# LimpBunion22/VIT-FPGA

Hardware: AMD Instinct MI355X
Metric: images/sec ViT-B/16 224x224, batch 512 per GPU (higher is better)
Workload: dtype bf16; 1 GPU; vit_base 224x224x3 inference, 512 images per GPU resident in HBM, random-init weights (seed 0); global_batch=512, per_gpu_batch=512

## Files before the change

### include/vithip.h

```cpp
#ifndef VITHIP_H
#define VITHIP_H

#include <stddef.h>
#include <stdint.h>

#ifdef __cplusplus
extern "C" {
#endif

#define VH_ABI_VERSION 1

#define VH_OK 0
#define VH_ERR_INVALID 1
#define VH_ERR_HIP 2
#define VH_ERR_STATE 3
#define VH_ERR_UNSUPPORTED 4
#define VH_ERR_NO_DEVICE 5
#define VH_ERR_RING_FULL 6
#define VH_ERR_RING_EMPTY 7

#define VH_DTYPE_BF16 0
#define VH_DTYPE_FP16 1
#define VH_DTYPE_FP8 2

// ... 104 lines not shown
int vh_ring_input_u8(vh_ctx* ctx, uint8_t** pinned_in_nhwc);
int vh_ring_submit_u8(vh_ctx* ctx, const uint8_t* in_nhwc_host, int batch);
int vh_ring_create_frames(vh_ctx* ctx, int slots, int batch_per_slot, size_t slot_bytes);
int vh_ring_input_frames(vh_ctx* ctx, uint8_t** pinned, size_t* capacity);
int vh_ring_submit_frames(vh_ctx* ctx, const uint8_t* frames_host, size_t nbytes, const vh_frame* desc, int batch);
int vh_ring_submit_frames_nv12(vh_ctx* ctx, const uint8_t* frames_host, size_t nbytes, const vh_frame_nv12* desc, int batch);

int vh_set_graph(vh_ctx* ctx, int enable);
int vh_get_graph(const vh_ctx* ctx, int* enabled, int* cached_graphs);

int vh_set_streams(vh_ctx* ctx, int n);
int vh_get_streams(const vh_ctx* ctx, int* n);

int vh_last_forward_us(const vh_ctx* ctx, int64_t* us);
int vh_last_kernel_ms(vh_ctx* ctx, double* ms);
int vh_profile_forward(vh_ctx* ctx, const float* in_nhwc_dev, int batch, float* logits_dev,
                       double* stage_ms, int n_stage_slots, int* n_stages_written);
const char* vh_stage_name(int stage_index);
int vh_set_stage_timing(vh_ctx* ctx, int stage_index);
int vh_get_stage_timing(vh_ctx* ctx, double* avg_ms, double* min_ms, int* launches);
int vh_set_step_timing(vh_ctx* ctx, int enable);
int vh_get_step_timing(vh_ctx* ctx, double* step_ms, int max_steps, int* steps);

int vh_debug_read(vh_ctx* ctx, int what, float* host_out, size_t n_floats);
int vh_debug_set_layers(vh_ctx* ctx, int n_layers);

#define VH_EPI_BIAS 0
#define VH_EPI_BIAS_GELU 1
#define VH_EPI_BIAS_RESID 2
#define VH_EPI_BIAS_F32 3
#define VH_EPI_PATCH 4
#define VH_EPI_LNFOLD 5
#define VH_EPI_LNFOLD_GELU 6
#define VH_EPI_RESID_LN 7
#define VH_EPI_RESID_SPLIT 8
#define VH_EPI_PATCH_SPLIT 9
#define VH_EPI_BIAS_QGELU 10
#define VH_EPI_LNFOLD_QGELU 11
int vh_op_gemm(const void* a16_dev, const void* w16_dev, const float* bias_dev, void* out_dev,
               int64_t M, int N, int K, int epilogue, const float* aux_dev, int aux_i,
               int dtype, int variant, void* stream);

int vh_op_gemm_fp8(const void* a8, const void* w8, const float* w_scale, const float* bias, void* out, int64_t M,
                   int N, int K, int epilogue, int variant , void* stream);
int vh_op_gemm_fp8_ex(const void* a8, const void* w8, const float* w_scale, const float* bias, void* out, int64_t M,
                      int N, int K, int epilogue, const float* c_dev, const float* stats_dev, void* out16,
                      float* partials, int variant, void* stream);
int vh_op_quantize_rows(const float* w, int rows, int cols, float post_scale, void* w8, float* scale, void* stream);

int vh_op_gemm_ex(const void* a16_dev, const void* w16_dev, const float* bias_dev, void* out_dev,
                  int64_t M, int N, int K, int epilogue, const float* aux_dev, int aux_i,
                  const float* stats_dev, void* out16_dev, float* partials_dev,
                  int dtype, int variant, void* stream);
int vh_op_rowstats_cast(const float* x_dev, int64_t rows, int dim, float eps, void* x16_dev, float* stats_dev,
                        int dtype, void* stream);
int vh_op_finalize_stats(const float* partials_dev, int nblk, int64_t rows, int dim, float eps, float* stats_dev,
                         void* stream);
int vh_op_rowstats_split(const float* x_dev, int64_t rows, int dim, float eps, void* hi_dev, void* lo_dev, float* stats_dev,
                         int dtype, void* stream);
int vh_op_fold_ln(const float* w_dev, const float* b_dev, const float* gamma_dev, const float* beta_dev, int rows,
                  int dim, float scale, void* w16_dev, float* c_dev, float* d_dev, int dtype, void* stream);
int vh_op_layernorm(const float* x_dev, int64_t rows, int dim, int64_t row_stride,
                    const float* gamma_dev, const float* beta_dev, float eps, void* out16_dev,
                    int dtype, void* stream);
int vh_op_pre_layernorm(const float* x_dev, int64_t rows, int dim, const float* gamma_dev, const float* beta_dev, float eps,
                        float* y32_dev, void* hi_dev, void* lo_dev, float* stats_dev, int dtype, void* stream);
#define VH_ATTN_Q_SCALE 0.18033688011112042f
int vh_op_attention(const void* qkv16_dev, int batch, int tokens, int heads, void* out16_dev,
                    int dtype, void* stream);
int vh_op_attention_stream(const void* qkv16_dev, int batch, int tokens, int heads, void* out16_dev,
                           int dtype, void* stream);
int vh_op_attention_hd(const void* qkv16_dev, int batch, int tokens, int heads, int head_dim, void* out16_dev,
                       int dtype, void* stream);
int vh_op_attention_cls(const void* qkv16_dev, int batch, int tokens, int heads, void* out16_dev,
                        int dtype, void* stream);
int vh_op_attention_layout(const void* qkv16_dev, int batch, int tokens, int heads, void* out16_dev,
                           int dtype, int out_tiled, int64_t in_hm_rows, void* stream);
int vh_op_im2col(const float* in_nhwc_dev, int batch, int image, int patch, int channels,
                 void* out16_dev, int dtype, void* stream);
int vh_op_im2col_padded(const float* in_nhwc_dev, int batch, int image, int patch, int channels, int kpad,
                        void* out16_dev, int dtype, void* stream);
int vh_op_im2col_u8(const uint8_t* in_nhwc_dev, int batch, int image, int patch, int channels, int kpad,
                    const float* scale_host, const float* shift_host, void* out16_dev, int dtype, void* stream);
int vh_op_resize_u8(const uint8_t* frames_dev, size_t nbytes, const vh_frame* desc_host, int batch, int channels,
                    int out_size, uint8_t* out_u8_dev, void* stream);
int vh_op_resize_nv12(const uint8_t* frames_dev, size_t nbytes, const vh_frame_nv12* desc_host, int batch, int out_size,
                      const float* m12_host, int chroma_site, uint8_t* out_u8_dev, void* stream);
int vh_op_cast(const float* in_dev, void* out16_dev, int64_t n, int dtype, void* stream);
int vh_op_fill(float* out_dev, int64_t n, uint64_t seed, uint32_t tensor_id, int kind,
               float sigma, void* stream);

int vh_bench_gemm(int device, int64_t M, int N, int K, int epilogue, int dtype, int variant, int iters,
                  double* avg_ms);

typedef struct vh_group vh_group;
int vh_group_create(const vh_config* cfg, const int* devices, int n, vh_group** out);
int vh_group_destroy(vh_group* g);
int vh_group_size(const vh_group* g, int* n);
int vh_group_member(vh_group* g, int i, vh_ctx** ctx, int* device);
const char* vh_group_last_error(const vh_group* g);
void vh_group_shard_bounds(int batch, int n, int r, int* lo, int* hi);
int vh_group_load_weights(vh_group* g, const void* host_blob, size_t nbytes);
int vh_group_init_weights_seeded(vh_group* g, uint64_t seed);
int vh_group_broadcast_weights(vh_group* g);
int vh_group_forward(vh_group* g, const float* in_nhwc_host, int batch, float* logits_host);
int vh_group_fill_inputs_seeded(vh_group* g, uint64_t seed, int batch_per_device);
// ... 31 lines not shown
```

### vit-fpga_amd/csrc/gemm_epilogue.h

```cpp
#pragma once

#include "vh_common.h"

namespace vh {

#ifndef VH_EPI_ABL
#define VH_EPI_ABL 0
#endif
#ifndef VH_EPI_NT
#define VH_EPI_NT 1
#endif
template <typename V>
__device__ __forceinline__ void epi_store(V v, V* p) {
    if constexpr (VH_EPI_NT) __builtin_nontemporal_store(v, p);
    else *p = v;
}

struct EpiArgs {
    const float* bias;
    void* out;
    int M, N;
    const float* aux;
    int aux_i;
    const float* stats;
    void* out16;
    float* partials;
    int64_t prow;
};

constexpr bool epi_has_qgelu(int epi) { return epi == VH_EPI_BIAS_QGELU || epi == VH_EPI_LNFOLD_QGELU; }
constexpr bool epi_has_act(int epi) { return epi == VH_EPI_BIAS_GELU || epi == VH_EPI_LNFOLD_GELU || epi_has_qgelu(epi); }
constexpr bool epi_is_lnfold(int epi) { return epi == VH_EPI_LNFOLD || epi == VH_EPI_LNFOLD_GELU || epi == VH_EPI_LNFOLD_QGELU; }
constexpr bool epi_is_16bit(int epi) { return epi == VH_EPI_BIAS || epi == VH_EPI_LNFOLD || epi_has_act(epi); }

__device__ __forceinline__ float gelu_fast(float v) {
    const float u = fabsf(v);
    const float t = __builtin_amdgcn_rcpf(fmaf(0.2316418882f, u, 1.0f));
    float p = fmaf(0.5307027145f, t, -0.7265760135f);
    p = fmaf(p, t, 0.7107068705f);
    p = fmaf(p, t, -0.142248368f);
    p = fmaf(p, t, 0.127414796f);
    p *= t;
    const float h = p * __builtin_amdgcn_exp2f(v * v * -0.72134752044f);
    return fmaf(-u, h, fmaxf(v, 0.f));
}

typedef __attribute__((ext_vector_type(2))) float f32x2;
template <int DEG> struct GeluW;
template <> struct GeluW<9> { static constexpr float a[10] = {1.111100093e-01f, 5.562581867e-02f, 3.875113651e-02f, 7.441916317e-02f, -2.459328771e-01f,
                                                                1.095633626e+00f, -2.419960260e+00f, 3.303298712e+00f, -2.415727854e+00f, 8.016663194e-01f}; };
template <> struct GeluW<8> { static constexpr float a[9] = {1.111119911e-01f, 5.524744466e-02f, 5.048053339e-02f, -6.402773410e-02f, 5.648611188e-01f,
                                                               -1.549515009e+00f, 2.612281084e+00f, -2.240322828e+00f, 8.585962057e-01f}; };
template <> struct GeluW<6> { static constexpr float a[7] = {1.111383960e-01f, 5.238987878e-02f, 9.770081192e-02f, -3.239865899e-01f, 1.061976552e+00f,
                                                               -1.360716462e+00f, 7.577903271e-01f}; };
__device__ __forceinline__ f32x2 pk_fma_clamp01(f32x2 a, f32x2 b, f32x2 c) {
    f32x2 d;
    asm("v_pk_fma_f32 %0, %1, %2, %3 clamp" : "=v"(d) : "v"(a), "v"(b), "v"(c));
    return d;
}
template <int DEG>
// ... 88 lines not shown
        if constexpr (EPI == VH_EPI_PATCH) {
            const int img = m / e.aux_i, p = m - img * e.aux_i;
            orow = (int64_t)img * (e.aux_i + 1) + 1 + p;
            posrow = e.aux + (int64_t)(1 + p) * N;
        }
        float rstd = 0.f, mr = 0.f;
        if constexpr (epi_is_lnfold(EPI)) {
            const float2 st = *(const float2*)(e.stats + 2 * (int64_t)m);
            rstd = st.y;
            mr = st.x * st.y;
        }
        f32x4 addv[NI];
        if constexpr (EPI == VH_EPI_BIAS_RESID || EPI == VH_EPI_PATCH) {
#pragma unroll
            for (int ni = 0; ni < NI; ++ni) {
                const int n = n0 + ni * 16;
                const bool ok = !GUARD || n < N;
                if constexpr (EPI == VH_EPI_BIAS_RESID) addv[ni] = ok ? *(const f32x4*)((const float*)e.out + orow * N + n) : f32x4{0.f, 0.f, 0.f, 0.f};
                else addv[ni] = ok ? *(const f32x4*)(posrow + n) : f32x4{0.f, 0.f, 0.f, 0.f};
            }
        }
#pragma unroll
        for (int ni = 0; ni < NI; ++ni) {
            const int n = n0 + ni * 16;
            if (GUARD && n >= N) continue;
            if constexpr (epi_is_16bit(EPI)) {
                const f32x4 v = epi_value16<EPI, T>(acc[mi][ni], bv[ni], cv[ni], mr, rstd);
                *(typename T::vec4*)((elem*)e.out + orow * N + n) = pack4<T>(v[0], v[1], v[2], v[3]);
            } else {
                const f32x4 v = acc[mi][ni] + bv[ni];
                f32x4* p = (f32x4*)((float*)e.out + orow * N + n);
                if constexpr (EPI == VH_EPI_BIAS_F32) *p = v;
                else *p = v + addv[ni];
            }
        }
    }
}

#ifndef VH_EPI_PRIO
#define VH_EPI_PRIO 1
#endif
__device__ __forceinline__ void epi_consts_from_lds(const char* sw, int frow, int fq, f32x4 (&bv)[4], f32x4 (&cv)[4], float2 (&lnst)[8]) {
    const uint32_t la = (uint32_t)(uintptr_t)sw + (uint32_t)((fq * 4) * 4), lr = (uint32_t)(uintptr_t)sw + (uint32_t)(frow * 8);
    asm volatile("ds_read_b128 %0, %8 offset:1024\n\tds_read_b128 %1, %8 offset:1088\n\tds_read_b128 %2, %8 offset:1152\n\tds_read_b128 %3, %8 offset:1216\n\t"
                 "ds_read_b128 %4, %8 offset:1280\n\tds_read_b128 %5, %8 offset:1344\n\tds_read_b128 %6, %8 offset:1408\n\tds_read_b128 %7, %8 offset:1472"
                 : "=&v"(bv[0]), "=&v"(bv[1]), "=&v"(bv[2]), "=&v"(bv[3]), "=&v"(cv[0]), "=&v"(cv[1]), "=&v"(cv[2]), "=&v"(cv[3]) : "v"(la));
    asm volatile("ds_read_b64 %0, %8\n\tds_read_b64 %1, %8 offset:128\n\tds_read_b64 %2, %8 offset:256\n\tds_read_b64 %3, %8 offset:384\n\t"
                 "ds_read_b64 %4, %8 offset:512\n\tds_read_b64 %5, %8 offset:640\n\tds_read_b64 %6, %8 offset:768\n\tds_read_b64 %7, %8 offset:896\n\t"
                 "s_waitcnt lgkmcnt(0)"
                 : "=&v"(lnst[0]), "=&v"(lnst[1]), "=&v"(lnst[2]), "=&v"(lnst[3]), "=&v"(lnst[4]), "=&v"(lnst[5]), "=&v"(lnst[6]), "=&v"(lnst[7]) : "v"(lr));
    asm volatile("" : "+v"(bv[0]), "+v"(bv[1]), "+v"(bv[2]), "+v"(bv[3]), "+v"(cv[0]), "+v"(cv[1]), "+v"(cv[2]), "+v"(cv[3]));
}

template <typename T, int EPI, int MI, int NI, int SMI = MI, bool MFULL = false, bool OTILED = false>
__device__ __forceinline__ void gemm_epilogue_staged(const f32x4 (&acc)[MI][NI], const EpiArgs& e, int m_w, int n_w,
                                                     int lane, char* sw, int prio_grp = -1, bool cpre = false) {
    static_assert(NI == 4, "staged epilogue assumes a 64-column wave tile");
    static_assert(MI % SMI == 0 && SMI % 2 == 0, "slice must divide the wave tile");
    using elem = typename T::elem;
    const int M = e.M, N = e.N;
    const int frow = lane & 15, fq = lane >> 4;
    f32x4 bv[NI], cv[NI];
    float2 lnst[epi_is_lnfold(EPI) ? MI : 1];
    auto consts_from_global = [&]() {
#pragma unroll
        for (int ni = 0; ni < NI; ++ni) {
            bv[ni] = *(const f32x4*)(e.bias + n_w + ni * 16 + fq * 4);
            if constexpr (epi_is_lnfold(EPI)) cv[ni] = *(const f32x4*)(e.aux + n_w + ni * 16 + fq * 4);
            else cv[ni] = f32x4{0.f, 0.f, 0.f, 0.f};
        }
        if constexpr (epi_is_lnfold(EPI)) {
#pragma unroll
            for (int mi = 0; mi < MI; ++mi) {
                int m = m_w + mi * 16 + frow;
                if constexpr (!MFULL) m = m < M ? m : M - 1;
                lnst[mi] = *(const float2*)(e.stats + 2 * (int64_t)m);
            }
        }
    };
    if constexpr (epi_is_lnfold(EPI) && MI == 8) {
        if (cpre) epi_consts_from_lds(sw, frow, fq, bv, cv, lnst);
        else consts_from_global();
    } else {
        consts_from_global();
    }

    if constexpr (epi_is_16bit(EPI) && (VH_EPI_ABL & 64)) {
#pragma unroll
        for (int mi = 0; mi < MI; ++mi)
#pragma unroll
            for (int ni = 0; ni < NI; ++ni) asm volatile("" :: "v"(acc[mi][ni]));
    } else if constexpr (epi_is_16bit(EPI) && epi_has_act(EPI) && MFULL && OTILED) {
        char* const obase = (char*)e.out + ((int64_t)(m_w >> 4) * (N >> 3) + (n_w >> 3) + (fq & 1) * 2 + (fq >> 1)) * 256 + frow * 16;
#pragma unroll
        for (int mi = 0; mi < MI; ++mi) {
            if constexpr (VH_EPI_PRIO == 1) {
                if (prio_grp >= 0 && (mi & 1) == 0) {
                    if (((mi >> 1) + prio_grp) & 1) __builtin_amdgcn_s_setprio(1);
                    else __builtin_amdgcn_s_setprio(0);
                }
            }
            float rstd = 0.f, mr = 0.f;
            if constexpr (epi_is_lnfold(EPI)) { rstd = lnst[mi].y; mr = lnst[mi].x * lnst[mi].y; }
#pragma unroll
            for (int j = 0; j < NI / 2; ++j) {
                const f32x4 v0 = epi_value16<EPI, T>(acc[mi][2 * j], bv[2 * j], cv[2 * j], mr, rstd);
                const f32x4 v1 = epi_value16<EPI, T>(acc[mi][2 * j + 1], bv[2 * j + 1], cv[2 * j + 1], mr, rstd);
// ... 78 lines not shown
            }
        };
        load_pass(0, xa[0]);
#pragma unroll
        for (int h = 0; h < NP; ++h) {
            if (h + 1 < NP) load_pass(h + 1, xa[(h + 1) & 1]);
#pragma unroll
            for (int mi = 0; mi < FMI; ++mi) {
                const int r = mi * 16 + frow;
#pragma unroll
                for (int ni = 0; ni < NI; ++ni)
                    *(f32x4*)(sw + r * 256 + (((ni * 4 + fq) ^ (r & 15)) << 4)) = acc[h * FMI + mi][ni] + bv[ni];
            }
#pragma unroll
            for (int i = 0; i < NL; ++i) {
                const int r = i * 8 + rr;
                const f32x4 v0 = *(const f32x4*)(sw + r * 256 + (((2 * pc) ^ (r & 15)) << 4));
                const f32x4 v1 = *(const f32x4*)(sw + r * 256 + (((2 * pc + 1) ^ (r & 15)) << 4));
                int m;
                const int64_t off = where(h, i, m);
                const bool ok = MFULL || m < M;
                const Add8& a = xa[h & 1][i];
                const f32x4 h0 = dec4(a.h[0]), h1 = dec4(a.h[1]);
                float v[8];
                float s1 = 0.f, s2 = 0.f;
#pragma unroll
                for (int j = 0; j < 8; ++j) {
                    v[j] = (j < 4 ? v0[j] : v1[j - 4]) + ((j < 4 ? h0[j] : h1[j - 4]) + (float)a.l[j]);
                    s1 += v[j];
                    s2 = fmaf(v[j], v[j], s2);
                }
                const u32x2 hn{pack4_e4m3(v[0], v[1], v[2], v[3]), pack4_e4m3(v[4], v[5], v[6], v[7])};
                const f32x4 d0 = dec4(hn[0]), d1 = dec4(hn[1]);
                lvec8 ln;
#pragma unroll
                for (int j = 0; j < 8; ++j) ln[j] = (typename BF16::elem)(v[j] - (j < 4 ? d0[j] : d1[j - 4]));
                if (ok && !(VH_EPI_ABL & 4)) { *(u32x2*)(hi + off) = hn; *(lvec8*)(lo + off) = ln; }
                s1 += dpp_mov<0xB1>(s1); s2 += dpp_mov<0xB1>(s2);
                s1 += dpp_mov<0x4E>(s1); s2 += dpp_mov<0x4E>(s2);
                s1 += dpp_mov<0x141>(s1); s2 += dpp_mov<0x141>(s2);
                if (ok && pc == 0 && !(VH_EPI_ABL & 1)) *(float2*)(e.partials + 2 * ((int64_t)(n_w >> 6) * M + m)) = make_float2(s1, s2);
            }
        }
    } else if constexpr (EPI == VH_EPI_RESID_SPLIT || EPI == VH_EPI_PATCH_SPLIT) {
        using vec8 = typename T::vec8;
        constexpr bool PATCHS = EPI == VH_EPI_PATCH_SPLIT;
        constexpr int FMI = SMI / 2, NP = MI / FMI, NL = FMI * 2;
        const int rr = lane >> 3, pc = lane & 7;
        elem* const hi = (elem*)e.out;
        uint8_t* const lo = (uint8_t*)e.out16;
        const int64_t prow = PATCHS ? e.prow : (int64_t)M;
        struct Add { vec8 h; u32x2 l; f32x4 p0, p1; };
        Add xa[2][NL];
        const int q0 = PATCHS ? m_w / e.aux_i : 0, r0 = PATCHS ? m_w - q0 * e.aux_i : 0;
        auto where = [&](int h, int i, int& m, int64_t& orow, int& p) {
            const int dr = h * FMI * 16 + i * 8 + rr;
            m = m_w + dr;
            p = 0;
            if constexpr (PATCHS) {
                int img = q0;
                p = r0 + dr;
                while (p >= e.aux_i) { p -= e.aux_i; ++img; }
                orow = (int64_t)m + img + 1;
            } else {
                orow = m;
            }
            return orow * N + n_w + 8 * pc;
        };
        auto load_pass = [&](int h, Add (&a)[NL]) {
#pragma unroll
            for (int i = 0; i < NL; ++i) {
                int m, p;
                int64_t orow;
                const int64_t off = where(h, i, m, orow, p);
                if constexpr (PATCHS) {
                    const float* pr = e.aux + (int64_t)(1 + p) * N + n_w + 8 * pc;
                    a[i].p0 = *(const f32x4*)pr;
                    a[i].p1 = *(const f32x4*)(pr + 4);
                } else {
                    if ((MFULL || m < M) && !(VH_EPI_ABL & 8)) { a[i].h = *(const vec8*)(hi + off); a[i].l = *(const u32x2*)(lo + off); }
                    else { a[i].h = vec8{}; a[i].l = u32x2{0u, 0u}; }
                }
            }
        };
        load_pass(0, xa[0]);
#pragma unroll
        for (int h = 0; h < NP; ++h) {
            if (h + 1 < NP) load_pass(h + 1, xa[(h + 1) & 1]);
#pragma unroll
            for (int mi = 0; mi < FMI; ++mi) {
                const int r = mi * 16 + frow;
#pragma unroll
                for (int ni = 0; ni < NI; ++ni)
                    *(f32x4*)(sw + r * 256 + (((ni * 4 + fq) ^ (r & 15)) << 4)) = acc[h * FMI + mi][ni] + bv[ni];
            }
#pragma unroll
            for (int i = 0; i < NL; ++i) {
                const int r = i * 8 + rr;
                const f32x4 v0 = *(const f32x4*)(sw + r * 256 + (((2 * pc) ^ (r & 15)) << 4));
                const f32x4 v1 = *(const f32x4*)(sw + r * 256 + (((2 * pc + 1) ^ (r & 15)) << 4));
                int m, p;
                int64_t orow;
                const int64_t off = where(h, i, m, orow, p);
                const bool ok = MFULL || m < M;
                const Add& a = xa[h & 1][i];
                float v[8], ln[8];
                vec8 hn;
                float s1 = 0.f, s2 = 0.f;
                f32x4 l0 = f32x4{0.f, 0.f, 0.f, 0.f}, l1 = l0;
                if constexpr (!PATCHS) { l0 = lo8_unpack4<T>(a.l[0]); l1 = lo8_unpack4<T>(a.l[1]); }
#pragma unroll
                for (int j = 0; j < 8; ++j) {
                    const float add = PATCHS ? (j < 4 ? a.p0[j] : a.p1[j - 4]) : ((float)a.h[j] + (j < 4 ? l0[j] : l1[j - 4]));
                    v[j] = (j < 4 ? v0[j] : v1[j - 4]) + add;
                    hn[j] = (elem)v[j];
                    ln[j] = v[j] - (float)hn[j];
                    s1 += v[j];
                    s2 = fmaf(v[j], v[j], s2);
                }
                if (ok && !(VH_EPI_ABL & 4)) {
                    *(vec8*)(hi + off) = hn;
                    *(u32x2*)(lo + off) = u32x2{lo8_pack4<T>(ln[0], ln[1], ln[2], ln[3]), lo8_pack4<T>(ln[4], ln[5], ln[6], ln[7])};
                }
                s1 += dpp_mov<0xB1>(s1); s2 += dpp_mov<0xB1>(s2);
                s1 += dpp_mov<0x4E>(s1); s2 += dpp_mov<0x4E>(s2);
                s1 += dpp_mov<0x141>(s1); s2 += dpp_mov<0x141>(s2);
                if (ok && pc == 0 && !(VH_EPI_ABL & 1)) *(float2*)(e.partials + 2 * ((int64_t)(n_w >> 6) * prow + orow)) = make_float2(s1, s2);
            }
        }
    } else {
        constexpr int FMI = SMI / 2, NP = MI / FMI, NL = FMI * 4;
        constexpr bool RESID = EPI == VH_EPI_BIAS_RESID || EPI == VH_EPI_RESID_LN;
        const int rr = lane >> 4, pc = lane & 15;
        f32x4 xv[2][RESID ? NL : 1];
        auto line = [&](int h, int i, int& m, int& n) {
            const int r = i * 4 + rr;
            n = n_w + ((pc ^ (r & 15)) << 2);
            m = m_w + h * FMI * 16 + r;
            return (f32x4*)((float*)e.out + (int64_t)m * N + n);
        };
        auto load_pass = [&](int h, f32x4 (&x)[RESID ? NL : 1]) {
            if constexpr (RESID) {
#pragma unroll
                for (int i = 0; i < NL; ++i) {
                    int m, n;
                    const f32x4* p = line(h, i, m, n);
                    x[i] = (m < M && !(VH_EPI_ABL & 8)) ? *p : f32x4{0.f, 0.f, 0.f, 0.f};
                }
            }
        };
        load_pass(0, xv[0]);
#pragma unroll
        for (int h = 0; h < NP; ++h) {
            if (h + 1 < NP) load_pass(h + 1, xv[(h + 1) & 1]);
#pragma unroll
            for (int mi = 0; mi < FMI; ++mi) {
                const int r = mi * 16 + frow;
#pragma unroll
                for (int ni = 0; ni < NI; ++ni)
                    *(f32x4*)(sw + r * 256 + (((ni * 4 + fq) ^ (r & 15)) << 4)) = acc[h * FMI + mi][ni] + bv[ni];
            }
#pragma unroll
            for (int i = 0; i < NL; ++i) {
                const int r = i * 4 + rr;
                f32x4 v = *(const f32x4*)(sw + r * 256 + (pc << 4));
                int m, n;
                f32x4* p = line(h, i, m, n);
                const bool ok = m < M;
                if constexpr (RESID) v = v + xv[h & 1][i];
                if (ok && !(VH_EPI_ABL & 4)) *p = v;
                if constexpr (EPI == VH_EPI_RESID_LN) {
                    if (ok && !(VH_EPI_ABL & 2)) *(typename T::vec4*)((elem*)e.out16 + (int64_t)m * N + n) = pack4<T>(v[0], v[1], v[2], v[3]);
                    const float s1 = row16_sum((v[0] + v[1]) + (v[2] + v[3]));
                    const float s2 = row16_sum(fmaf(v[0], v[0], v[1] * v[1]) + fmaf(v[2], v[2], v[3] * v[3]));
                    if (ok && pc == 0 && !(VH_EPI_ABL & 1)) *(float2*)(e.partials + 2 * ((int64_t)(n_w >> 6) * M + m)) = make_float2(s1, s2);
                }
            }
        }
    }
}

template <typename T, int EPI, int MI, int NI, int SMI = MI, bool BARRIER = true>
__device__ __forceinline__ void gemm_epilogue(const f32x4 (&acc)[MI][NI], const EpiArgs& e, int m_w, int n_w, int lane,
                                              bool n_full, bool m_full, char* smem, int wave) {
    if constexpr (EPI != VH_EPI_PATCH) {
        if (EPI == VH_EPI_RESID_LN || EPI == VH_EPI_RESID_SPLIT || EPI == VH_EPI_PATCH_SPLIT || n_full) {
            if constexpr (BARRIER) __syncthreads();
            if (m_full && epi_is_16bit(EPI)) gemm_epilogue_staged<T, EPI, MI, NI, SMI, true>(acc, e, m_w, n_w, lane, smem + wave * (SMI * 16 * 128));
            else gemm_epilogue_staged<T, EPI, MI, NI, SMI, false>(acc, e, m_w, n_w, lane, smem + wave * (SMI * 16 * 128));
            return;
        }
    }
    if constexpr (EPI != VH_EPI_RESID_LN && EPI != VH_EPI_RESID_SPLIT && EPI != VH_EPI_PATCH_SPLIT) {
        const int m0 = m_w + (lane & 15), n0 = n_w + (lane >> 4) * 4;
        if (n_full && m_full) gemm_epilogue_impl<T, EPI, MI, NI, false>(acc, e, m0, n0);
        else gemm_epilogue_impl<T, EPI, MI, NI, true>(acc, e, m0, n0);
    }
}

template <int EPI, int MI, int NI, int SMI, bool MFULL = false, bool OTILED = false>
__device__ __forceinline__ void gemm_epilogue8(const f32x4 (&acc)[MI][NI], const EpiArgs& e, int m_w, int n_w, int lane,
                                               bool n_full, char* smem, int wave, bool cpre = false) {
    static_assert(NI == 4 && MI % SMI == 0, "64-column wave tile");
    static_assert(EPI == VH_EPI_BIAS || (epi_has_act(EPI)), "8-bit output: bias, bias + activation or LN-fold + activation");
    const int M = e.M, N = e.N;
    const int frow = lane & 15, fq = lane >> 4;
    uint8_t* const out = (uint8_t*)e.out;
    auto value = [&](const f32x4& a, const f32x4& b, const f32x4& cq = f32x4{0.f, 0.f, 0.f, 0.f}, float mean_rstd = 0.f, float rstd = 0.f) {
        f32x4 v = epi_value16<EPI, E4M3>(a, b, cq, mean_rstd, rstd);
        return pack4_e4m3(v[0], v[1], v[2], v[3]);
    };
    if (n_full || epi_is_lnfold(EPI)) {
        f32x4 bv[NI], cv[NI];
        float2 lnst[epi_is_lnfold(EPI) ? MI : 1];
        bool have = false;
        if constexpr (epi_is_lnfold(EPI) && MI == 8) { if (cpre) { epi_consts_from_lds(smem + wave * (SMI * 16 * 128), frow, fq, bv, cv, lnst); have = true; } }
        if (!have) {
#pragma unroll
            for (int ni = 0; ni < NI; ++ni) {
                bv[ni] = *(const f32x4*)(e.bias + n_w + ni * 16 + fq * 4);
                if constexpr (epi_is_lnfold(EPI)) cv[ni] = *(const f32x4*)(e.aux + n_w + ni * 16 + fq * 4);
                else cv[ni] = f32x4{0.f, 0.f, 0.f, 0.f};
            }
            if constexpr (epi_is_lnfold(EPI)) {
#pragma unroll
                for (int mi = 0; mi < MI; ++mi) {
                    int m = m_w + mi * 16 + frow;
                    m = m < M ? m : M - 1;
                    lnst[mi] = *(const float2*)(e.stats + 2 * (int64_t)m);
                }
            }
        }
        if constexpr (OTILED && MFULL) {
            uint8_t* const obase = out + ((int64_t)(m_w >> 4) * (N >> 4) + (n_w >> 4) + fq) * 256 + frow * 16;
#pragma unroll
            for (int mi = 0; mi < MI; ++mi) {
                uint32_t x[NI];
#pragma unroll
                for (int ni = 0; ni < NI; ++ni) {
                    if constexpr (epi_is_lnfold(EPI)) x[ni] = value(acc[mi][ni], bv[ni], cv[ni], lnst[mi].x * lnst[mi].y, lnst[mi].y);
                    else x[ni] = value(acc[mi][ni], bv[ni]);
                }
// ... 53 lines not shown
```

### vit-fpga_amd/csrc/kernels_gemm.hip

```cpp
#include <cstdlib>

#include "gemm_epilogue.h"
#include "vh_kernels.h"

namespace vh {

template <typename T, int BM, int BN, int WM, int WN, int EPI>
__global__ void __launch_bounds__(WM* WN * 64)
gemm_nt_kernel(const typename T::elem* __restrict__ A, const typename T::elem* __restrict__ W,
               const float* __restrict__ bias, void* __restrict__ outp, int M, int N, int K,
               const float* __restrict__ aux, int aux_i, int tiles_m, int tiles_n, const float* __restrict__ stats,
               void* __restrict__ out16, float* __restrict__ partials, int64_t prow) {
    using elem = typename T::elem;
    using vec8 = typename T::vec8;
    constexpr int NW = WM * WN;
    constexpr int BK = 64;
    constexpr int ROWS = BM + BN;
    constexpr int STAGE_BYTES = ROWS * 128;
    constexpr int GROUPS_A = BM / 8;
    constexpr int GROUPS = ROWS / 8;
    constexpr int LOADS = GROUPS / NW;
    constexpr int LOADS_A = GROUPS_A / NW;
    constexpr int TM = BM / WM, TN = BN / WN;
    constexpr int MI = TM / 16, NI = TN / 16;
// ... 112 lines not shown
    case VH_EPI_PATCH: return launch_tile<T, VH_EPI_PATCH>(g, variant, s);
    case VH_EPI_LNFOLD: return launch_tile<T, VH_EPI_LNFOLD>(g, variant, s);
    case VH_EPI_LNFOLD_GELU: return launch_tile<T, VH_EPI_LNFOLD_GELU>(g, variant, s);
    case VH_EPI_RESID_LN: return launch_tile<T, VH_EPI_RESID_LN>(g, variant, s);
    case VH_EPI_RESID_SPLIT: return launch_tile<T, VH_EPI_RESID_SPLIT>(g, variant, s);
    case VH_EPI_PATCH_SPLIT: return launch_tile<T, VH_EPI_PATCH_SPLIT>(g, variant, s);
    case VH_EPI_BIAS_QGELU: return launch_tile<T, VH_EPI_BIAS_QGELU>(g, variant, s);
    case VH_EPI_LNFOLD_QGELU: return launch_tile<T, VH_EPI_LNFOLD_QGELU>(g, variant, s);
    default: return hipErrorInvalidValue;
    }
}

int gemm_pp_variant(int epilogue) {
    (void)epilogue;
    static const int v = [] { const int e = env_int("VH_GEMM_PP", 0); return e < 5 || e > 7 ? 0 : e; }();
    return v ? v : 6;
}
int gemm_pick_variant(int64_t M, int N, int epilogue) {
    static const int min_tiles = [] { const int e = env_int("VH_PP_MIN_TILES", 128); return e < 1 ? 1 : e; }();
    const int64_t t256 = ((M + 255) / 256) * ((N + 255) / 256);
    return t256 >= min_tiles ? gemm_pp_variant(epilogue) : 1;
}

bool gemm_tiled_applies(int64_t M, int N, int K) {
    return M > 0 && M % 256 == 0 && N % 256 == 0 && K % 64 == 0 && K / 64 >= 4 && gemm_pick_variant(M, N, VH_EPI_BIAS) == 6;
}

bool gemm_tiled_applies_f8(int64_t M, int N, int K) {
    return M > 0 && M % 256 == 0 && N % 256 == 0 && K % 128 == 0 && K / 128 >= 4 && gemm_pp_variant(VH_EPI_BIAS) == 6;
}

const char* gemm_check(const GemmArgs& g) {
    if (g.M <= 0 || g.N <= 0 || g.K <= 0) return "gemm: empty shape";
    if (g.K % 64) return "gemm: K must be a multiple of 64";
    if (g.N % 4) return "gemm: N must be a multiple of 4";
    if (g.M > 0x7fffffff) return "gemm: M too large";
    if (g.epilogue < 0 || g.epilogue > VH_EPI_LNFOLD_QGELU) return "gemm: unknown epilogue";
    if ((g.epilogue == VH_EPI_LNFOLD || g.epilogue == VH_EPI_LNFOLD_GELU || g.epilogue == VH_EPI_LNFOLD_QGELU) && (!g.stats || !g.aux)) return "gemm: LNFOLD needs stats and c (aux)";
    if ((g.epilogue == VH_EPI_RESID_LN || g.epilogue == VH_EPI_RESID_SPLIT) && (!g.out16 || !g.partials || g.N % 256))
        return "gemm: RESID_LN / RESID_SPLIT need out16, partials and N % 256 == 0";
    if (g.epilogue == VH_EPI_PATCH && (!g.aux || g.aux_i <= 0)) return "gemm: EPI_PATCH needs pos-emb and patches/image";
    if (g.epilogue == VH_EPI_PATCH_SPLIT && (!g.aux || g.aux_i <= 0 || !g.out16 || !g.partials || g.N % 256 || g.prow < 0))
        return "gemm: EPI_PATCH_SPLIT needs pos-emb, patches/image, the lo plane, partials and N % 256 == 0";
    if (g.dtype != VH_DTYPE_BF16 && g.dtype != VH_DTYPE_FP16) return "gemm: dtype";
    if (g.variant < 0 || g.variant > 7) return "gemm: variant";
    if (g.variant == 3 || g.variant == 4) return "gemm: variants 3/4 (BK=32 pipeline) were removed";
    if (!g.a || !g.w || !g.bias || !g.out) return "gemm: null pointer";
    return nullptr;
}

hipError_t launch_gemm(const GemmArgs& g, hipStream_t s) {
    if (gemm_check(g)) return hipErrorInvalidValue;
    const int variant = g.variant ? g.variant : gemm_pick_variant(g.M, g.N, g.epilogue);
    if ((g.out_tiled || g.ab_tiled) && variant != 6) return hipErrorInvalidValue;
    if ((g.tile_count || g.tile_begin) && variant != 5 && variant != 7) return hipErrorInvalidValue;
    return g.dtype == VH_DTYPE_BF16 ? launch_epi<BF16>(g, variant, s) : launch_epi<FP16>(g, variant, s);
}

}
```

### vit-fpga_amd/csrc/kernels_gemm5.hip

```cpp
#include <cstdlib>
#include <type_traits>

#include "gemm_epilogue.h"
#include "vh_kernels.h"

#ifndef VH_PP_SMI
#define VH_PP_SMI 2
#endif

namespace vh {

#ifndef VH_MAIN_ABL
#define VH_MAIN_ABL 0
#endif
#ifndef VH_PP_CPRE
#define VH_PP_CPRE 1
#endif
constexpr int kAblHalf = (VH_MAIN_ABL & 64) ? 1 : 0;
constexpr int kWPieces = kAblHalf ? 2 : 4;
#ifdef VH_DIAG_STAMPS
#ifndef VH_DIAG_KT
#define VH_DIAG_KT -1
#endif
#ifndef VH_DIAG_REC_IT
#define VH_DIAG_REC_IT 1
#endif
#define VH_STAMP_PARAM , unsigned long long* __restrict__ stamps
__device__ __forceinline__ unsigned long long diag_rt() {
    unsigned long long t;
    asm volatile("s_memrealtime %0\n\ts_waitcnt lgkmcnt(0)" : "=s"(t)::"memory");
    return t;
}
__device__ __forceinline__ unsigned long long diag_ct() {
    unsigned long long t;
    asm volatile("s_memtime %0\n\ts_waitcnt lgkmcnt(0)" : "=s"(t)::"memory");
    return t;
}
__device__ __forceinline__ unsigned long long diag_hwid() {
    unsigned int hw, xcc;
    asm volatile("s_getreg_b32 %0, hwreg(HW_REG_HW_ID)" : "=s"(hw));
    asm volatile("s_getreg_b32 %0, hwreg(HW_REG_XCC_ID)" : "=s"(xcc));
    return ((unsigned long long)xcc << 32) | hw;
}
#define VH_STAMP(i, expr) do { __builtin_amdgcn_sched_barrier(0); st_[i] = (expr); __builtin_amdgcn_sched_barrier(0); } while (0)
#define VH_PSTAMP(i) do { if (pst_) { __builtin_amdgcn_sched_barrier(0); const unsigned long long t_ = diag_ct(); \
    if (lane == 0) pst_[i] = t_; __builtin_amdgcn_sched_barrier(0); } } while (0)
#else
#define VH_PSTAMP(i) do { } while (0)
#define VH_STAMP_PARAM
#define VH_STAMP(i, expr) do { } while (0)
#endif

template <int EPI, bool F8>
__host__ __device__ constexpr bool pp_uses_cpre() {
    return VH_PP_CPRE && epi_is_lnfold(EPI) && !(F8 && epi_has_act(EPI));
}

template <int N>
__device__ __forceinline__ void pp_wait_vmcnt() {
    asm volatile("s_waitcnt vmcnt(%0)" ::"n"(N) : "memory");
}
__device__ __forceinline__ void pp_barrier() {
    __builtin_amdgcn_sched_barrier(0);
#if VH_MAIN_ABL & 16
    return;
#endif
    __builtin_amdgcn_s_barrier();
    __builtin_amdgcn_sched_barrier(0);
}
__device__ __forceinline__ int xcd_remap(int bid, int n) {
    const int xcd = bid & 7, qd = n >> 3, rm = n & 7;
    return (xcd < rm ? xcd * (qd + 1) : rm * (qd + 1) + (xcd - rm) * qd) + (bid >> 3);
}

template <typename T, int EPI, bool PERSIST, bool F8 = false, int AST = 2, bool OT = false, bool AT = false>
__global__ void __launch_bounds__(512, 2)
gemm_nt_pp_kernel(const void* __restrict__ Av, const void* __restrict__ Wv,
                  const float* __restrict__ bias, void* __restrict__ outp, int M, int N, int K,
                  const float* __restrict__ aux, int aux_i, int tiles_m, int tiles_n, const float* __restrict__ stats,
                  void* __restrict__ out16, float* __restrict__ partials, int tile0, int sn,
                  const float* __restrict__ wscale, int64_t prow VH_STAMP_PARAM) {
    using vec8 = typename T::vec8;
#ifdef VH_DIAG_STAMPS
    unsigned long long st_[8] = {0, 0, 0, 0, 0, 0, 0, 0};
    int it_ = 0;
    constexpr int rec_it_ = PERSIST ? VH_DIAG_REC_IT : 0;
#define first_tile_ (it_ == rec_it_)
#endif
    constexpr int BM = 256, BN = 256;
    constexpr int KT_BYTES = 128;
    static_assert(!(OT || AT) || PERSIST, "tiled layouts: persistent form only");
    constexpr int KT_STEP = AT ? 2048 : KT_BYTES;
    constexpr int STAGE_BYTES = 65536, W_OFF = 32768;
    static_assert(AST == 2 || (AST == 3 && !PERSIST), "three A stages: one tile per workgroup only");
    const char* const A = (const char*)Av;
    const char* const W = (const char*)Wv;
    const int64_t row_bytes = (int64_t)K * (F8 ? 1 : 2);
    constexpr int MI = 8, NI = 4;

    extern __shared__ __attribute__((aligned(16))) char smem[];

    const int ntiles = tiles_m * tiles_n;
    const int stride = (int)gridDim.x;
    int t = tile0 + xcd_remap(blockIdx.x, stride);

    const int lane = threadIdx.x & 63;
    const int wave = __builtin_amdgcn_readfirstlane(threadIdx.x >> 6);
    const int grp = wave >> 2, wn = wave & 3;

    const int lr = lane >> 3, lc = (lane & 7) ^ lr;
    const int rb = (int)row_bytes;
    struct TileSrc { const char *a, *w; uint32_t oa[4], ow[4]; };
    int tile_m = 0, tile_n = 0;
    auto tile_coords = [&](int tt, int& tm, int& tn) {
        if (sn > 0) {
            const int blk = tiles_m * sn, sc = tt / blk, r = tt - sc * blk;
            const int width = tiles_n - sc * sn < sn ? tiles_n - sc * sn : sn;
            tm = r / width;
            tn = sc * sn + (r - tm * width);
        } else {
            tm = tt / tiles_n;
            tn = tt - tm * tiles_n;
        }
    };
    auto base_a = [&](int tm) { return A + (int64_t)tm * BM * row_bytes; };
    auto base_w = [&](int tn) { return W + (int64_t)tn * BN * row_bytes; };
    TileSrc cur;
    auto setup_tile = [&](int tt) {
// ... 222 lines not shown
            for (int mi = 0; mi < MI_A; ++mi)
#pragma unroll
                for (int ni = 0; ni < NI; ++ni) {
                    if constexpr (VH_MAIN_ABL & 1) asm volatile("" : "+v"(acc[mi][ni]) : "v"(wf1[ni]), "v"(xf[mi]));
                    else acc[mi][ni] = T::mfma16(wf1[ni], xf[mi], acc[mi][ni]);
                }
            __builtin_amdgcn_s_setprio(0);
            c1_wait(kt);
            VH_PSTAMP(7);
            pp_barrier();
        }
        }
        if (grp == 0) pp_barrier();
#ifdef VH_DIAG_STAMPS
        if (first_tile_) { VH_STAMP(6, diag_ct()); VH_STAMP(2, diag_rt()); }
#endif

        const int m_w = tile_m * BM + grp * 128, n_w = tile_n * BN + wn * 64;
        const bool m_full = (tile_m + 1) * BM <= M, n_full = (tile_n + 1) * BN <= N;
        char* const stage_epi = smem + (PERSIST ? 2 * STAGE_BYTES : STAGE_BYTES);
        const EpiArgs e{bias, outp, M, N, aux, aux_i, stats, out16, partials, prow};
        int lane_e = lane;
        if constexpr (PERSIST) asm volatile("" : "+v"(lane_e));
        if constexpr (F8) {
#pragma clang fp contract(off)
            const int fq_e = lane_e >> 4;
            f32x4 wsv[NI];
            if (cpre) {
                const uint32_t la = (uint32_t)(uintptr_t)(smem + 2 * STAGE_BYTES + wave * 4096) + (uint32_t)(fq_e * 16);
                static_assert(NI == 4, "64-column wave tile");
                asm volatile("ds_read_b128 %0, %4 offset:1536\n\tds_read_b128 %1, %4 offset:1600\n\tds_read_b128 %2, %4 offset:1664\n\tds_read_b128 %3, %4 offset:1728\n\t"
                             "s_waitcnt lgkmcnt(0)" : "=&v"(wsv[0]), "=&v"(wsv[1]), "=&v"(wsv[2]), "=&v"(wsv[3]) : "v"(la));
            } else {
#pragma unroll
                for (int ni = 0; ni < NI; ++ni) {
                    const int n = n_w + ni * 16 + fq_e * 4;
                    wsv[ni] = n < N ? *(const f32x4*)(wscale + n) : f32x4{0.f, 0.f, 0.f, 0.f};
                }
            }
#pragma unroll
            for (int ni = 0; ni < NI; ++ni) {
#pragma unroll
                for (int mi = 0; mi < MI; ++mi) acc[mi][ni] = acc[mi][ni] * wsv[ni];
            }
        }
        if constexpr (PERSIST) {
            constexpr int SLICE = VH_PP_SMI * 16 * 128;
            static_assert(VH_PP_SMI == 2, "staging region of the persistent form: 8 waves x 4 KiB");
            if constexpr (F8 && epi_has_act(EPI))
                gemm_epilogue8<EPI, MI, NI, VH_PP_SMI, true, OT>(acc, e, m_w, n_w, lane_e, true, stage_epi, wave, cpre);
            else if constexpr (F8 && (EPI == VH_EPI_RESID_LN || EPI == VH_EPI_RESID_SPLIT))
                gemm_epilogue_staged<E4M3, EPI, MI, NI, VH_PP_SMI, true>(acc, e, m_w, n_w, lane_e, stage_epi + wave * SLICE);
            else
                gemm_epilogue_staged<T, EPI, MI, NI, VH_PP_SMI, true, OT>(acc, e, m_w, n_w, lane_e, stage_epi + wave * SLICE, epi_is_16bit(EPI) ? grp : -1, cpre);
        } else {
            if constexpr (F8 && epi_has_act(EPI))
                gemm_epilogue8<EPI, MI, NI, VH_PP_SMI>(acc, e, m_w, n_w, lane_e, n_full, stage_epi, wave);
            else if constexpr (F8 && (EPI == VH_EPI_RESID_LN || EPI == VH_EPI_RESID_SPLIT))
                gemm_epilogue<E4M3, EPI, MI, NI, 4, false>(acc, e, m_w, n_w, lane_e, n_full, m_full, stage_epi, wave);
            else
                gemm_epilogue<T, EPI, MI, NI, (epi_is_16bit(EPI) ? VH_PP_SMI : 4), false>(acc, e, m_w, n_w, lane_e, n_full, m_full, stage_epi, wave);
        }
#ifdef VH_DIAG_STAMPS
        if (first_tile_) VH_STAMP(3, diag_rt());
        if (!has_next && first_tile_) asm volatile("s_waitcnt vmcnt(0)" ::: "memory");
        if (first_tile_) {
            VH_STAMP(4, diag_rt());
            st_[7] = diag_hwid();
            if (stamps && lane == 0) {
#pragma unroll
                for (int i = 0; i < 8; ++i) stamps[((size_t)blockIdx.x * 8 + wave) * 16 + i] = st_[i];
            }
        }
        ++it_;
#endif
        if (!has_next) break;
        par = (par + nk) & 1;
        first = false;
        t = t_next;
        tile_m = tm_n;
        tile_n = tn_n;
    }
}

static int gemm_super_columns(int tiles_n) {
    static const int env = [] { const int e = env_int("VH_PP_SN", -1); return e < -1 ? -1 : e; }();
    if (env >= 0) return env > 0 && env < tiles_n ? env : 0;
    if (tiles_n < 6) return 0;
    if (tiles_n % 4 == 0) return 4;
    if (tiles_n % 3 == 0) return 3;
    return 4;
}

#ifdef VH_DIAG_STAMPS
struct DiagRec { int64_t M; int N, K, epi, f8, grid, variant; };
static unsigned long long* g_diag_buf = nullptr;
static int g_diag_slots = 0, g_diag_max_wgs = 0;
static long long g_diag_count = 0;
static DiagRec g_diag_rec[1024];
static unsigned long long* diag_next(const GemmArgs& g, int epi, bool f8, int grid, int variant) {
    if (!g_diag_buf || grid > g_diag_max_wgs) return nullptr;
    const int slot = (int)(g_diag_count % g_diag_slots);
    g_diag_rec[slot] = DiagRec{g.M, g.N, g.K, epi, f8 ? 1 : 0, grid, variant};
    ++g_diag_count;
    return g_diag_buf + (size_t)slot * g_diag_max_wgs * 128;
}
#define VH_STAMP_ARG(g, epi, f8, grid, variant) , diag_next(g, epi, f8, grid, variant)
#else
#define VH_STAMP_ARG(g, epi, f8, grid, variant)
#endif

template <typename T, int EPI, bool F8, bool PERSIST, int AST, bool OT = false, bool AT = false>
static hipError_t launch_pp_one(const GemmArgs& g, int grid, int tiles_m, int tiles_n, hipStream_t s) {
    constexpr size_t lds = (AST == 3 || PERSIST) ? 163840 : 131072;
    auto k = gemm_nt_pp_kernel<T, EPI, PERSIST, F8, AST, OT, AT>;
    static LdsDone lds_done;
    if (hipError_t e = ensure_dynamic_lds((const void*)k, lds, lds_done); e != hipSuccess) return e;
    hipLaunchKernelGGL(k, dim3(grid), dim3(512), lds, s, g.a, g.w, g.bias, g.out, (int)g.M, g.N, g.K, g.aux, g.aux_i, tiles_m,
                       tiles_n, g.stats, g.out16, g.partials, PERSIST ? 0 : g.tile_begin, (g.tile_count || g.tile_begin) ? 0 : gemm_super_columns(tiles_n),
                       F8 ? (g.wscale ? g.wscale : g.aux) : (const float*)nullptr, gemm_prow(g)
                       VH_STAMP_ARG(g, EPI, F8, grid, PERSIST ? 6 : (AST == 3 ? 7 : 5)));
    return hipGetLastError();
}

template <typename T, int EPI, bool F8>
static hipError_t launch_pp(const GemmArgs& g, int mode, hipStream_t s) {
    if constexpr (EPI == VH_EPI_PATCH) { if (mode == 1) mode = 0; }
    const int tiles_m = (int)((g.M + 255) / 256), tiles_n = (g.N + 255) / 256;
    int ntiles = tiles_m * tiles_n;
    if (g.tile_count > 0) {
        if (mode == 1 || g.tile_begin < 0 || g.tile_begin + g.tile_count > ntiles) return hipErrorInvalidValue;
        ntiles = g.tile_count;
    } else if (g.tile_begin != 0) {
        return hipErrorInvalidValue;
    }
    if (mode == 2) return launch_pp_one<T, EPI, F8, false, 3>(g, ntiles, tiles_m, tiles_n, s);
    if constexpr (EPI != VH_EPI_PATCH) {
        const int full_m = (int)(g.M / 256);
        const int nk = g.K / (F8 ? 128 : 64);
        if (mode == 1 && (g.N % 256 != 0 || full_m == 0 || nk < (pp_uses_cpre<EPI, F8>() ? 4 : 2))) mode = 0;
        if (mode == 1 && full_m != tiles_m && g.variant != 6) mode = 0;
        if ((g.out_tiled || g.ab_tiled) && (mode != 1 || full_m != tiles_m)) return hipErrorInvalidValue;
        if (mode == 1) {
            const int num_cu = device_num_cu();
            if (!num_cu) return hipErrorUnknown;
            const int nfull = full_m * tiles_n;
            if constexpr (epi_has_act(EPI) || EPI == VH_EPI_LNFOLD || (!F8 && EPI == VH_EPI_BIAS)) {
                if (g.out_tiled) return g.ab_tiled ? hipErrorInvalidValue : launch_pp_one<T, EPI, F8, true, 2, true, false>(g, nfull < num_cu ? nfull : num_cu, full_m, tiles_n, s);
            }
            if constexpr (F8 ? EPI == VH_EPI_RESID_SPLIT : (EPI == VH_EPI_RESID_SPLIT || EPI == VH_EPI_BIAS)) {
                if (g.ab_tiled) return g.out_tiled ? hipErrorInvalidValue : launch_pp_one<T, EPI, F8, true, 2, false, true>(g, nfull < num_cu ? nfull : num_cu, full_m, tiles_n, s);
            }
            if (g.out_tiled || g.ab_tiled) return hipErrorInvalidValue;
            if (hipError_t e = launch_pp_one<T, EPI, F8, true, 2>(g, nfull < num_cu ? nfull : num_cu, full_m, tiles_n, s); e != hipSuccess) return e;
            if (full_m == tiles_m) return hipSuccess;
            GemmArgs tail = g;
            tail.tile_begin = nfull;
            tail.tile_count = tiles_n;
            return launch_pp_one<T, EPI, F8, false, 2>(tail, tiles_n, tiles_m, tiles_n, s);
        }
    }
    if (g.out_tiled || g.ab_tiled) return hipErrorInvalidValue;
    return launch_pp_one<T, EPI, F8, false, 2>(g, ntiles, tiles_m, tiles_n, s);
}

template <typename T, int EPI>
hipError_t launch_gemm_pingpong(const GemmArgs& g, int mode, hipStream_t s) {
    return launch_pp<T, EPI, false>(g, mode, s);
}

#define VH_INST(T)                                                                                     \
    template hipError_t launch_gemm_pingpong<T, VH_EPI_BIAS>(const GemmArgs&, int, hipStream_t);       \
    template hipError_t launch_gemm_pingpong<T, VH_EPI_BIAS_GELU>(const GemmArgs&, int, hipStream_t);  \
    template hipError_t launch_gemm_pingpong<T, VH_EPI_BIAS_RESID>(const GemmArgs&, int, hipStream_t); \
    template hipError_t launch_gemm_pingpong<T, VH_EPI_BIAS_F32>(const GemmArgs&, int, hipStream_t);   \
    template hipError_t launch_gemm_pingpong<T, VH_EPI_PATCH>(const GemmArgs&, int, hipStream_t);       \
    template hipError_t launch_gemm_pingpong<T, VH_EPI_LNFOLD>(const GemmArgs&, int, hipStream_t);      \
    template hipError_t launch_gemm_pingpong<T, VH_EPI_LNFOLD_GELU>(const GemmArgs&, int, hipStream_t); \
    template hipError_t launch_gemm_pingpong<T, VH_EPI_RESID_LN>(const GemmArgs&, int, hipStream_t);   \
    template hipError_t launch_gemm_pingpong<T, VH_EPI_RESID_SPLIT>(const GemmArgs&, int, hipStream_t); \
    template hipError_t launch_gemm_pingpong<T, VH_EPI_PATCH_SPLIT>(const GemmArgs&, int, hipStream_t); \
    template hipError_t launch_gemm_pingpong<T, VH_EPI_BIAS_QGELU>(const GemmArgs&, int, hipStream_t);  \
    template hipError_t launch_gemm_pingpong<T, VH_EPI_LNFOLD_QGELU>(const GemmArgs&, int, hipStream_t);
VH_INST(BF16)
VH_INST(FP16)

hipError_t launch_gemm_fp8(const GemmArgs& g, hipStream_t s) {
    const int v = g.variant ? g.variant : gemm_pp_variant(g.epilogue);
    const int mode = v == 7 ? 2 : (v == 6 && !g.tile_count && !g.tile_begin ? 1 : 0);
    switch (g.epilogue) {
        case VH_EPI_BIAS: return launch_pp<BF16, VH_EPI_BIAS, true>(g, mode, s);
        case VH_EPI_BIAS_GELU: return launch_pp<BF16, VH_EPI_BIAS_GELU, true>(g, mode, s);
        case VH_EPI_BIAS_QGELU: return launch_pp<BF16, VH_EPI_BIAS_QGELU, true>(g, mode, s);
        case VH_EPI_BIAS_RESID: return launch_pp<BF16, VH_EPI_BIAS_RESID, true>(g, mode, s);
        case VH_EPI_BIAS_F32: return launch_pp<BF16, VH_EPI_BIAS_F32, true>(g, mode, s);
        case VH_EPI_LNFOLD: return g.wscale && g.stats && g.aux ? launch_pp<BF16, VH_EPI_LNFOLD, true>(g, mode, s) : hipErrorInvalidValue;
        case VH_EPI_LNFOLD_GELU: return g.wscale && g.stats && g.aux && g.N % 256 == 0 ? launch_pp<BF16, VH_EPI_LNFOLD_GELU, true>(g, mode, s) : hipErrorInvalidValue;
        case VH_EPI_LNFOLD_QGELU: return g.wscale && g.stats && g.aux && g.N % 256 == 0 ? launch_pp<BF16, VH_EPI_LNFOLD_QGELU, true>(g, mode, s) : hipErrorInvalidValue;
        case VH_EPI_RESID_LN: return g.out16 && g.partials && g.N % 256 == 0 ? launch_pp<BF16, VH_EPI_RESID_LN, true>(g, mode, s) : hipErrorInvalidValue;
        case VH_EPI_RESID_SPLIT: return g.out16 && g.partials && g.N % 256 == 0 ? launch_pp<BF16, VH_EPI_RESID_SPLIT, true>(g, mode, s) : hipErrorInvalidValue;
        default: return hipErrorInvalidValue;
    }
}

}

#ifdef VH_DIAG_STAMPS
extern "C" int vh_diag_stamps_arm(int slots, int max_wgs) {
    using namespace vh;
    if (slots < 1 || slots > 1024 || max_wgs < 1) return 1;
    if (g_diag_buf) { hipFree(g_diag_buf); g_diag_buf = nullptr; }
    if (hipMalloc((void**)&g_diag_buf, (size_t)slots * max_wgs * 1024) != hipSuccess) return 2;
    if (hipMemset(g_diag_buf, 0, (size_t)slots * max_wgs * 1024) != hipSuccess) return 2;
    g_diag_slots = slots; g_diag_max_wgs = max_wgs; g_diag_count = 0;
    return 0;
// ... 15 lines not shown
```

### vit-fpga_amd/csrc/kernels_misc.hip

```cpp
#include <type_traits>

#include "vh_kernels.h"

namespace vh {

template <typename T, int CH>
__global__ void __launch_bounds__(256)
layernorm_kernel(const float* __restrict__ x, int64_t rows, int dim, int64_t row_stride,
                 const float* __restrict__ gamma, const float* __restrict__ beta, float eps,
                 typename T::elem* __restrict__ out) {
    const int lane = threadIdx.x & 63;
    const int64_t row = (int64_t)blockIdx.x * 4 + (threadIdx.x >> 6);
    if (row >= rows) return;
    const int nchunk = dim >> 2;
    const f32x4* xr = (const f32x4*)(x + row * row_stride);
    f32x4 v[CH];
    float sum = 0.f;
#pragma unroll
    for (int i = 0; i < CH; ++i) {
        const int c = lane + 64 * i;
        v[i] = c < nchunk ? xr[c] : f32x4{0.f, 0.f, 0.f, 0.f};
        sum += (v[i][0] + v[i][1]) + (v[i][2] + v[i][3]);
    }
#pragma unroll
// ... 158 lines not shown
#pragma unroll
            for (int i = 0; i < 8; ++i) {
                v[i] = k0 + i < kp ? __builtin_fmaf((float)src[((int64_t)ky * image) * ch + r], s_scale[c], s_shift[c]) : 0.f;
                if (++r == pc) { r = 0; ++ky; }
                if (++c == ch) c = 0;
            }
        }
        const typename T::vec4 lo = pack4<T>(v[0], v[1], v[2], v[3]), hi = pack4<T>(v[4], v[5], v[6], v[7]);
        *(typename T::vec8*)(out + f * 8) = __builtin_shufflevector(lo, hi, 0, 1, 2, 3, 4, 5, 6, 7);
    }
}

hipError_t launch_im2col_u8(const uint8_t* in, int batch, int image, int patch, int channels, int kpad, const float* scale,
                            const float* shift, void* out16, int dtype, hipStream_t s) {
    if (patch <= 0 || image % patch || channels < 1 || channels > kMaxChannels || batch < 1) return hipErrorInvalidValue;
    const int kp = patch * patch * channels;
    if (kpad < kp || kpad % 8 || (dtype != VH_DTYPE_BF16 && dtype != VH_DTYPE_FP16)) return hipErrorInvalidValue;
    U8Norm norm;
    for (int c = 0; c < kMaxChannels; ++c) {
        norm.scale[c] = c < channels ? scale[c] : 0.f;
        norm.shift[c] = c < channels ? shift[c] : 0.f;
    }
    const int g = image / patch;
    const int64_t n8 = (int64_t)batch * g * g * (kpad / 8);
    const unsigned grid = (unsigned)((n8 + 255) / 256 < 16384 ? (n8 + 255) / 256 : 16384);
    const bool vec8 = (patch * channels) % 8 == 0 && (image * channels) % 8 == 0 && ((uintptr_t)in & 7) == 0;
    auto go = [&](auto kern, auto* o) { hipLaunchKernelGGL(kern, dim3(grid), dim3(256), 0, s, in, o, n8, image, patch, channels, kpad, norm); };
    if (dtype == VH_DTYPE_BF16) {
        if (vec8) go(im2col_u8_kernel<BF16, true>, (BF16::elem*)out16);
        else go(im2col_u8_kernel<BF16, false>, (BF16::elem*)out16);
    } else {
        if (vec8) go(im2col_u8_kernel<FP16, true>, (FP16::elem*)out16);
        else go(im2col_u8_kernel<FP16, false>, (FP16::elem*)out16);
    }
    return hipGetLastError();
}

__global__ void cls_rows_kernel(float* __restrict__ x, const float* __restrict__ cls, const float* __restrict__ pos,
                                int batch, int tokens, int dim) {
    const int64_t i = (int64_t)blockIdx.x * blockDim.x + threadIdx.x;
    if (i >= (int64_t)batch * dim) return;
    const int b = (int)(i / dim), d = (int)(i - (int64_t)b * dim);
    x[(int64_t)b * tokens * dim + d] = cls[d] + pos[d];
}
hipError_t launch_cls_rows(float* x, const float* cls, const float* pos, int batch, int tokens, int dim, hipStream_t s) {
    const int64_t n = (int64_t)batch * dim;
    hipLaunchKernelGGL(cls_rows_kernel, dim3((unsigned)((n + 255) / 256)), dim3(256), 0, s, x, cls, pos, batch, tokens, dim);
    return hipGetLastError();
}

template <typename T>
__global__ void __launch_bounds__(256)
cls_rows_split_kernel(typename T::elem* __restrict__ hi, uint8_t* __restrict__ lo, float* __restrict__ partials, int64_t prow,
                      const float* __restrict__ cls, const float* __restrict__ pos, int batch, int tokens, int dim) {
    const int lane = threadIdx.x & 63;
    const int b = blockIdx.x * 4 + (threadIdx.x >> 6);
    if (b >= batch) return;
    const int64_t row = (int64_t)b * tokens;
    for (int blk = 0; blk * 64 < dim; ++blk) {
        const int d = blk * 64 + lane;
        float v = 0.f;
        if (d < dim) {
            v = cls[d] + pos[d];
            const typename T::elem h = (typename T::elem)v;
            hi[row * dim + d] = h;
            lo[row * dim + d] = lo8_pack1<T>(v - (float)h);
        }
        float s1 = v, s2 = v * v;
#pragma unroll
        for (int o = 32; o > 0; o >>= 1) { s1 += __shfl_xor(s1, o); s2 += __shfl_xor(s2, o); }
        if (lane == 0) *(float2*)(partials + 2 * ((int64_t)blk * prow + row)) = make_float2(s1, s2);
    }
}
hipError_t launch_cls_rows_split(void* hi, void* lo, float* partials, int64_t prow, const float* cls, const float* pos, int batch,
                                 int tokens, int dim, int dtype, hipStream_t s) {
    if (batch <= 0 || dim % 64) return hipErrorInvalidValue;
    const dim3 grid((unsigned)((batch + 3) / 4));
    if (dtype == VH_DTYPE_BF16)
        hipLaunchKernelGGL(cls_rows_split_kernel<BF16>, grid, dim3(256), 0, s, (BF16::elem*)hi, (uint8_t*)lo, partials, prow, cls, pos, batch, tokens, dim);
    else
        hipLaunchKernelGGL(cls_rows_split_kernel<FP16>, grid, dim3(256), 0, s, (FP16::elem*)hi, (uint8_t*)lo, partials, prow, cls, pos, batch, tokens, dim);
    return hipGetLastError();
}

template <typename T>
__global__ void __launch_bounds__(256) cast_kernel(const float* __restrict__ in, typename T::elem* __restrict__ out, int64_t n4) {
    for (int64_t f = (int64_t)blockIdx.x * blockDim.x + threadIdx.x; f < n4; f += (int64_t)gridDim.x * blockDim.x) {
        const f32x4 v = ((const f32x4*)in)[f];
        ((typename T::vec4*)out)[f] = pack4<T>(v[0], v[1], v[2], v[3]);
    }
}
hipError_t launch_cast(const float* in, void* out16, int64_t n, int dtype, hipStream_t s) {
    if (n <= 0 || (n & 3)) return hipErrorInvalidValue;
    const int64_t n4 = n / 4;
    const unsigned grid = (unsigned)((n4 + 255) / 256 < 8192 ? (n4 + 255) / 256 : 8192);
    if (dtype == VH_DTYPE_FP8) hipLaunchKernelGGL(cast_kernel<E4M3>, dim3(grid), dim3(256), 0, s, in, (E4M3::elem*)out16, n4);
    else if (dtype == VH_DTYPE_BF16) hipLaunchKernelGGL(cast_kernel<BF16>, dim3(grid), dim3(256), 0, s, in, (BF16::elem*)out16, n4);
    else hipLaunchKernelGGL(cast_kernel<FP16>, dim3(grid), dim3(256), 0, s, in, (FP16::elem*)out16, n4);
    return hipGetLastError();
}

template <typename T>
__global__ void __launch_bounds__(256) cast_tiled_w_kernel(const float* __restrict__ w, typename T::elem* __restrict__ out, int rows, int cols) {
    const int64_t nchunk = (int64_t)rows * (cols >> 3);
    for (int64_t i = (int64_t)blockIdx.x * blockDim.x + threadIdx.x; i < nchunk; i += (int64_t)gridDim.x * blockDim.x) {
        const int r16 = (int)(i & 15);
        const int64_t bc = i >> 4;
        const int chunk = (int)(bc % (cols >> 3)), block = (int)(bc / (cols >> 3));
        const float* src = w + (int64_t)(block * 16 + r16) * cols + chunk * 8;
        const f32x4 a = *(const f32x4*)src, b = *(const f32x4*)(src + 4);
        const typename T::vec4 lo = pack4<T>(a[0], a[1], a[2], a[3]), hi = pack4<T>(b[0], b[1], b[2], b[3]);
        *(typename T::vec8*)(out + i * 8) = __builtin_shufflevector(lo, hi, 0, 1, 2, 3, 4, 5, 6, 7);
    }
}
hipError_t launch_cast_tiled_w(const float* w, int rows, int cols, void* w16, int dtype, hipStream_t s) {
    if (rows <= 0 || cols <= 0 || (rows & 15) || (cols & 7)) return hipErrorInvalidValue;
    const int64_t nchunk = (int64_t)rows * (cols >> 3);
    const unsigned grid = (unsigned)((nchunk + 255) / 256 < 8192 ? (nchunk + 255) / 256 : 8192);
    if (dtype == VH_DTYPE_BF16) hipLaunchKernelGGL(cast_tiled_w_kernel<BF16>, dim3(grid), dim3(256), 0, s, w, (BF16::elem*)w16, rows, cols);
    else if (dtype == VH_DTYPE_FP16) hipLaunchKernelGGL(cast_tiled_w_kernel<FP16>, dim3(grid), dim3(256), 0, s, w, (FP16::elem*)w16, rows, cols);
    else return hipErrorInvalidValue;
    return hipGetLastError();
}

__global__ void __launch_bounds__(256) tile_bytes_kernel(const u32x4* __restrict__ w, u32x4* __restrict__ out, int rows, int cols) {
    const int cpr = cols >> 4;
    const int64_t nchunk = (int64_t)rows * cpr;
    for (int64_t i = (int64_t)blockIdx.x * blockDim.x + threadIdx.x; i < nchunk; i += (int64_t)gridDim.x * blockDim.x) {
        const int r16 = (int)(i & 15);
        const int64_t bc = i >> 4;
        const int chunk = (int)(bc % cpr), block = (int)(bc / cpr);
        out[i] = w[(int64_t)(block * 16 + r16) * cpr + chunk];
    }
}
// ... 405 lines not shown
                if constexpr (!std::is_same<T, E4M3>::value) {
                    uint8_t* const xlo = (uint8_t*)lo_;
                    if (xlo) *(uint32_t*)(xlo + row * dim + 4 * c) = lo8_pack4<T>(v[i][0] - (float)hq[0], v[i][1] - (float)hq[1],
                                                                                v[i][2] - (float)hq[2], v[i][3] - (float)hq[3]);
                } else {
                    typename BF16::elem* const xlo = (typename BF16::elem*)lo_;
                    if (xlo) {
                        const uint32_t w = (uint32_t)hq;
                        *(typename BF16::vec4*)(xlo + row * dim + 4 * c) =
                            pack4<BF16>(v[i][0] - __builtin_amdgcn_cvt_f32_fp8((int)w, 0), v[i][1] - __builtin_amdgcn_cvt_f32_fp8((int)w, 1),
                                        v[i][2] - __builtin_amdgcn_cvt_f32_fp8((int)w, 2), v[i][3] - __builtin_amdgcn_cvt_f32_fp8((int)w, 3));
                    }
                }
            }
        }
    }
#pragma unroll
    for (int o = 32; o > 0; o >>= 1) yvar += __shfl_xor(yvar, o);
    const float yrstd = 1.0f / sqrtf(yvar / (float)dim + eps);
    if (stats && lane == 0) *(float2*)(stats + 2 * row) = make_float2(ymean, yrstd);
    if (guard) ln_guard_update(row < guard_rows ? fabsf(ymean) * yrstd : 0.f, guard);
}

template <typename T>
static hipError_t pre_ln_t(const float* x, int64_t rows, int dim, const float* g, const float* b, float eps, float* y32, void* hi, void* lo,
                           float* stats, hipStream_t s, int64_t guard_rows, unsigned int* guard, unsigned int* amax_guard) {
    const dim3 grid((unsigned)((rows + 3) / 4)), block(256);
    auto h = (typename T::elem*)hi;
#define VH_PRE_LN(CH) hipLaunchKernelGGL((pre_layernorm_kernel<T, CH>), grid, block, 0, s, x, rows, dim, g, b, eps, y32, h, lo, stats, guard_rows, guard, amax_guard)
    if (dim <= 256) VH_PRE_LN(1);
    else if (dim <= 512) VH_PRE_LN(2);
    else if (dim <= 768) VH_PRE_LN(3);
    else if (dim <= 1024) VH_PRE_LN(4);
    else if (dim <= 1280) VH_PRE_LN(5);
    else if (dim <= 2048) VH_PRE_LN(8);
    else return hipErrorInvalidValue;
#undef VH_PRE_LN
    return hipGetLastError();
}
hipError_t launch_pre_layernorm(const float* x, int64_t rows, int dim, const float* gamma, const float* beta, float eps, float* y32,
                                void* hi, void* lo, float* stats, int dtype, hipStream_t s, int64_t guard_rows, unsigned int* guard,
                                unsigned int* amax_guard) {
    if (rows <= 0 || dim <= 0 || (dim & 3) || dim > 2048 || !x || !gamma || !beta || (!y32 && !hi) || (lo && !hi)) return hipErrorInvalidValue;
    if (dtype == VH_DTYPE_FP8) return pre_ln_t<E4M3>(x, rows, dim, gamma, beta, eps, y32, hi, lo, stats, s, guard_rows, guard, amax_guard);
    if (dtype == VH_DTYPE_BF16) return pre_ln_t<BF16>(x, rows, dim, gamma, beta, eps, y32, hi, lo, stats, s, guard_rows, guard, amax_guard);
    if (dtype == VH_DTYPE_FP16) return pre_ln_t<FP16>(x, rows, dim, gamma, beta, eps, y32, hi, lo, stats, s, guard_rows, guard, amax_guard);
    return hipErrorInvalidValue;
}

template <typename T>
__global__ void __launch_bounds__(256)
layernorm_split_kernel(const typename T::elem* __restrict__ hi, const void* __restrict__ lo_, int64_t rows, int dim,
                       int64_t row_stride, const float* __restrict__ gamma, const float* __restrict__ beta, float eps,
                       float* __restrict__ out) {
    const int lane = threadIdx.x & 63;
    const int64_t row = (int64_t)blockIdx.x * 4 + (threadIdx.x >> 6);
    if (row >= rows) return;
    const typename T::elem* hr = hi + row * row_stride;
    auto xk = [&](int k) {
        if constexpr (std::is_same<T, E4M3>::value)
            return __builtin_amdgcn_cvt_f32_fp8((int)hr[k], 0) + (float)((const typename BF16::elem*)lo_ + row * row_stride)[k];
        else
            return (float)hr[k] + lo8_unpack1<T>(((const uint8_t*)lo_ + row * row_stride)[k]);
    };
    float sum = 0.f;
    for (int k = lane; k < dim; k += 64) sum += xk(k);
#pragma unroll
    for (int o = 32; o > 0; o >>= 1) sum += __shfl_xor(sum, o);
    const float mean = sum / (float)dim;
    float var = 0.f;
    for (int k = lane; k < dim; k += 64) { const float d = (xk(k)) - mean; var += d * d; }
#pragma unroll
    for (int o = 32; o > 0; o >>= 1) var += __shfl_xor(var, o);
    const float rstd = 1.0f / sqrtf(var / (float)dim + eps);
    for (int k = lane; k < dim; k += 64) out[row * dim + k] = ((xk(k)) - mean) * rstd * gamma[k] + beta[k];
}
hipError_t launch_layernorm_split(const void* hi, const void* lo, int64_t rows, int dim, int64_t row_stride, const float* gamma,
                                  const float* beta, float eps, float* out32, int dtype, hipStream_t s) {
    if (rows <= 0 || dim <= 0) return hipErrorInvalidValue;
    const dim3 grid((unsigned)((rows + 3) / 4)), block(256);
    if (dtype == VH_DTYPE_FP8)
        hipLaunchKernelGGL(layernorm_split_kernel<E4M3>, grid, block, 0, s, (const E4M3::elem*)hi, lo, rows, dim, row_stride, gamma, beta, eps, out32);
    else if (dtype == VH_DTYPE_BF16)
        hipLaunchKernelGGL(layernorm_split_kernel<BF16>, grid, block, 0, s, (const BF16::elem*)hi, (const void*)lo, rows, dim, row_stride, gamma, beta, eps, out32);
    else
        hipLaunchKernelGGL(layernorm_split_kernel<FP16>, grid, block, 0, s, (const FP16::elem*)hi, (const void*)lo, rows, dim, row_stride, gamma, beta, eps, out32);
    return hipGetLastError();
}

__device__ __forceinline__ void ln_guard_update(float ratio, unsigned int* guard) {
    unsigned int b = __float_as_uint(ratio) & 0x7FFFFFFFu;
#pragma unroll
    for (int o = 32; o > 0; o >>= 1) { const unsigned int t = (unsigned int)__shfl_xor((int)b, o); b = t > b ? t : b; }
    if ((threadIdx.x & 63) == 0 && b > __hip_atomic_load(guard, __ATOMIC_RELAXED, __HIP_MEMORY_SCOPE_AGENT)) atomicMax(guard, b);
}
__global__ void __launch_bounds__(256)
finalize_stats_kernel(const float* __restrict__ partials, int nblk, int64_t rows, int dim, float eps, float* __restrict__ stats,
                      int64_t guard_rows, unsigned int* __restrict__ guard, unsigned int* __restrict__ amax_guard) {
    const int64_t r = (int64_t)blockIdx.x * blockDim.x + threadIdx.x;
    float ratio = 0.f, bound = 0.f;
    if (r < rows) {
        float s1 = 0.f, s2 = 0.f, b2 = 0.f;
        constexpr int U = 16;
        for (int b0 = 0; b0 < nblk; b0 += U) {
            float2 p[U];
#pragma unroll
            for (int u = 0; u < U; ++u)
                p[u] = b0 + u < nblk ? *(const float2*)(partials + 2 * ((int64_t)(b0 + u) * rows + r)) : make_float2(0.f, 0.f);
#pragma unroll
            for (int u = 0; u < U; ++u) {
                s1 += p[u].x;
                s2 += p[u].y;
                b2 = fmaxf(b2, p[u].y);
            }
        }
        const float mean = s1 / (float)dim;
        const float var = fmaxf(s2 / (float)dim - mean * mean, 0.f);
        const float rstd = 1.0f / sqrtf(var + eps);
        *(float2*)(stats + 2 * r) = make_float2(mean, rstd);
        if (r < guard_rows) { ratio = fabsf(mean) * rstd; bound = sqrtf(b2); }
    }
    if (guard) ln_guard_update(ratio, guard);
    if (amax_guard) ln_guard_update(bound, amax_guard);
}
hipError_t launch_finalize_stats(const float* partials, int nblk, int64_t rows, int dim, float eps, float* stats, hipStream_t s,
                                 int64_t guard_rows, unsigned int* guard, unsigned int* amax_guard) {
    if (rows <= 0 || nblk <= 0) return hipErrorInvalidValue;
    hipLaunchKernelGGL(finalize_stats_kernel, dim3((unsigned)((rows + 255) / 256)), dim3(256), 0, s, partials, nblk, rows, dim, eps, stats,
                       guard_rows, guard, amax_guard);
    return hipGetLastError();
}
__global__ void __launch_bounds__(256)
ln_guard_kernel(const float* __restrict__ stats, int64_t rows, unsigned int* __restrict__ guard) {
    const int64_t r = (int64_t)blockIdx.x * blockDim.x + threadIdx.x;
    float ratio = 0.f;
    if (r < rows) {
        const float2 st = *(const float2*)(stats + 2 * r);
        ratio = fabsf(st.x) * st.y;
    }
// ... 191 lines not shown
```

### vit-fpga_amd/csrc/vh_common.h

```cpp
#pragma once

#include <hip/hip_runtime.h>
#include <stdint.h>

#include "../../include/vithip.h"

namespace vh {

typedef __attribute__((ext_vector_type(8))) __bf16 bf16x8;
typedef __attribute__((ext_vector_type(4))) __bf16 bf16x4;
typedef __attribute__((ext_vector_type(8))) _Float16 f16x8;
typedef __attribute__((ext_vector_type(4))) _Float16 f16x4;
typedef __attribute__((ext_vector_type(4))) float f32x4;
typedef __attribute__((ext_vector_type(16))) float f32x16;
typedef __attribute__((ext_vector_type(4))) uint32_t u32x4;
typedef __attribute__((ext_vector_type(2))) uint32_t u32x2;

struct BF16 {
    using elem = __bf16;
    using vec8 = bf16x8;
    using vec4 = bf16x4;
    static constexpr int id = VH_DTYPE_BF16;
    static __device__ __forceinline__ f32x4 mfma16(vec8 a, vec8 b, f32x4 c) {
        return __builtin_amdgcn_mfma_f32_16x16x32_bf16(a, b, c, 0, 0, 0);
// ... 32 lines not shown

template <typename T>
__device__ __forceinline__ typename T::vec4 pack4(float a, float b, float c, float d) {
    typedef float f32x2_ __attribute__((ext_vector_type(2)));
    typedef typename T::elem e2_ __attribute__((ext_vector_type(2)));
    const e2_ lo = __builtin_convertvector(f32x2_{a, b}, e2_), hi = __builtin_convertvector(f32x2_{c, d}, e2_);
    return __builtin_shufflevector(lo, hi, 0, 1, 2, 3);
}

typedef __attribute__((ext_vector_type(8))) int i32x8;
struct E4M3 {
    using elem = uint8_t;
    using vec4 = uint32_t;
    static constexpr int id = VH_DTYPE_FP8;
};
__device__ __forceinline__ uint32_t pack4_e4m3(float a, float b, float c, float d) {
    a = __builtin_amdgcn_fmed3f(a, -448.f, 448.f);
    b = __builtin_amdgcn_fmed3f(b, -448.f, 448.f);
    c = __builtin_amdgcn_fmed3f(c, -448.f, 448.f);
    d = __builtin_amdgcn_fmed3f(d, -448.f, 448.f);
    int p = __builtin_amdgcn_cvt_pk_fp8_f32(a, b, 0, false);
    p = __builtin_amdgcn_cvt_pk_fp8_f32(c, d, p, true);
    return (uint32_t)p;
}
template <>
__device__ __forceinline__ uint32_t pack4<E4M3>(float a, float b, float c, float d) {
    return pack4_e4m3(a, b, c, d);
}
template <>
__device__ __forceinline__ f32x4 pack4<F32OUT>(float a, float b, float c, float d) {
    return f32x4{a, b, c, d};
}

template <typename T> struct Lo8;
template <> struct Lo8<BF16> { static constexpr float scale = 32.f, inv = 1.f / 32.f; };
template <> struct Lo8<FP16> { static constexpr float scale = 256.f, inv = 1.f / 256.f; };
template <typename T>
__device__ __forceinline__ uint32_t lo8_pack4(float a, float b, float c, float d) {
    return pack4_e4m3(a * Lo8<T>::scale, b * Lo8<T>::scale, c * Lo8<T>::scale, d * Lo8<T>::scale);
}
template <typename T>
__device__ __forceinline__ f32x4 lo8_unpack4(uint32_t w) {
    typedef float f32x2_ __attribute__((ext_vector_type(2)));
    const f32x2_ a = __builtin_amdgcn_cvt_pk_f32_fp8((int)w, false), b = __builtin_amdgcn_cvt_pk_f32_fp8((int)w, true);
    return f32x4{a[0] * Lo8<T>::inv, a[1] * Lo8<T>::inv, b[0] * Lo8<T>::inv, b[1] * Lo8<T>::inv};
}
template <typename T>
__device__ __forceinline__ uint8_t lo8_pack1(float a) {
    a = __builtin_amdgcn_fmed3f(a * Lo8<T>::scale, -448.f, 448.f);
    return (uint8_t)(__builtin_amdgcn_cvt_pk_fp8_f32(a, a, 0, false) & 0xFF);
}
template <typename T>
__device__ __forceinline__ float lo8_unpack1(uint8_t b) { return __builtin_amdgcn_cvt_f32_fp8((int)b, 0) * Lo8<T>::inv; }

__device__ __forceinline__ void asm_lds_dma16(const void* base, uint32_t lane_off, uint32_t lds_addr) {
    asm volatile("s_mov_b32 m0, %0\n\ts_nop 4\n\tglobal_load_lds_dwordx4 %1, %2"
                 :: "s"(lds_addr), "v"(lane_off), "s"(base) : "memory", "m0");
}
__device__ __forceinline__ void asm_lds_dma4(const void* base, uint32_t lane_off, uint32_t lds_addr) {
    asm volatile("s_mov_b32 m0, %0\n\ts_nop 4\n\tglobal_load_lds_dword %1, %2"
                 :: "s"(lds_addr), "v"(lane_off), "s"(base) : "memory", "m0");
}
__device__ __forceinline__ void asm_atomic_add_ret_issue(unsigned int* base, uint32_t add, uint32_t& ret) {
    const uint32_t zero = 0;
    asm volatile("s_nop 4\n\tglobal_atomic_add %0, %1, %2, %3 sc0" : "=&v"(ret) : "v"(zero), "v"(add), "s"(base) : "memory");
}

__device__ __forceinline__ float gelu_erf(float v) {
    return 0.5f * v * (1.0f + erff(v * 0.70710678118654752440f));
}

__host__ __device__ __forceinline__ uint64_t mix64(uint64_t x) {
    x += 0x9E3779B97F4A7C15ull;
    x ^= x >> 30;
    x *= 0xBF58476D1CE4E5B9ull;
    x ^= x >> 27;
    x *= 0x94D049BB133111EBull;
    x ^= x >> 31;
    return x;
}
__host__ __device__ __forceinline__ uint64_t rng_stream(uint64_t seed, uint32_t tensor_id) {
    return mix64(mix64(seed) ^ (uint64_t)tensor_id);
}
__host__ __device__ __forceinline__ float rng_uniform(uint64_t stream, uint64_t i) {
    const uint64_t w = mix64(stream ^ i);
    const int32_t u = (int32_t)(w >> 40) - (1 << 23);
    return (float)u * (1.0f / 8388608.0f);
}
__host__ __device__ __forceinline__ float rng_ih4(uint64_t stream, uint64_t i, double scale,
                                                  float offset) {
    const uint64_t w = mix64(stream ^ i);
    const int32_t s = (int32_t)(w & 0xFFFF) + (int32_t)((w >> 16) & 0xFFFF) +
                      (int32_t)((w >> 32) & 0xFFFF) + (int32_t)((w >> 48) & 0xFFFF) - 131070;
    const float v = (float)((double)s * scale);
    return offset + v;
}
constexpr double kIH4Std = 37837.22725;

enum : uint32_t { TID_PATCH_W = 1, TID_PATCH_B = 2, TID_CLS = 3, TID_POS = 4, TID_PRE_LN_W = 5, TID_PRE_LN_B = 6, TID_LAYER0 = 16,
                  TID_FINAL = 0x7000, TID_IMAGES = 0x100 };

}
```

### vit-fpga_amd/csrc/vh_kernels.h

```cpp
#pragma once

#include <atomic>
#include <cstdlib>
#include <vector>

#include "vh_common.h"

namespace vh {

struct GemmArgs {
    const void* a;
    const void* w;
    const float* bias;
    void* out;
    int64_t M;
    int N, K;
    int epilogue;
    const float* aux;
    int aux_i;
    int dtype;
    int variant;
    const float* stats = nullptr;
    void* out16 = nullptr;
    float* partials = nullptr;
    const float* wscale = nullptr;
    int tile_begin = 0, tile_count = 0;
    int64_t prow = 0;
    int out_tiled = 0, ab_tiled = 0;
};
bool gemm_tiled_applies(int64_t M, int N, int K);
hipError_t launch_cast_tiled_w(const float* w, int rows, int cols, void* w16, int dtype, hipStream_t stream);
bool gemm_tiled_applies_f8(int64_t M, int N, int K);
hipError_t launch_tile_bytes(const void* w8, int rows, int cols, void* out, hipStream_t stream);

inline int64_t gemm_prow(const GemmArgs& g) {
    if (g.epilogue != VH_EPI_PATCH_SPLIT) return g.M;
    return g.prow > 0 ? g.prow : (g.M / g.aux_i) * (int64_t)(g.aux_i + 1);
}

hipError_t launch_gemm(const GemmArgs& g, hipStream_t stream);
hipError_t launch_gemm_fp8(const GemmArgs& g, hipStream_t stream);
const char* gemm_check(const GemmArgs& g);
int gemm_pick_variant(int64_t M, int N, int epilogue);
int gemm_pp_variant(int epilogue);

hipError_t launch_layernorm(const float* x, int64_t rows, int dim, int64_t row_stride,
                            const float* gamma, const float* beta, float eps, void* out16,
                            int dtype, hipStream_t stream);
constexpr int VH_DTYPE_F32_INTERNAL = 100;
hipError_t launch_head_f32(const float* y, const float* w, const float* bias, float* out, int batch, int classes, int dim,
                           hipStream_t stream);
constexpr float kAttnQScale = 0.125f * 1.4426950408889634f;
hipError_t launch_attention(const void* qkv16, int batch, int tokens, int heads, void* out16,
                            int dtype, unsigned int* ticket, hipStream_t stream, bool ticket_zeroed = false, bool out_tiled = false,
                            int64_t in_hm_rows = 0);
bool attention_tiled_applies(int batch, int tokens, int heads);
hipError_t launch_attention_cls(const void* qkv16, int batch, int tokens, int heads, void* out16, int dtype, hipStream_t stream);
size_t attention_lds_bytes(int tokens);
constexpr int kAttnStreamMaxTokens = 4097;
hipError_t launch_attention_stream(const void* qkv16, int batch, int tokens, int heads, void* out16, int dtype, hipStream_t stream);
constexpr int kAttnHdMaxWidth = 2048;
bool attention_hd_supported(int head_dim);
hipError_t launch_attention_hd(const void* qkv16, int batch, int tokens, int heads, int head_dim, void* out16, int dtype,
                               hipStream_t stream);
inline float attention_q_scale(int head_dim) {
    return head_dim == 64 ? kAttnQScale : (float)(1.4426950408889634 / __builtin_sqrt((double)head_dim));
}
hipError_t launch_im2col(const float* in_nhwc, int batch, int image, int patch, int channels, int kpad,
                         void* out16, int dtype, hipStream_t stream);
constexpr int kMaxChannels = 64;
hipError_t launch_im2col_u8(const uint8_t* in_nhwc, int batch, int image, int patch, int channels, int kpad,
                            const float* scale, const float* shift, void* out16, int dtype, hipStream_t stream);
constexpr int kResizeMaxTaps = 65, kResizeMaxScale = 32, kResizeMaxSide = 8192;
constexpr int kResizeLdsFloats = 16384;
constexpr int kResizeFrameWords = 16;
int resize_axis_table(int n_in, double lo, double hi, int n_out, int32_t* first, int32_t* count, float* weights, int max_taps);
const char* resize_plan_build(const vh_frame* desc, int batch, int channels, int S, size_t nbytes, bool base_aligned4,
                              std::vector<uint32_t>* words, int* max_tiles);
hipError_t launch_resize_u8(const uint8_t* frames, const uint32_t* plan_dev, int batch, int channels, int S, int max_tiles,
                            uint8_t* out_u8, hipStream_t stream);
constexpr int kResizeNv12FrameWords = 24;
int resize_axis_table_over(int n_in, double lo, double hi, double over, int n_out, int32_t* first, int32_t* count, float* weights,
                           int max_taps);
const char* resize_plan_build_nv12(const vh_frame_nv12* desc, int batch, int S, size_t nbytes, bool base_aligned2, int chroma_site,
                                   std::vector<uint32_t>* words, int* max_tiles);
hipError_t launch_resize_nv12(const uint8_t* frames, const uint32_t* plan_dev, int batch, int S, int max_tiles, const float* m12_host,
                              uint8_t* out_u8, hipStream_t stream);
int yuv_matrix(int standard, int full_range, float m[12]);
bool patch_fused_supported(int image, int patch, int channels, int dim);
hipError_t launch_patch_fused(const float* images, int batch, int image, int patch, int channels, const void* wp16, const float* bias,
                              const float* pos, void* hi, void* lo, float* partials, int64_t prow, int dim, int dtype, hipStream_t stream);
hipError_t launch_cls_rows(float* x, const float* cls, const float* pos, int batch, int tokens,
                           int dim, hipStream_t stream);
hipError_t launch_cls_rows_split(void* hi, void* lo, float* partials, int64_t prow, const float* cls, const float* pos, int batch,
                                 int tokens, int dim, int dtype, hipStream_t stream);
hipError_t launch_cast(const float* in, void* out16, int64_t n, int dtype, hipStream_t stream);
hipError_t launch_fill(float* out, int64_t n, uint64_t seed, uint32_t tensor_id, int kind,
                       float sigma, float offset, hipStream_t stream);
hipError_t launch_fake_quant_rows(const float* w, int rows, int cols, float* out, hipStream_t stream);
hipError_t launch_quantize_rows(const float* w, int rows, int cols, float post, void* w8, float* scale, hipStream_t stream);
hipError_t launch_pack_qkv(const float* qw, const float* qb, const float* kw, const float* kb,
                           const float* vw, const float* vb, int dim, float q_scale, void* w16,
                           float* b32, int dtype, hipStream_t stream);
hipError_t launch_permute_patch(const float* w_nchw, int dim, int channels, int patch, int kpad, void* w16,
                                int dtype, hipStream_t stream);
hipError_t launch_rowstats_cast(const float* x, int64_t rows, int dim, float eps, void* x16, float* stats, int dtype,
                                hipStream_t stream, int64_t guard_rows = 0, unsigned int* amax_guard = nullptr);
hipError_t launch_finalize_stats(const float* partials, int nblk, int64_t rows, int dim, float eps, float* stats,
                                 hipStream_t stream, int64_t guard_rows = 0, unsigned int* guard = nullptr,
                                 unsigned int* amax_guard = nullptr);
hipError_t launch_ln_guard(const float* stats, int64_t rows, unsigned int* guard, hipStream_t stream);
hipError_t launch_rowstats_split(const float* x, int64_t rows, int dim, float eps, void* hi, void* lo, float* stats, int dtype,
                                 hipStream_t stream, int64_t guard_rows = 0, unsigned int* amax_guard = nullptr);
hipError_t launch_pre_layernorm(const float* x, int64_t rows, int dim, const float* gamma, const float* beta, float eps, float* y32,
                                void* hi, void* lo, float* stats, int dtype, hipStream_t stream, int64_t guard_rows = 0,
                                unsigned int* guard = nullptr, unsigned int* amax_guard = nullptr);
hipError_t launch_layernorm_split(const void* hi, const void* lo, int64_t rows, int dim, int64_t row_stride, const float* gamma,
                                  const float* beta, float eps, float* out32, int dtype, hipStream_t stream);
hipError_t launch_fold_ln_f8(const float* w, const float* b, const float* gamma, const float* beta, int rows, int dim,
                             float scale, void* w8, float* wscale, float* c, float* d, hipStream_t stream);
hipError_t launch_fold_ln(const float* w, const float* b, const float* gamma, const float* beta, int rows, int dim,
                          float scale, void* w16, float* c, float* d, int dtype, hipStream_t stream);
hipError_t launch_dense_layer(const float* w, const float* b, const float* x, float* y, int n_in,
                              int n_out, int n_vec, int activation, hipStream_t stream, float* z = nullptr);
hipError_t launch_mlp_out_delta(const float* a, const float* z, const float* t, float* d, int64_t n, int act, float* err,
                                hipStream_t stream);
hipError_t launch_mlp_back_delta(const float* w, const float* d, const float* z_prev, float* d_prev, int n_in, int n_out,
                                 int n_sets, int act, hipStream_t stream);
hipError_t launch_mlp_update(float* w, float* b, const float* d, const float* x, int n_in, int n_out, int n_sets, float scale,
                             hipStream_t stream);

hipError_t launch_filter3x3(const uint8_t* in, uint8_t* out, int h, int w, int kind, hipStream_t stream);

constexpr int kMaxDevices = 64;
inline int env_int(const char* name, int dflt) {
    const char* e = getenv(name);
    return e ? atoi(e) : dflt;
}
inline int device_num_cu() {
    static std::atomic<int> table[kMaxDevices];
    int dev = 0;
    if (hipGetDevice(&dev) != hipSuccess || dev < 0 || dev >= kMaxDevices) return 0;
    int n = table[dev].load(std::memory_order_relaxed);
    if (n) return n;
    if (hipDeviceGetAttribute(&n, hipDeviceAttributeMultiprocessorCount, dev) != hipSuccess || n <= 0) return 0;
    table[dev].store(n, std::memory_order_relaxed);
    return n;
}
using LdsDone = std::atomic<int>[kMaxDevices];
inline hipError_t ensure_dynamic_lds(const void* kernel, size_t bytes, LdsDone& done) {
    int dev = 0;
    hipError_t e = hipGetDevice(&dev);
    if (e != hipSuccess) return e;
    if (dev < 0 || dev >= kMaxDevices) return hipErrorInvalidDevice;
    if ((size_t)done[dev].load(std::memory_order_acquire) >= bytes) return hipSuccess;
    e = hipFuncSetAttribute(kernel, hipFuncAttributeMaxDynamicSharedMemorySize, (int)bytes);
    if (e == hipSuccess) done[dev].store((int)bytes, std::memory_order_release);
    return e;
}

}
```

### vit-fpga_amd/csrc/vithip_api.hip

```cpp
#include <dlfcn.h>

#include <chrono>
#include <cmath>
#include <condition_variable>
#include <cstdarg>
#include <cstdio>
#include <cstdlib>
#include <cstring>
#include <functional>
#include <memory>
#include <mutex>
#include <string>
#include <thread>
#include <vector>

#include "vh_kernels.h"

using namespace vh;

namespace {

thread_local std::string g_err;

int fail(std::string* ctx_err, int code, const char* fmt, ...) {
// ... 152 lines not shown
    float* partials = nullptr;
    bool split = false;
    bool cls_tail = false;
    int head_dim = 64;
    float q_scale = kAttnQScale;
    bool patch_fused = false;
    void* xlo16 = nullptr;
    bool ln_fold_cfg = false, split_cfg = false;
    unsigned int* guard_dev = nullptr;
    float* guard_host = nullptr;
    float guard_thresh = 0.5f;
    bool guard_auto = false, guard_tripped = false;
    char* arena = nullptr;
    unsigned int* tickets = nullptr;
    float* x = nullptr;
    void* xn16 = nullptr;
    void* qkv16 = nullptr;
    void* att16 = nullptr;
    void* h16 = nullptr;
    void* col16 = nullptr;
    float* clsn32 = nullptr;
    float* in_dev = nullptr;
    float in_scale[kMaxChannels], in_shift[kMaxChannels];
    float* logits_dev = nullptr;
    uint8_t* rz_u8 = nullptr;
    uint32_t *rz_plan_dev = nullptr, *rz_plan_host = nullptr;
    size_t rz_plan_dev_cap = 0, rz_plan_host_cap = 0;
    uint8_t* rz_frames = nullptr;
    size_t rz_frames_cap = 0;
    std::vector<uint32_t> rz_words;
    float nv12_m[12];
    int nv12_site = VH_CHROMA_LEFT;
    int64_t last_us = 0;
    bool timed = false;
    int last_batch = 0;
    struct RingSlot {
        float *h_in = nullptr, *h_out = nullptr, *d_in = nullptr, *d_out = nullptr;
        hipEvent_t in_done = nullptr, fwd_done = nullptr, out_done = nullptr;
        int batch = 0;
        uint32_t* h_plan = nullptr;
        size_t plan_cap = 0;
    };
    std::vector<RingSlot> ring;
    enum RingKind { RING_F32, RING_U8, RING_FRAMES };
    RingKind ring_kind = RING_F32;
    size_t ring_slot_bytes = 0;
    hipStream_t copy_in = nullptr, copy_out = nullptr;
    int ring_batch = 0, ring_wr = 0, ring_rd = 0, ring_used = 0;
    hipStream_t tstream = nullptr;
    hipEvent_t ev_tail_a = nullptr, ev_tail_l = nullptr;
    bool tail_overlap = false;
    bool last_h_tiled = false;
    bool last_qkv_hm = false;
    int tail_splits = 0;
    int num_cu = 256;
    bool use_graph = false;
    struct GraphEntry { ImgIn in; float* out; int batch; hipGraph_t graph; hipGraphExec_t exec; };
    std::vector<GraphEntry> graphs;
    std::vector<int> graph_warm;
    int timing_stage = -1;
    std::vector<hipEvent_t> tev;
    size_t tev_used = 0;
    bool step_timing = false;
    std::vector<hipEvent_t> sev;
    size_t sev_used = 0;
    std::string err;
};

struct vh_filter {
    int device, height, width, kind;
    struct Slot {
        uint8_t *h_in = nullptr, *h_out = nullptr, *d_in = nullptr, *d_out = nullptr;
        hipEvent_t in_done = nullptr, k_done = nullptr, out_done = nullptr;
    };
    std::vector<Slot> slot;
    hipStream_t copy_in = nullptr, compute = nullptr, copy_out = nullptr;
    int wr = 0, rd = 0, used = 0;
    std::string err;
};

struct vh_mlp {
    int device, n_ins, n_layers, activation;
    std::vector<int> npl;
    size_t n_params = 0, n_neurons = 0;
    int widest = 0, max_vec = 0;
    hipStream_t stream = nullptr;
    float *params = nullptr, *bias = nullptr, *buf0 = nullptr, *buf1 = nullptr;
    bool loaded = false;
    int64_t last_us = 0;
    int n_sets = 0;
    float *set_ins = nullptr, *set_outs = nullptr, *tz = nullptr, *ta = nullptr, *td = nullptr, *terr = nullptr;
    int64_t last_gradient_us = 0;
    std::string err;
};

namespace {

size_t align_up(size_t v, size_t a) { return (v + a - 1) / a * a; }

int set_device(std::string* err, int device) {
    int n = 0;
    hipError_t e = hipGetDeviceCount(&n);
    if (e != hipSuccess || n <= 0) return fail(err, VH_ERR_NO_DEVICE, "no HIP device visible (%s)", hipGetErrorString(e));
    if (device < 0 || device >= n) return fail(err, VH_ERR_INVALID, "device %d out of range (0..%d)", device, n - 1);
    HIPCHK(err, hipSetDevice(device));
    return VH_OK;
// ... 87 lines not shown
    c->split = c->split_cfg;
    drop_graphs(c);
    return VH_OK;
}

int check_blob_header(vh_ctx* c, const BlobHeader& h) {
    const vh_config& f = c->cfg;
    if (memcmp(h.magic, "VHBLOB1", 8) != 0) return fail(&c->err, VH_ERR_INVALID, "weight blob: bad magic");
    if (h.image_size != f.image_size || h.patch_size != f.patch_size || h.channels != f.channels || h.dim != f.dim ||
        h.heads != f.heads || h.mlp_dim != f.mlp_dim || h.layers != f.layers || h.classes != f.classes)
        return fail(&c->err, VH_ERR_INVALID, "weight blob: shape differs from the context's vh_config");
    const uint32_t want = blob_model_bits(f);
    if ((h.flags ^ want) & kBlobPreLn)
        return fail(&c->err, VH_ERR_INVALID, "weight blob: header bit 1 (pre-LayerNorm) is %d, the context's VH_FLAG_PRE_LN is %d",
                    (h.flags & kBlobPreLn) != 0, (want & kBlobPreLn) != 0);
    if ((h.flags ^ want) & kBlobQuickGelu)
        return fail(&c->err, VH_ERR_INVALID, "weight blob: header bit 2 (QuickGELU) is %d, the context's VH_FLAG_QUICK_GELU is %d",
                    (h.flags & kBlobQuickGelu) != 0, (want & kBlobQuickGelu) != 0);
    return VH_OK;
}

int enqueue_forward(vh_ctx* c, ImgIn in, int batch, float* logits, std::vector<std::pair<int, hipEvent_t>>* ev,
                    hipStream_t s, int img0, bool allow_tail = false, bool may_pad = true) {
    const vh_config& f = c->cfg;
    const Layout& L = c->L;
    const int D = f.dim, M = f.mlp_dim, T = L.T;
    const int64_t rows = (int64_t)batch * T;
    const int64_t row_tiles = (rows + 255) / 256;
    const int64_t rows_g = (may_pad && c->ln_fold && row_tiles * ((D + 255) / 256) >= 2 * (int64_t)c->num_cu) ? row_tiles * 256 : rows;
    const float* P = c->params;
    const size_t r0 = (size_t)img0 * T, esz = 2, esz_op = c->fp8 ? 1 : 2;
    const int dt16 = c->dt16;
    float* const x = c->x + r0 * D;
    float* const stats_p = c->stats + r0 * 2;
    float* const partials_p = c->partials + (size_t)(D / 64) * r0 * 2;
    char* const xn16 = (char*)c->xn16 + r0 * D * esz_op;
    char* const xlo16 = (char*)c->xlo16 + r0 * D * (c->fp8 ? 2 : 1);
    char* const qkv16 = (char*)c->qkv16 + r0 * 3 * D * esz;
    char* const att16 = (char*)c->att16 + r0 * D * esz_op;
    char* const h16 = (char*)c->h16 + r0 * M * esz_op;
    char* const col16 = (char*)c->col16 + (size_t)img0 * L.NP * L.KPA * esz;
    float* const clsn32 = c->clsn32 + (size_t)img0 * D;
    unsigned int* const tickets_part = c->tickets + (size_t)img0 * (f.layers > 0 ? f.layers : 1);
    if (f.layers > 0) HIPCHK(&c->err, hipMemsetAsync(tickets_part, 0, sizeof(unsigned int) * f.layers, s));
    unsigned int* const amax_guard = c->fp8 ? c->guard_dev + 1 : nullptr;
    auto mark = [&](int stage) -> int {
        if (!ev) return VH_OK;
        hipEvent_t e;
        HIPCHK(&c->err, hipEventCreate(&e));
        HIPCHK(&c->err, hipEventRecord(e, s));
        ev->push_back({stage, e});
        return VH_OK;
    };
    auto gemm = [&](const void* a, const void* w, const float* bias, void* out, int64_t Mr, int N, int K, int epi,
                    const float* aux, int aux_i, const float* wscale = nullptr) {
        GemmArgs g{a, w, bias, out, Mr, N, K, epi, aux, aux_i, dt16, 0};
        g.stats = stats_p;
        g.out16 = epi == VH_EPI_RESID_SPLIT ? xlo16 : xn16;
        g.partials = partials_p;
        if (wscale) {
            g.dtype = VH_DTYPE_FP8;
            if (epi == VH_EPI_LNFOLD || epi == VH_EPI_LNFOLD_GELU || epi == VH_EPI_LNFOLD_QGELU) g.wscale = wscale;
            else g.aux = wscale;
            return launch_gemm_fp8(g, s);
        }
        return launch_gemm(g, s);
    };
    auto tmark = [&](int stage) -> int {
        if (stage != c->timing_stage) return VH_OK;
        if (c->tev_used == c->tev.size()) {
            hipEvent_t e;
            HIPCHK(&c->err, hipEventCreate(&e));
            c->tev.push_back(e);
        }
        HIPCHK(&c->err, hipEventRecord(c->tev[c->tev_used++], s));
        return VH_OK;
    };
    int rc;
    if (img0 == 0) c->tail_splits = 0;
    if ((rc = mark(-1))) return rc;
    const int nl = (c->run_layers < 0 || c->run_layers > f.layers) ? f.layers : c->run_layers;
    const bool pre_ln = (f.flags & VH_FLAG_PRE_LN) != 0;
    const int epi_fc1 = (f.flags & VH_FLAG_QUICK_GELU) ? VH_EPI_LNFOLD_QGELU : VH_EPI_LNFOLD_GELU;
    const int epi_fc1_plain = (f.flags & VH_FLAG_QUICK_GELU) ? VH_EPI_BIAS_QGELU : VH_EPI_BIAS_GELU;
    const bool fused_patch = !in.u8 && !pre_ln && c->patch_fused && c->split && !c->fp8 && nl > 0 && patch_fused_supported(f.image_size, f.patch_size, f.channels, D);
    if (!fused_patch) {
        if ((rc = tmark(ST_IM2COL))) return rc;
        if (in.u8)
            HIPCHK(&c->err, launch_im2col_u8((const uint8_t*)in.p, batch, f.image_size, f.patch_size, f.channels, L.KPA, c->in_scale, c->in_shift,
                                             col16, dt16, s));
        else
            HIPCHK(&c->err, launch_im2col((const float*)in.p, batch, f.image_size, f.patch_size, f.channels, L.KPA, col16, dt16, s));
        if ((rc = tmark(ST_IM2COL))) return rc;
    }
    if ((rc = mark(ST_IM2COL))) return rc;
    if (fused_patch) {
        if ((rc = tmark(ST_PATCH))) return rc;
        HIPCHK(&c->err, launch_patch_fused((const float*)in.p, batch, f.image_size, f.patch_size, f.channels, c->wp16, P + L.patch_b, P + L.pos, xn16, xlo16,
                                           partials_p, rows_g, D, dt16, s));
        if ((rc = tmark(ST_PATCH))) return rc;
        if ((rc = mark(ST_PATCH))) return rc;
        HIPCHK(&c->err, launch_cls_rows_split(xn16, xlo16, partials_p, rows_g, P + L.cls, P + L.pos, batch, T, D, dt16, s));
        if ((rc = mark(ST_CLS))) return rc;
        HIPCHK(&c->err, launch_finalize_stats(partials_p, D / 64, rows_g, D, f.ln_eps, stats_p, s, rows, c->guard_dev, amax_guard));
        if ((rc = mark(ST_LNSTATS))) return rc;
    } else if (c->split && !c->fp8 && nl > 0 && !pre_ln) {
        GemmArgs g{col16, c->wp16, P + L.patch_b, xn16, (int64_t)batch * L.NP, D, L.KPA, VH_EPI_PATCH_SPLIT, P + L.pos, L.NP, dt16, 0};
        g.out16 = xlo16; g.partials = partials_p; g.prow = rows_g;
        if ((rc = tmark(ST_PATCH))) return rc;
        HIPCHK(&c->err, launch_gemm(g, s));
        if ((rc = tmark(ST_PATCH))) return rc;
        if ((rc = mark(ST_PATCH))) return rc;
        HIPCHK(&c->err, launch_cls_rows_split(xn16, xlo16, partials_p, rows_g, P + L.cls, P + L.pos, batch, T, D, dt16, s));
        if ((rc = mark(ST_CLS))) return rc;
        HIPCHK(&c->err, launch_finalize_stats(partials_p, D / 64, rows_g, D, f.ln_eps, stats_p, s, rows, c->guard_dev, amax_guard));
        if ((rc = mark(ST_LNSTATS))) return rc;
    } else {
        if ((rc = tmark(ST_PATCH))) return rc;
        HIPCHK(&c->err, gemm(col16, c->wp16, P + L.patch_b, x, (int64_t)batch * L.NP, D, L.KPA, VH_EPI_PATCH, P + L.pos, L.NP));
        if ((rc = tmark(ST_PATCH))) return rc;
        if ((rc = mark(ST_PATCH))) return rc;
        HIPCHK(&c->err, launch_cls_rows(x, P + L.cls, P + L.pos, batch, T, D, s));
        if ((rc = mark(ST_CLS))) return rc;
        if (pre_ln) {
            const bool fold0 = c->ln_fold && nl > 0;
            if ((rc = tmark(ST_PRELN))) return rc;
            HIPCHK(&c->err, launch_pre_layernorm(x, fold0 ? rows_g : rows, D, P + L.prew, P + L.preb, f.ln_eps, fold0 && c->split ? nullptr : x,
                                                 fold0 ? xn16 : nullptr, fold0 && c->split ? xlo16 : nullptr, fold0 ? stats_p : nullptr,
                                                 c->fp8 ? VH_DTYPE_FP8 : dt16, s, rows, fold0 ? c->guard_dev : nullptr, fold0 ? amax_guard : nullptr));
            if ((rc = tmark(ST_PRELN))) return rc;
            if ((rc = mark(ST_PRELN))) return rc;
        } else if (c->ln_fold && nl > 0) {
            if (c->split) HIPCHK(&c->err, launch_rowstats_split(x, rows_g, D, f.ln_eps, xn16, xlo16, stats_p, c->fp8 ? VH_DTYPE_FP8 : dt16, s, rows, amax_guard));
            else HIPCHK(&c->err, launch_rowstats_cast(x, rows_g, D, f.ln_eps, xn16, stats_p, c->fp8 ? VH_DTYPE_FP8 : dt16, s, rows, amax_guard));
            HIPCHK(&c->err, launch_ln_guard(stats_p, rows, c->guard_dev, s));
            if ((rc = mark(ST_LNSTATS))) return rc;
        }
    }
    const bool hd64 = c->head_dim == 64;
    const bool tail = c->cls_tail && hd64 && c->ln_fold && c->split && !c->fp8 && nl == f.layers && c->run_layers < 0 && T <= 1024 &&
                      (size_t)L.NP * L.KPA * esz >= 2 * ((size_t)D * esz + 256);
    const bool h_tiled = c->h_tiled && c->split && !c->fp8 && c->weights_ready_tiled && gemm_tiled_applies(rows_g, M, D) && gemm_tiled_applies(rows_g, D, M);
    const bool h_tiled8 = c->h_tiled && c->split && c->fp8 && c->weights_ready_tiled && gemm_tiled_applies_f8(rows_g, M, D) && gemm_tiled_applies_f8(rows_g, D, M);
    const bool att_tiled = hd64 && h_tiled && c->att_tiled && gemm_tiled_applies(rows_g, D, D) && attention_tiled_applies(batch, T, f.heads) && !tail;
    const bool att_tiled8 = hd64 && h_tiled8 && c->att_tiled && gemm_tiled_applies_f8(rows_g, D, D) && attention_tiled_applies(batch, T, f.heads);
    const bool qkv_hm = hd64 && c->qkv_hm && ((att_tiled && gemm_tiled_applies(rows_g, 3 * D, D)) || (att_tiled8 && gemm_tiled_applies_f8(rows_g, 3 * D, D)));
    c->last_h_tiled = (h_tiled || h_tiled8) && nl > 0 && c->ln_fold;
    c->last_qkv_hm = qkv_hm && nl > 0 && c->ln_fold;
    for (int l = 0; l < nl && c->ln_fold; ++l) {
        const LayerOff& o = L.layer[l];
        const float* cd = c->fold_cd + (size_t)l * (6 * D + 2 * M);
        const int nblk = D / 64;
        if ((rc = tmark(ST_QKV))) return rc;
        const float *sq = c->fp8 ? c->sqkv[l] : nullptr, *so = c->fp8 ? c->so[l] : nullptr;
        const float *s1 = c->fp8 ? c->s1[l] : nullptr, *s2 = c->fp8 ? c->s2[l] : nullptr;
        if (qkv_hm) {
            GemmArgs gq{xn16, c->wqkv16[l], cd + 3 * D, qkv16, rows_g, 3 * D, D, VH_EPI_LNFOLD, cd, 0, c->fp8 ? VH_DTYPE_FP8 : dt16, 0};
            gq.stats = stats_p; gq.out_tiled = 1; gq.wscale = sq;
            HIPCHK(&c->err, c->fp8 ? launch_gemm_fp8(gq, s) : launch_gemm(gq, s));
        } else
        HIPCHK(&c->err, gemm(xn16, c->wqkv16[l], cd + 3 * D, qkv16, rows_g, 3 * D, D, VH_EPI_LNFOLD, cd, 0, sq));
        if ((rc = tmark(ST_QKV))) return rc;
        if ((rc = mark(ST_QKV))) return rc;
        if (tail && l + 1 == nl) {
            char* const hc = col16;
            char* const lc = col16 + (((size_t)batch * D * esz + 255) & ~(size_t)255);
            HIPCHK(&c->err, launch_attention_cls(qkv16, batch, T, f.heads, att16, dt16, s));
            if ((rc = mark(ST_ATTN))) return rc;
            HIPCHK(&c->err, hipMemcpy2DAsync(hc, (size_t)D * esz, xn16, (size_t)T * D * esz, (size_t)D * esz, batch, hipMemcpyDeviceToDevice, s));
            HIPCHK(&c->err, hipMemcpy2DAsync(lc, (size_t)D, xlo16, (size_t)T * D, (size_t)D, batch, hipMemcpyDeviceToDevice, s));
            GemmArgs gp{att16, c->wo16[l], P + o.ob, hc, batch, D, D, VH_EPI_RESID_SPLIT, nullptr, 0, dt16, 0};
            gp.out16 = lc; gp.partials = partials_p;
            HIPCHK(&c->err, launch_gemm(gp, s));
            if ((rc = mark(ST_PROJ))) return rc;
            HIPCHK(&c->err, launch_finalize_stats(partials_p, nblk, batch, D, f.ln_eps, stats_p, s, batch, c->guard_dev));
            if ((rc = mark(ST_LNSTATS))) return rc;
            GemmArgs g1{hc, c->w1_16[l], cd + 6 * D + M, h16, batch, M, D, epi_fc1, cd + 6 * D, 0, dt16, 0};
            g1.stats = stats_p;
            HIPCHK(&c->err, launch_gemm(g1, s));
            if ((rc = mark(ST_FC1))) return rc;
            GemmArgs g2{h16, c->w2_16[l], P + o.f2b, hc, batch, D, M, VH_EPI_RESID_SPLIT, nullptr, 0, dt16, 0};
            g2.out16 = lc; g2.partials = partials_p;
            HIPCHK(&c->err, launch_gemm(g2, s));
            if ((rc = mark(ST_FC2))) return rc;
            HIPCHK(&c->err, launch_layernorm_split(hc, lc, batch, D, D, P + L.lnfw, P + L.lnfb, f.ln_eps, clsn32, dt16, s));
            if ((rc = mark(ST_LNF))) return rc;
            HIPCHK(&c->err, launch_head_f32(clsn32, P + L.headw, P + L.headb, logits, batch, f.classes, D, s));
            if ((rc = mark(ST_HEAD))) return rc;
            c->last_batch = batch;
            return VH_OK;
        }
        if ((rc = tmark(ST_ATTN))) return rc;
        if (hd64)
            HIPCHK(&c->err, launch_attention(qkv16, batch, T, f.heads, att16, c->fp8 ? VH_DTYPE_FP8 : dt16, tickets_part + l, s, true, att_tiled || att_tiled8,
                                             qkv_hm ? (int64_t)rows_g : 0));
        else
            HIPCHK(&c->err, launch_attention_hd(qkv16, batch, T, f.heads, c->head_dim, att16, c->fp8 ? VH_DTYPE_FP8 : dt16, s));
        if ((rc = tmark(ST_ATTN))) return rc;
        if ((rc = mark(ST_ATTN))) return rc;
        if ((rc = tmark(ST_PROJ))) return rc;
        if (att_tiled) {
            GemmArgs go{att16, c->wot_16[l], P + o.ob, xn16, rows_g, D, D, VH_EPI_RESID_SPLIT, nullptr, 0, dt16, 0};
            go.out16 = xlo16; go.partials = partials_p; go.ab_tiled = 1;
            HIPCHK(&c->err, launch_gemm(go, s));
        } else if (att_tiled8) {
            GemmArgs go{att16, c->wot_16[l], P + o.ob, xn16, rows_g, D, D, VH_EPI_RESID_SPLIT, so, 0, VH_DTYPE_FP8, 0};
            go.out16 = xlo16; go.partials = partials_p; go.ab_tiled = 1;
            HIPCHK(&c->err, launch_gemm_fp8(go, s));
        } else
        if (c->split) HIPCHK(&c->err, gemm(att16, c->wo16[l], P + o.ob, xn16, rows_g, D, D, VH_EPI_RESID_SPLIT, nullptr, 0, so));
        else HIPCHK(&c->err, gemm(att16, c->wo16[l], P + o.ob, x, rows_g, D, D, VH_EPI_RESID_LN, nullptr, 0, so));
        if ((rc = tmark(ST_PROJ))) return rc;
        if ((rc = mark(ST_PROJ))) return rc;
        HIPCHK(&c->err, launch_finalize_stats(partials_p, nblk, rows_g, D, f.ln_eps, stats_p, s, rows, c->guard_dev, amax_guard));
        if ((rc = mark(ST_LNSTATS))) return rc;
        if ((rc = tmark(ST_FC1))) return rc;
        if (h_tiled) {
            GemmArgs g1{xn16, c->w1_16[l], cd + 6 * D + M, h16, rows_g, M, D, epi_fc1, cd + 6 * D, 0, dt16, 0};
            g1.stats = stats_p; g1.out_tiled = 1;
            HIPCHK(&c->err, launch_gemm(g1, s));
        } else if (h_tiled8) {
            GemmArgs g1{xn16, c->w1_16[l], cd + 6 * D + M, h16, rows_g, M, D, epi_fc1, cd + 6 * D, 0, VH_DTYPE_FP8, 0};
            g1.stats = stats_p; g1.wscale = s1; g1.out_tiled = 1;
            HIPCHK(&c->err, launch_gemm_fp8(g1, s));
        } else
        HIPCHK(&c->err, gemm(xn16, c->w1_16[l], cd + 6 * D + M, h16, rows_g, M, D, epi_fc1, cd + 6 * D, 0, s1));
        if ((rc = tmark(ST_FC1))) return rc;
        if ((rc = mark(ST_FC1))) return rc;
        if ((rc = tmark(ST_FC2))) return rc;
        if (h_tiled) {
            GemmArgs g2{h16, c->w2t_16[l], P + o.f2b, xn16, rows_g, D, M, VH_EPI_RESID_SPLIT, nullptr, 0, dt16, 0};
            g2.out16 = xlo16; g2.partials = partials_p; g2.ab_tiled = 1;
            HIPCHK(&c->err, launch_gemm(g2, s));
        } else if (h_tiled8) {
            GemmArgs g2{h16, c->w2t_16[l], P + o.f2b, xn16, rows_g, D, M, VH_EPI_RESID_SPLIT, s2, 0, VH_DTYPE_FP8, 0};
            g2.out16 = xlo16; g2.partials = partials_p; g2.ab_tiled = 1;
            HIPCHK(&c->err, launch_gemm_fp8(g2, s));
        } else
        if (c->split) HIPCHK(&c->err, gemm(h16, c->w2_16[l], P + o.f2b, xn16, rows_g, D, M, VH_EPI_RESID_SPLIT, nullptr, 0, s2));
        else HIPCHK(&c->err, gemm(h16, c->w2_16[l], P + o.f2b, x, rows_g, D, M, l + 1 < nl ? VH_EPI_RESID_LN : VH_EPI_BIAS_RESID, nullptr, 0, s2));
        if ((rc = tmark(ST_FC2))) return rc;
        if ((rc = mark(ST_FC2))) return rc;
        if (l + 1 < nl) {
            HIPCHK(&c->err, launch_finalize_stats(partials_p, nblk, rows_g, D, f.ln_eps, stats_p, s, rows, c->guard_dev, amax_guard));
            if ((rc = mark(ST_LNSTATS))) return rc;
        }
    }
    const bool plain = !c->ln_fold;
    const int op_dt = c->fp8 ? VH_DTYPE_FP8 : dt16;
    auto gemm_any = [&](const void* a, const void* w, const float* bias, const float* scale, void* out, int N, int K, int epi,
                        int tile_begin, int tile_count) {
        GemmArgs g{a, w, bias, out, rows, N, K, epi, c->fp8 ? scale : nullptr, 0, op_dt, 0};
        g.tile_begin = tile_begin;
        g.tile_count = tile_count;
        if ((tile_begin || tile_count) && !c->fp8) g.variant = gemm_pick_variant(rows, N, epi) == 7 ? 7 : 5;
        return c->fp8 ? launch_gemm_fp8(g, s) : launch_gemm(g, s);
    };
    auto ln_rows = [&](int64_t r_begin, int64_t r_count, const float* w, const float* b, hipStream_t st) {
        return launch_layernorm(x + r_begin * D, r_count, D, D, w, b, f.ln_eps, xn16 + r_begin * D * esz_op, op_dt, st);
    };
    auto resid_gemm_ln = [&](const void* a, const void* w, const float* bias, const float* scale, int K, const float* lnw,
                             const float* lnb, int st_gemm) -> int {
        const int tiles_n = (D + 255) / 256, ntile = (int)((rows + 255) / 256) * tiles_n;
        int split = 0;
        const bool pp = c->fp8 || gemm_pick_variant(rows, D, VH_EPI_BIAS_RESID) >= 5;
        if (allow_tail && c->tail_overlap && lnw && !ev && pp && ntile > c->num_cu && ntile % c->num_cu != 0 &&
            c->timing_stage != ST_LN && c->timing_stage != ST_PROJ && c->timing_stage != ST_FC2) {
            split = ntile / c->num_cu * c->num_cu;
            split -= split % tiles_n;
        }
        int r;
        if ((r = tmark(st_gemm))) return r;
        if (!split) {
            HIPCHK(&c->err, gemm_any(a, w, bias, scale, x, D, K, VH_EPI_BIAS_RESID, 0, 0));
            if ((r = tmark(st_gemm))) return r;
            if ((r = mark(st_gemm))) return r;
            if (!lnw) return VH_OK;
            if ((r = tmark(ST_LN))) return r;
            HIPCHK(&c->err, ln_rows(0, rows, lnw, lnb, s));
            if ((r = tmark(ST_LN))) return r;
            return mark(ST_LN);
        }
        ++c->tail_splits;
        const int64_t rows_a = (int64_t)(split / tiles_n) * 256;
        HIPCHK(&c->err, gemm_any(a, w, bias, scale, x, D, K, VH_EPI_BIAS_RESID, 0, split));
        HIPCHK(&c->err, hipEventRecord(c->ev_tail_a, s));
        HIPCHK(&c->err, gemm_any(a, w, bias, scale, x, D, K, VH_EPI_BIAS_RESID, split, ntile - split));
        HIPCHK(&c->err, hipStreamWaitEvent(c->tstream, c->ev_tail_a, 0));
        HIPCHK(&c->err, ln_rows(0, rows_a, lnw, lnb, c->tstream));
        HIPCHK(&c->err, hipEventRecord(c->ev_tail_l, c->tstream));
        HIPCHK(&c->err, ln_rows(rows_a, rows - rows_a, lnw, lnb, s));
        HIPCHK(&c->err, hipStreamWaitEvent(s, c->ev_tail_l, 0));
        return tmark(st_gemm);
    };
    if (plain && nl > 0) {
        const LayerOff& o0 = L.layer[0];
        if ((rc = tmark(ST_LN))) return rc;
        HIPCHK(&c->err, ln_rows(0, rows, P + o0.ln1w, P + o0.ln1b, s));
        if ((rc = tmark(ST_LN))) return rc;
        if ((rc = mark(ST_LN))) return rc;
    }
    for (int l = 0; l < nl && plain; ++l) {
        const LayerOff& o = L.layer[l];
        const float *sq = c->fp8 ? c->sqkv[l] : nullptr, *so = c->fp8 ? c->so[l] : nullptr;
        const float *s1 = c->fp8 ? c->s1[l] : nullptr, *s2 = c->fp8 ? c->s2[l] : nullptr;
        if ((rc = tmark(ST_QKV))) return rc;
        HIPCHK(&c->err, gemm_any(xn16, c->wqkv16[l], c->bqkv + (size_t)l * 3 * D, sq, qkv16, 3 * D, D, VH_EPI_BIAS, 0, 0));
        if ((rc = tmark(ST_QKV))) return rc;
        if ((rc = mark(ST_QKV))) return rc;
        if ((rc = tmark(ST_ATTN))) return rc;
        if (c->head_dim == 64) HIPCHK(&c->err, launch_attention(qkv16, batch, T, f.heads, att16, op_dt, tickets_part + l, s, true));
        else HIPCHK(&c->err, launch_attention_hd(qkv16, batch, T, f.heads, c->head_dim, att16, op_dt, s));
        if ((rc = tmark(ST_ATTN))) return rc;
        if ((rc = mark(ST_ATTN))) return rc;
        if ((rc = resid_gemm_ln(att16, c->wo16[l], P + o.ob, so, D, P + o.ln2w, P + o.ln2b, ST_PROJ))) return rc;
        if ((rc = tmark(ST_FC1))) return rc;
        HIPCHK(&c->err, gemm_any(xn16, c->w1_16[l], P + o.f1b, s1, h16, M, D, epi_fc1_plain, 0, 0));
        if ((rc = tmark(ST_FC1))) return rc;
        if ((rc = mark(ST_FC1))) return rc;
        const bool more = l + 1 < nl;
        if ((rc = resid_gemm_ln(h16, c->w2_16[l], P + o.f2b, s2, M, more ? P + L.layer[l + 1].ln1w : nullptr,
                                more ? P + L.layer[l + 1].ln1b : nullptr, ST_FC2))) return rc;
    }
    if (c->split && nl > 0)
        HIPCHK(&c->err, launch_layernorm_split(xn16, xlo16, batch, D, (int64_t)T * D, P + L.lnfw, P + L.lnfb, f.ln_eps, clsn32, c->fp8 ? VH_DTYPE_FP8 : dt16, s));
    else
        HIPCHK(&c->err, launch_layernorm(x, batch, D, (int64_t)T * D, P + L.lnfw, P + L.lnfb, f.ln_eps, clsn32, VH_DTYPE_F32_INTERNAL, s));
    if ((rc = mark(ST_LNF))) return rc;
    HIPCHK(&c->err, launch_head_f32(clsn32, P + L.headw, P + L.headb, logits, batch, f.classes, D, s));
    if ((rc = mark(ST_HEAD))) return rc;
    c->last_batch = batch;
    return VH_OK;
}

int guard_publish(vh_ctx* c) {
    if (c->ln_fold) HIPCHK(&c->err, hipMemcpyAsync(c->guard_host, c->guard_dev, 2 * sizeof(float), hipMemcpyDeviceToHost, c->stream));
    return VH_OK;
}
constexpr float kE4M3Max = 448.f;
bool guard_exceeded(const vh_ctx* c) {
    if (!c->ln_fold || !c->guard_host) return false;
    const volatile float* g = c->guard_host;
    return !(g[0] <= c->guard_thresh) || (c->fp8 && !(g[1] <= kE4M3Max));
}
int prepare_weights(vh_ctx* c);
void drop_graphs(vh_ctx* c);
int guard_poll(vh_ctx* c) {
    if (!guard_exceeded(c)) return VH_OK;
    c->guard_tripped = true;
    if (!c->guard_auto) return VH_OK;
    c->ln_fold = false;
    c->split = false;
    drop_graphs(c);
    return prepare_weights(c);
}

int enqueue_step(vh_ctx* c, ImgIn in, int batch, float* logits) {
    const size_t img_elems = (size_t)c->cfg.image_size * c->cfg.image_size * c->cfg.channels;
    const int parts = batch < c->nstreams ? batch : c->nstreams;
    int rc;
    if (parts > 1) {
        HIPCHK(&c->err, hipEventRecord(c->ev_fork, c->stream));
        int b0 = 0;
        for (int p = 0; p < parts; ++p) {
            const int nb = batch / parts + (p < batch % parts ? 1 : 0);
            hipStream_t st = p == 0 ? c->stream : c->xstream[p - 1];
            if (p) HIPCHK(&c->err, hipStreamWaitEvent(st, c->ev_fork, 0));
            if ((rc = enqueue_forward(c, in.skip((size_t)b0 * img_elems), nb, logits + (size_t)b0 * c->cfg.classes, nullptr, st, b0, false,
                                       p == parts - 1))) return rc;
            if (p) {
                HIPCHK(&c->err, hipEventRecord(c->ev_join[p - 1], st));
                HIPCHK(&c->err, hipStreamWaitEvent(c->stream, c->ev_join[p - 1], 0));
            }
            b0 += nb;
        }
        c->last_batch = batch;
        return guard_publish(c);
    }
// ... 313 lines not shown
        c->tail_overlap = e && e[0] == '1';
    }
    {
        const char* e = getenv("VH_GRAPH");
        c->use_graph = e && e[0] == '1';
    }
    CK(hipEventCreate(&c->ev0));
    CK(hipEventCreate(&c->ev1));
    CK(hipMalloc((void**)&c->blob, sizeof(BlobHeader) + 4 * L.total));
    c->params = (float*)(c->blob + sizeof(BlobHeader));
    size_t w16_bytes = 0;
    auto carve16 = [&](size_t elems) { size_t o = w16_bytes; w16_bytes += align_up(elems * 2, 256); return o; };
    const size_t o_wp = carve16(D * L.KPA);
    std::vector<size_t> o_qkv(cfg->layers), o_o(cfg->layers), o_1(cfg->layers), o_2(cfg->layers), o_2t(cfg->layers);
    const bool want_tiled_any = D % 256 == 0 && M % 256 == 0 && !(getenv("VH_H_TILED") && getenv("VH_H_TILED")[0] == '0');
    const bool want_tiled = cfg->dtype != VH_DTYPE_FP8 && want_tiled_any;
    const bool want_tiled8 = cfg->dtype == VH_DTYPE_FP8 && want_tiled_any;
    for (int l = 0; l < cfg->layers; ++l) {
        o_qkv[l] = carve16(3 * D * D); o_o[l] = carve16(D * D); o_1[l] = carve16(M * D); o_2[l] = carve16(D * M);
        o_2t[l] = want_tiled ? carve16(D * M) : want_tiled8 ? carve16((D * M + 1) / 2) : 0;
    }
    std::vector<size_t> o_ot(cfg->layers);
    for (int l = 0; l < cfg->layers; ++l) o_ot[l] = want_tiled ? carve16(D * D) : want_tiled8 ? carve16((D * D + 1) / 2) : 0;
    const size_t o_bqkv = w16_bytes;
    w16_bytes += align_up((size_t)cfg->layers * 3 * D * 4, 256);
    {
        const bool eligible = (cfg->dim % 256 == 0) && (cfg->mlp_dim % 256 == 0);
        bool want = true;
        if (cfg->flags & VH_FLAG_LN_FOLD_OFF) want = false;
        else if (!(cfg->flags & VH_FLAG_LN_FOLD_ON)) { const char* e = getenv("VH_LN_FOLD"); if (e) want = e[0] == '1'; }
        c->ln_fold = eligible && want;
        c->guard_auto = c->ln_fold && !(cfg->flags & (VH_FLAG_LN_FOLD_ON | VH_FLAG_LN_FOLD_OFF)) && !getenv("VH_LN_FOLD");
        if (const char* e = getenv("VH_LN_GUARD")) { const float t = (float)atof(e); if (t > 0.f) c->guard_thresh = t; }
    }
    c->fp8 = cfg->dtype == VH_DTYPE_FP8;
    c->dt16 = c->fp8 ? VH_DTYPE_BF16 : cfg->dtype;
    for (int i = 0; i < kMaxChannels; ++i) {
        c->in_scale[i] = i < cfg->channels ? 1.0f / 255.0f : 0.f;
        c->in_shift[i] = 0.f;
    }
    yuv_matrix(VH_YUV_BT709, 0, c->nv12_m);
    c->nv12_site = VH_CHROMA_LEFT;
    {
        const char* e = getenv("VH_RESID_SPLIT");
        c->split = c->ln_fold && !(e && e[0] == '0');
        c->ln_fold_cfg = c->ln_fold;
        c->split_cfg = c->split;
        c->cls_tail = (cfg->flags & VH_FLAG_CLS_TAIL) != 0;
        c->head_dim = cfg->dim / cfg->heads;
        c->q_scale = attention_q_scale(c->head_dim);
        c->h_tiled = want_tiled || want_tiled8;
        { const char* e = getenv("VH_ATT_TILED"); c->att_tiled = !(e && e[0] == '0'); }
        { const char* e = getenv("VH_QKV_HM"); c->qkv_hm = !(e && e[0] == '0'); }
        const char* pf = getenv("VH_PATCH_FUSED");
        c->patch_fused = pf && pf[0] == '1';
    }
    CK(hipHostMalloc((void**)&c->guard_host, 64, hipHostMallocDefault));
    *c->guard_host = 0.f;
    const size_t o_cd = w16_bytes;
    w16_bytes += align_up((size_t)cfg->layers * (6 * D + 2 * M) * 4, 256);
    const size_t o_sc = w16_bytes, sc_per_layer = 5 * D + M;
    if (c->fp8) w16_bytes += align_up((size_t)cfg->layers * sc_per_layer * 4, 256);
    CK(hipMalloc((void**)&c->w16, w16_bytes));
    c->wp16 = c->w16 + o_wp; c->bqkv = (float*)(c->w16 + o_bqkv);
    c->fold_cd = (float*)(c->w16 + o_cd);
    for (int l = 0; l < cfg->layers; ++l) {
        c->wqkv16.push_back(c->w16 + o_qkv[l]); c->wo16.push_back(c->w16 + o_o[l]);
        c->w1_16.push_back(c->w16 + o_1[l]); c->w2_16.push_back(c->w16 + o_2[l]);
        c->w2t_16.push_back(want_tiled || want_tiled8 ? c->w16 + o_2t[l] : nullptr);
        c->wot_16.push_back(want_tiled || want_tiled8 ? c->w16 + o_ot[l] : nullptr);
        if (c->fp8) {
            float* sc = (float*)(c->w16 + o_sc) + (size_t)l * sc_per_layer;
            c->sqkv.push_back(sc); c->so.push_back(sc + 3 * D); c->s1.push_back(sc + 4 * D); c->s2.push_back(sc + 4 * D + M);
        }
    }
    size_t a = 0;
    auto carve = [&](size_t bytes) { size_t o = a; a += align_up(bytes, 256); return o; };
    const size_t rows_p = rows + 256;
    const size_t o_x = carve(rows_p * D * 4), o_xn = carve(rows_p * D * 2), o_qkvA = carve(rows_p * 3 * D * 2),
                 o_att = carve(rows_p * D * 2), o_h = carve(rows_p * M * 2), o_col = carve(B * L.NP * (size_t)L.KPA * 2),
                 o_cls = carve(B * D * 4),
                 o_in = carve(B * (size_t)cfg->image_size * cfg->image_size * cfg->channels * 4), o_lg = carve(B * C * 4),
                 o_st = carve(rows_p * 2 * 4), o_pt = carve((D / 64 + 1) * rows_p * 2 * 4), o_xlo = carve(rows_p * D * 2),
                 o_tk = carve(B * 4 * (size_t)(cfg->layers > 0 ? cfg->layers : 1)),
                 o_gd = carve(256);
    CK(hipMalloc((void**)&c->arena, a));
    c->guard_dev = (unsigned int*)(c->arena + o_gd);
    CK(hipMemsetAsync(c->guard_dev, 0, 256, c->stream));
    c->x = (float*)(c->arena + o_x); c->xn16 = c->arena + o_xn; c->qkv16 = c->arena + o_qkvA; c->att16 = c->arena + o_att;
    c->h16 = c->arena + o_h; c->col16 = c->arena + o_col; c->clsn32 = (float*)(c->arena + o_cls);
    c->in_dev = (float*)(c->arena + o_in); c->logits_dev = (float*)(c->arena + o_lg);
    c->stats = (float*)(c->arena + o_st); c->partials = (float*)(c->arena + o_pt); c->xlo16 = c->arena + o_xlo;
    c->tickets = (unsigned int*)(c->arena + o_tk);
#undef CK
    *out = c;
    return VH_OK;
}

int vh_destroy(vh_ctx* c) {
    if (!c) return VH_OK;
    hipSetDevice(c->device);
    vh_ring_destroy(c);
    if (c->stream) hipStreamSynchronize(c->stream);
    drop_graphs(c);
    if (c->guard_host) hipHostFree(c->guard_host);
    if (c->rz_plan_host) hipHostFree(c->rz_plan_host);
// ... 661 lines not shown
}

int vh_set_step_timing(vh_ctx* c, int enable) {
    if (!c) return fail(nullptr, VH_ERR_INVALID, "null context");
    c->step_timing = enable != 0;
    c->sev_used = 0;
    return VH_OK;
}

int vh_get_step_timing(vh_ctx* c, double* step_ms, int max_steps, int* steps) {
    if (!c || !steps || (max_steps > 0 && !step_ms)) return fail(c ? &c->err : nullptr, VH_ERR_INVALID, "null argument");
    HIPCHK(&c->err, hipSetDevice(c->device));
    HIPCHK(&c->err, hipStreamSynchronize(c->stream));
    int n = 0;
    for (size_t i = 0; i + 1 < c->sev_used; ++i) {
        float t = 0.f;
        HIPCHK(&c->err, hipEventElapsedTime(&t, c->sev[i], c->sev[i + 1]));
        if (n < max_steps) step_ms[n] = t;
        ++n;
    }
    *steps = n;
    return VH_OK;
}

int vh_debug_read(vh_ctx* c, int what, float* host_out, size_t n_floats) {
    if (!c || !host_out) return fail(c ? &c->err : nullptr, VH_ERR_INVALID, "null argument");
    if (c->last_batch <= 0) return fail(&c->err, VH_ERR_STATE, "no forward has run");
    HIPCHK(&c->err, hipSetDevice(c->device));
    HIPCHK(&c->err, hipStreamSynchronize(c->stream));
    const size_t D = c->cfg.dim;
    if (what == 0) {
        const size_t n = (size_t)c->last_batch * c->L.T * D;
        if (n_floats != n) return fail(&c->err, VH_ERR_INVALID, "expected %zu floats", n);
        const int nl = (c->run_layers < 0 || c->run_layers > c->cfg.layers) ? c->cfg.layers : c->run_layers;
        if (c->split && nl > 0) {
            auto f = [&](uint16_t b, int dt) {
                if (dt == VH_DTYPE_BF16) { uint32_t u = (uint32_t)b << 16; float v; memcpy(&v, &u, 4); return v; }
                _Float16 hv; memcpy(&hv, &b, 2); return (float)hv;
            };
            auto g = [&](uint8_t b) {
                const int e = (b >> 3) & 15, m = b & 7;
                float v = e ? ldexpf(1.f + m / 8.f, e - 7) : ldexpf(m / 8.f, -6);
                return (b & 0x80) ? -v : v;
            };
            if (c->fp8) {
                std::vector<uint8_t> hi(n);
                std::vector<uint16_t> lo(n);
                HIPCHK(&c->err, hipMemcpy(hi.data(), c->xn16, n, hipMemcpyDeviceToHost));
                HIPCHK(&c->err, hipMemcpy(lo.data(), c->xlo16, n * 2, hipMemcpyDeviceToHost));
                for (size_t i = 0; i < n; ++i) host_out[i] = g(hi[i]) + f(lo[i], VH_DTYPE_BF16);
                return VH_OK;
            }
            std::vector<uint16_t> hi(n);
            std::vector<uint8_t> lo(n);
            HIPCHK(&c->err, hipMemcpy(hi.data(), c->xn16, n * 2, hipMemcpyDeviceToHost));
            HIPCHK(&c->err, hipMemcpy(lo.data(), c->xlo16, n, hipMemcpyDeviceToHost));
            const float inv = c->dt16 == VH_DTYPE_BF16 ? 1.f / 32.f : 1.f / 256.f;
            for (size_t i = 0; i < n; ++i) host_out[i] = f(hi[i], c->dt16) + g(lo[i]) * inv;
            return VH_OK;
        }
        HIPCHK(&c->err, hipMemcpy(host_out, c->x, n * 4, hipMemcpyDeviceToHost));
        return VH_OK;
    }
    if (what == 1) {
        const size_t n = (size_t)c->last_batch * D;
        if (n_floats != n) return fail(&c->err, VH_ERR_INVALID, "expected %zu floats", n);
        HIPCHK(&c->err, hipMemcpy(host_out, c->clsn32, n * 4, hipMemcpyDeviceToHost));
        return VH_OK;
    }
    if (what == 2) {
        if (n_floats != 1) return fail(&c->err, VH_ERR_INVALID, "expected 1 float");
        host_out[0] = (float)c->tail_splits;
        return VH_OK;
    }
    if (what == 3) {
        if (n_floats != 1) return fail(&c->err, VH_ERR_INVALID, "expected 1 float");
        host_out[0] = c->last_h_tiled ? 1.f : 0.f;
        return VH_OK;
    }
    if (what == 4) {
        if (n_floats != 1) return fail(&c->err, VH_ERR_INVALID, "expected 1 float");
        host_out[0] = c->last_qkv_hm ? 1.f : 0.f;
        return VH_OK;
    }
    return fail(&c->err, VH_ERR_INVALID, "unknown tap %d", what);
}

int vh_debug_set_layers(vh_ctx* c, int n_layers) {
    if (!c) return fail(nullptr, VH_ERR_INVALID, "null context");
    c->run_layers = n_layers;
    if (c->stream) hipStreamSynchronize(c->stream);
    drop_graphs(c);
    return VH_OK;
}

#define OPCHK(expr) do { hipError_t e_ = (expr); if (e_ != hipSuccess) return fail(nullptr, VH_ERR_HIP, "%s failed: %s", #expr, hipGetErrorString(e_)); } while (0)

int vh_op_gemm(const void* a, const void* w, const float* bias, void* out, int64_t M, int N, int K, int epi,
               const float* aux, int aux_i, int dtype, int variant, void* stream) {
    GemmArgs g{a, w, bias, out, M, N, K, epi, aux, aux_i, dtype, variant};
    if (const char* why = gemm_check(g)) return fail(nullptr, VH_ERR_INVALID, "%s", why);
    OPCHK(launch_gemm(g, (hipStream_t)stream));
    OPCHK(hipStreamSynchronize((hipStream_t)stream));
    return VH_OK;
}
int vh_op_gemm_fp8(const void* a8, const void* w8, const float* w_scale, const float* bias, void* out, int64_t M, int N, int K,
                   int epi, int variant, void* stream) {
    if (variant != 0 && variant != 5 && variant != 6 && variant != 7) return fail(nullptr, VH_ERR_INVALID, "gemm_fp8: variant must be 0, 5, 6 or 7");
    if (!a8 || !w8 || !w_scale || !bias || !out) return fail(nullptr, VH_ERR_INVALID, "gemm_fp8: null pointer");
    if (M <= 0 || N <= 0 || K <= 0 || K % 128 || N % 4) return fail(nullptr, VH_ERR_INVALID, "gemm_fp8: need K %% 128 == 0 and N %% 4 == 0");
    if (M > 0x7FFFFFFF / 2) return fail(nullptr, VH_ERR_INVALID, "gemm_fp8: M too large");
    if (epi != VH_EPI_BIAS && epi != VH_EPI_BIAS_GELU && epi != VH_EPI_BIAS_QGELU && epi != VH_EPI_BIAS_RESID && epi != VH_EPI_BIAS_F32)
        return fail(nullptr, VH_ERR_UNSUPPORTED, "gemm_fp8: epilogue %d not available", epi);
    GemmArgs g{a8, w8, bias, out, M, N, K, epi, w_scale, 0, VH_DTYPE_FP8, variant};
    OPCHK(launch_gemm_fp8(g, (hipStream_t)stream));
    OPCHK(hipStreamSynchronize((hipStream_t)stream));
    return VH_OK;
}
int vh_op_gemm_fp8_ex(const void* a8, const void* w8, const float* w_scale, const float* bias, void* out, int64_t M, int N, int K,
                      int epi, const float* c_dev, const float* stats, void* out16, float* partials, int variant, void* stream) {
    if (variant != 0 && variant != 5 && variant != 6 && variant != 7) return fail(nullptr, VH_ERR_INVALID, "gemm_fp8_ex: variant must be 0, 5, 6 or 7");
    if (!a8 || !w8 || !w_scale || !bias || !out) return fail(nullptr, VH_ERR_INVALID, "gemm_fp8_ex: null pointer");
    if (M <= 0 || N <= 0 || K <= 0 || K % 128 || N % 4) return fail(nullptr, VH_ERR_INVALID, "gemm_fp8_ex: need K %% 128 == 0 and N %% 4 == 0");
    if (M > 0x7FFFFFFF / 2) return fail(nullptr, VH_ERR_INVALID, "gemm_fp8_ex: M too large");
    const bool fold_act = epi == VH_EPI_LNFOLD_GELU || epi == VH_EPI_LNFOLD_QGELU;
    const bool fold = epi == VH_EPI_LNFOLD || fold_act, resid = epi == VH_EPI_RESID_LN || epi == VH_EPI_RESID_SPLIT;
    if (!fold && !resid) return fail(nullptr, VH_ERR_UNSUPPORTED, "gemm_fp8_ex: epilogue %d not available", epi);
    if (fold && (!c_dev || !stats)) return fail(nullptr, VH_ERR_INVALID, "gemm_fp8_ex: LNFOLD needs c and stats");
    if (resid && (!out16 || !partials)) return fail(nullptr, VH_ERR_INVALID, "gemm_fp8_ex: RESID_* needs out16 and partials");
    if ((resid || fold_act) && N % 256) return fail(nullptr, VH_ERR_INVALID, "gemm_fp8_ex: N %% 256 != 0");
    GemmArgs g{a8, w8, bias, out, M, N, K, epi, fold ? c_dev : w_scale, 0, VH_DTYPE_FP8, variant};
    if (fold) g.wscale = w_scale;
    g.stats = stats; g.out16 = out16; g.partials = partials;
    OPCHK(launch_gemm_fp8(g, (hipStream_t)stream));
    OPCHK(hipStreamSynchronize((hipStream_t)stream));
    return VH_OK;
}
int vh_op_quantize_rows(const float* w, int rows, int cols, float post_scale, void* w8, float* scale, void* stream) {
    if (!w || !w8 || !scale || rows <= 0 || cols <= 0 || cols % 4) return fail(nullptr, VH_ERR_INVALID, "quantize_rows: bad argument");
    OPCHK(launch_quantize_rows(w, rows, cols, post_scale, w8, scale, (hipStream_t)stream));
    OPCHK(hipStreamSynchronize((hipStream_t)stream));
    return VH_OK;
}
int vh_op_gemm_ex(const void* a, const void* w, const float* bias, void* out, int64_t M, int N, int K, int epi,
                  const float* aux, int aux_i, const float* stats, void* out16, float* partials, int dtype, int variant,
                  void* stream) {
    GemmArgs g{a, w, bias, out, M, N, K, epi, aux, aux_i, dtype, variant};
    g.stats = stats; g.out16 = out16; g.partials = partials;
    if (const char* why = gemm_check(g)) return fail(nullptr, VH_ERR_INVALID, "%s", why);
    OPCHK(launch_gemm(g, (hipStream_t)stream));
    OPCHK(hipStreamSynchronize((hipStream_t)stream));
    return VH_OK;
}
int vh_op_rowstats_cast(const float* x, int64_t rows, int dim, float eps, void* x16, float* stats, int dtype, void* stream) {
    if (!x || !x16 || !stats || rows <= 0 || dim <= 0 || dim % 4 || dim > 2048) return fail(nullptr, VH_ERR_INVALID, "rowstats_cast: bad argument");
    OPCHK(launch_rowstats_cast(x, rows, dim, eps, x16, stats, dtype, (hipStream_t)stream));
    OPCHK(hipStreamSynchronize((hipStream_t)stream));
    return VH_OK;
}
int vh_op_rowstats_split(const float* x, int64_t rows, int dim, float eps, void* hi, void* lo, float* stats, int dtype, void* stream) {
    if (!x || !hi || !lo || !stats || rows <= 0 || dim <= 0 || dim % 4 || dim > 2048) return fail(nullptr, VH_ERR_INVALID, "rowstats_split: bad argument");
    OPCHK(launch_rowstats_split(x, rows, dim, eps, hi, lo, stats, dtype, (hipStream_t)stream));
    OPCHK(hipStreamSynchronize((hipStream_t)stream));
    return VH_OK;
}
int vh_op_pre_layernorm(const float* x, int64_t rows, int dim, const float* gamma, const float* beta, float eps, float* y32, void* hi,
                        void* lo, float* stats, int dtype, void* stream) {
    if (!x || !gamma || !beta) return fail(nullptr, VH_ERR_INVALID, "pre_layernorm: null pointer");
    if (!y32 && !hi) return fail(nullptr, VH_ERR_INVALID, "pre_layernorm: one of y32 / hi is needed");
    if (lo && !hi) return fail(nullptr, VH_ERR_INVALID, "pre_layernorm: the lo plane needs the hi plane");
    if (rows <= 0 || dim <= 0 || dim % 4 || dim > 2048) return fail(nullptr, VH_ERR_INVALID, "pre_layernorm: need rows > 0, dim %% 4 == 0, dim <= 2048");
    if (!(eps > 0.f)) return fail(nullptr, VH_ERR_INVALID, "pre_layernorm: eps must be positive");
    if (dtype != VH_DTYPE_BF16 && dtype != VH_DTYPE_FP16 && dtype != VH_DTYPE_FP8) return fail(nullptr, VH_ERR_INVALID, "pre_layernorm: dtype");
    OPCHK(launch_pre_layernorm(x, rows, dim, gamma, beta, eps, y32, hi, lo, stats, dtype, (hipStream_t)stream));
    OPCHK(hipStreamSynchronize((hipStream_t)stream));
    return VH_OK;
}
int vh_op_finalize_stats(const float* partials, int nblk, int64_t rows, int dim, float eps, float* stats, void* stream) {
    if (!partials || !stats || nblk <= 0 || rows <= 0 || dim <= 0) return fail(nullptr, VH_ERR_INVALID, "finalize_stats: bad argument");
    OPCHK(launch_finalize_stats(partials, nblk, rows, dim, eps, stats, (hipStream_t)stream));
    OPCHK(hipStreamSynchronize((hipStream_t)stream));
    return VH_OK;
}
int vh_op_fold_ln(const float* w, const float* b, const float* gamma, const float* beta, int rows, int dim, float scale,
                  void* w16, float* c, float* d, int dtype, void* stream) {
    if (!w || !b || !gamma || !beta || !w16 || !c || !d || rows <= 0 || dim <= 0) return fail(nullptr, VH_ERR_INVALID, "fold_ln: bad argument");
    OPCHK(launch_fold_ln(w, b, gamma, beta, rows, dim, scale, w16, c, d, dtype, (hipStream_t)stream));
    OPCHK(hipStreamSynchronize((hipStream_t)stream));
    return VH_OK;
}
int vh_op_layernorm(const float* x, int64_t rows, int dim, int64_t row_stride, const float* gamma, const float* beta,
                    float eps, void* out16, int dtype, void* stream) {
    if (!x || !gamma || !beta || !out16) return fail(nullptr, VH_ERR_INVALID, "null pointer");
    if (dim <= 0 || dim % 4 || dim > 2048 || rows <= 0 || row_stride % 4) return fail(nullptr, VH_ERR_INVALID, "layernorm: unsupported shape");
    OPCHK(launch_layernorm(x, rows, dim, row_stride, gamma, beta, eps, out16, dtype, (hipStream_t)stream));
    OPCHK(hipStreamSynchronize((hipStream_t)stream));
    return VH_OK;
}
int vh_op_attention(const void* qkv16, int batch, int tokens, int heads, void* out16, int dtype, void* stream) {
    if (!qkv16 || !out16) return fail(nullptr, VH_ERR_INVALID, "null pointer");
    if (batch <= 0 || tokens <= 0 || heads <= 0 || tokens > kAttnStreamMaxTokens ||
// ... 734 lines not shown
```

### vit-fpga_amd/python/vithip.py

```python
from __future__ import annotations

import ctypes as C
import os

import numpy as np

_HERE = os.path.dirname(os.path.abspath(__file__))
PKG_ROOT = os.path.dirname(_HERE)
REPO_ROOT = os.path.dirname(PKG_ROOT)
LIB_PATH = os.environ.get("VITHIP_LIB") or os.path.join(PKG_ROOT, "libvithip.so")

DTYPE_BF16, DTYPE_FP16, DTYPE_FP8 = 0, 1, 2
FLAG_LN_FOLD_OFF, FLAG_LN_FOLD_ON, FLAG_W8_E4M3, FLAG_CLS_TAIL = 1, 2, 4, 8
FLAG_PRE_LN, FLAG_QUICK_GELU = 16, 32
EPI_BIAS, EPI_BIAS_GELU, EPI_BIAS_RESID, EPI_BIAS_F32, EPI_PATCH, EPI_LNFOLD, EPI_LNFOLD_GELU, EPI_RESID_LN, EPI_RESID_SPLIT, EPI_PATCH_SPLIT = range(10)
EPI_BIAS_QGELU, EPI_LNFOLD_QGELU = 10, 11
ACT_IDENTITY, ACT_RELU2, ACT_RELU, ACT_HARDTANH, ACT_GELU = range(5)

STAGES = ["im2col", "patch_gemm", "cls_rows", "layernorm", "qkv_gemm", "attention", "proj_gemm",
          "fc1_gemm", "fc2_gemm", "final_layernorm", "head_gemm", "ln_stats", "pre_layernorm"]
STAGE_RESIZE = "resize"
TIMED_STAGES = STAGES + [STAGE_RESIZE]


# ... 57 lines not shown
    "vh_forward_device_u8_async": (_i, [_vp, _vp, _i, _vp, _i]),
    "vh_resize_table": (_i, [_i, C.c_double, C.c_double, _i, _vp, _vp, _vp, _i]),
    "vh_forward_frames_u8": (_i, [_vp, _vp, _sz, _vp, _i, _vp]),
    "vh_forward_device_frames_u8": (_i, [_vp, _vp, _sz, _vp, _i, _vp]),
    "vh_yuv_matrix": (_i, [_i, _i, _vp]),
    "vh_set_frame_colour": (_i, [_vp, _vp, _i]),
    "vh_get_frame_colour": (_i, [_vp, _vp, _pi]),
    "vh_forward_frames_nv12": (_i, [_vp, _vp, _sz, _vp, _i, _vp]),
    "vh_forward_device_frames_nv12": (_i, [_vp, _vp, _sz, _vp, _i, _vp]),
    "vh_fill_input_seeded": (_i, [_vp, _u64, _i, _vp]),
    "vh_last_forward_us": (_i, [_vp, C.POINTER(_i64)]),
    "vh_last_kernel_ms": (_i, [_vp, C.POINTER(C.c_double)]),
    "vh_profile_forward": (_i, [_vp, _vp, _i, _vp, C.POINTER(C.c_double), _i, _pi]),
    "vh_stage_name": (C.c_char_p, [_i]),
    "vh_filter_create": (_i, [_i, _i, _i, _i, _i, C.POINTER(C.c_void_p)]),
    "vh_filter_destroy": (_i, [_vp]),
    "vh_filter_free_slots": (_i, [_vp, _pi]),
    "vh_filter_submit": (_i, [_vp, _vp]),
    "vh_filter_collect": (_i, [_vp, _vp]),
    "vh_filter_last_error": (C.c_char_p, [_vp]),
    "vh_device_mem_info": (_i, [_i, C.POINTER(C.c_size_t), C.POINTER(C.c_size_t)]),
    "vh_blob_file_config": (_i, [C.c_char_p, C.POINTER(Config)]),
    "vh_blob_file_read": (_i, [C.c_char_p, _vp, _sz]),
    "vh_save_weights_file": (_i, [_vp, C.c_char_p]),
    "vh_load_weights_file": (_i, [_vp, C.c_char_p]),
    "vh_ring_create": (_i, [_vp, _i, _i]),
    "vh_ring_destroy": (_i, [_vp]),
    "vh_ring_free_slots": (_i, [_vp, _pi]),
    "vh_ring_input": (_i, [_vp, C.POINTER(C.POINTER(C.c_float))]),
    "vh_ring_submit": (_i, [_vp, _vp, _i]),
    "vh_ring_collect": (_i, [_vp, _vp, _pi]),
    "vh_ring_create_u8": (_i, [_vp, _i, _i]),
    "vh_ring_input_u8": (_i, [_vp, C.POINTER(C.POINTER(C.c_uint8))]),
    "vh_ring_submit_u8": (_i, [_vp, _vp, _i]),
    "vh_ring_create_frames": (_i, [_vp, _i, _i, _sz]),
    "vh_ring_input_frames": (_i, [_vp, C.POINTER(C.POINTER(C.c_uint8)), C.POINTER(_sz)]),
    "vh_ring_submit_frames": (_i, [_vp, _vp, _sz, _vp, _i]),
    "vh_ring_submit_frames_nv12": (_i, [_vp, _vp, _sz, _vp, _i]),
    "vh_set_graph": (_i, [_vp, _i]),
    "vh_get_graph": (_i, [_vp, _pi, _pi]),
    "vh_set_streams": (_i, [_vp, _i]),
    "vh_get_streams": (_i, [_vp, _pi]),
    "vh_set_stage_timing": (_i, [_vp, _i]),
    "vh_get_stage_timing": (_i, [_vp, C.POINTER(C.c_double), C.POINTER(C.c_double), _pi]),
    "vh_set_step_timing": (_i, [_vp, _i]),
    "vh_get_step_timing": (_i, [_vp, C.POINTER(C.c_double), _i, _pi]),
    "vh_debug_read": (_i, [_vp, _i, _vp, _sz]),
    "vh_debug_set_layers": (_i, [_vp, _i]),
    "vh_op_gemm": (_i, [_vp, _vp, _vp, _vp, _i64, _i, _i, _i, _vp, _i, _i, _i, _vp]),
    "vh_op_gemm_fp8": (_i, [_vp, _vp, _vp, _vp, _vp, _i64, _i, _i, _i, _i, _vp]),
    "vh_op_gemm_fp8_ex": (_i, [_vp, _vp, _vp, _vp, _vp, _i64, _i, _i, _i, _vp, _vp, _vp, _vp, _i, _vp]),
    "vh_op_quantize_rows": (_i, [_vp, _i, _i, C.c_float, _vp, _vp, _vp]),
    "vh_op_gemm_ex": (_i, [_vp, _vp, _vp, _vp, _i64, _i, _i, _i, _vp, _i, _vp, _vp, _vp, _i, _i, _vp]),
    "vh_op_rowstats_cast": (_i, [_vp, _i64, _i, _f, _vp, _vp, _i, _vp]),
    "vh_op_finalize_stats": (_i, [_vp, _i, _i64, _i, _f, _vp, _vp]),
    "vh_op_pre_layernorm": (_i, [_vp, _i64, _i, _vp, _vp, _f, _vp, _vp, _vp, _vp, _i, _vp]),
    "vh_op_rowstats_split": (_i, [_vp, _i64, _i, _f, _vp, _vp, _vp, _i, _vp]),
    "vh_op_fold_ln": (_i, [_vp, _vp, _vp, _vp, _i, _i, _f, _vp, _vp, _vp, _i, _vp]),
    "vh_op_layernorm": (_i, [_vp, _i64, _i, _i64, _vp, _vp, _f, _vp, _i, _vp]),
    "vh_op_attention": (_i, [_vp, _i, _i, _i, _vp, _i, _vp]),
    "vh_op_attention_stream": (_i, [_vp, _i, _i, _i, _vp, _i, _vp]),
    "vh_op_attention_hd": (_i, [_vp, _i, _i, _i, _i, _vp, _i, _vp]),
    "vh_op_attention_cls": (_i, [_vp, _i, _i, _i, _vp, _i, _vp]),
    "vh_op_attention_layout": (_i, [_vp, _i, _i, _i, _vp, _i, _i, _i64, _vp]),
    "vh_op_im2col": (_i, [_vp, _i, _i, _i, _i, _vp, _i, _vp]),
    "vh_op_im2col_padded": (_i, [_vp, _i, _i, _i, _i, _i, _vp, _i, _vp]),
    "vh_op_im2col_u8": (_i, [_vp, _i, _i, _i, _i, _i, _vp, _vp, _vp, _i, _vp]),
    "vh_op_resize_u8": (_i, [_vp, _sz, _vp, _i, _i, _i, _vp, _vp]),
    "vh_op_resize_nv12": (_i, [_vp, _sz, _vp, _i, _i, _vp, _i, _vp, _vp]),
    "vh_op_cast": (_i, [_vp, _vp, _i64, _i, _vp]),
    "vh_op_fill": (_i, [_vp, _i64, _u64, C.c_uint32, _i, _f, _vp]),
    "vh_bench_gemm": (_i, [_i, _i64, _i, _i, _i, _i, _i, _i, C.POINTER(C.c_double)]),
    "vh_group_create": (_i, [C.POINTER(Config), _pi, _i, C.POINTER(_vp)]),
    "vh_group_destroy": (_i, [_vp]),
    "vh_group_size": (_i, [_vp, _pi]),
    "vh_group_member": (_i, [_vp, _i, C.POINTER(_vp), _pi]),
    "vh_group_last_error": (C.c_char_p, [_vp]),
    "vh_group_shard_bounds": (None, [_i, _i, _i, _pi, _pi]),
    "vh_group_load_weights": (_i, [_vp, _vp, _sz]),
    "vh_group_init_weights_seeded": (_i, [_vp, _u64]),
    "vh_group_broadcast_weights": (_i, [_vp]),
    "vh_group_forward": (_i, [_vp, _vp, _i, _vp]),
    "vh_group_fill_inputs_seeded": (_i, [_vp, _u64, _i]),
    "vh_group_forward_resident": (_i, [_vp, _i, _i]),
    "vh_group_read_logits": (_i, [_vp, _i, _vp]),
    "vh_mlp_create": (_i, [_i, _i, _i, _pi, _i, C.POINTER(_vp)]),
    "vh_mlp_load_params": (_i, [_vp, _vp, _sz, _vp, _sz]),
    "vh_mlp_forward": (_i, [_vp, _vp, _i, _vp]),
    "vh_mlp_last_forward_us": (_i, [_vp, C.POINTER(_i64)]),
    "vh_mlp_init_gradient": (_i, [_vp, _vp, _vp, _i]),
    "vh_mlp_launch_gradient": (_i, [_vp, _i, _f, _f, _vp]),
    "vh_mlp_read_params": (_i, [_vp, _vp, _sz, _vp, _sz]),
    "vh_mlp_last_gradient_us": (_i, [_vp, C.POINTER(_i64)]),
    "vh_mlp_last_error": (C.c_char_p, [_vp]),
    "vh_mlp_destroy": (_i, [_vp]),
}

_lib = None


def lib():
    global _lib
    if _lib is None:
        if not os.path.exists(LIB_PATH):
            raise ImportError(f"{LIB_PATH} not found: run `make -C vit-fpga_amd` (or "
                              "__graft_entry__.build()); there is no fallback path")
# ... 703 lines not shown
    _check(lib().vh_op_gemm_fp8(a8_ptr, w8_ptr, scale_ptr, bias_ptr, out_ptr, M, N, K, epilogue, variant, None))


def op_quantize_rows(w_ptr, rows, cols, post_scale, w8_ptr, scale_ptr):
    _check(lib().vh_op_quantize_rows(w_ptr, rows, cols, post_scale, w8_ptr, scale_ptr, None))


def op_gemm_fp8_ex(a8_ptr, w8_ptr, scale_ptr, bias_ptr, out_ptr, M, N, K, epilogue, c_ptr=None, stats_ptr=None, out16_ptr=None,
                   partials_ptr=None, variant=0):
    _check(lib().vh_op_gemm_fp8_ex(a8_ptr, w8_ptr, scale_ptr, bias_ptr, out_ptr, M, N, K, epilogue, c_ptr, stats_ptr, out16_ptr,
                                   partials_ptr, variant, None))


def e4m3_table():
    b = np.arange(256, dtype=np.uint32)
    e, m = (b >> 3) & 15, b & 7
    v = np.where(e == 0, m * 2.0 ** -9, (1 + m / 8.0) * 2.0 ** (e.astype(np.float64) - 7))
    v = np.where((e == 15) & (m == 7), np.nan, v)
    return np.where(b >> 7 == 1, -v, v).astype(np.float32)


def from_e4m3(b):
    return e4m3_table()[np.ascontiguousarray(b, dtype=np.uint8)]


def to_e4m3(x):
    x = np.ascontiguousarray(x, dtype=np.float32)
    pos = e4m3_table()[:127].astype(np.float64)
    a = np.minimum(np.abs(x).astype(np.float64), 448.0)
    hi = np.clip(np.searchsorted(pos, a, side="left"), 1, 126)
    lo = hi - 1
    dl, dh = a - pos[lo], pos[hi] - a
    code = np.where(dl < dh, lo, np.where(dh < dl, hi, np.where(lo % 2 == 0, lo, hi)))
    return (code | np.where(np.signbit(x), 0x80, 0)).astype(np.uint8)


LO8_SCALE = {DTYPE_BF16: 32.0, DTYPE_FP16: 256.0}


def to_lo8(residue, dtype):
    return to_e4m3(np.asarray(residue, dtype=np.float32) * np.float32(LO8_SCALE[dtype]))


def from_lo8(b, dtype):
    return from_e4m3(b) / np.float32(LO8_SCALE[dtype])


def op_gemm_ex(a_ptr, w_ptr, bias_ptr, out_ptr, M, N, K, epilogue, dtype, aux_ptr=None, aux_i=0, stats_ptr=None,
               out16_ptr=None, partials_ptr=None, variant=0):
    _check(lib().vh_op_gemm_ex(a_ptr, w_ptr, bias_ptr, out_ptr, M, N, K, epilogue, aux_ptr, aux_i, stats_ptr, out16_ptr,
                               partials_ptr, dtype, variant, None))


def op_rowstats_cast(x_ptr, rows, dim, eps, x16_ptr, stats_ptr, dtype):
    _check(lib().vh_op_rowstats_cast(x_ptr, rows, dim, eps, x16_ptr, stats_ptr, dtype, None))


def op_rowstats_split(x_ptr, rows, dim, eps, hi_ptr, lo_ptr, stats_ptr, dtype):
    _check(lib().vh_op_rowstats_split(x_ptr, rows, dim, eps, hi_ptr, lo_ptr, stats_ptr, dtype, None))


def op_pre_layernorm(x_ptr, rows, dim, gamma_ptr, beta_ptr, eps, y32_ptr, hi_ptr, lo_ptr, stats_ptr, dtype):
    _check(lib().vh_op_pre_layernorm(x_ptr, rows, dim, gamma_ptr, beta_ptr, eps, y32_ptr, hi_ptr, lo_ptr, stats_ptr, dtype, None))


def op_finalize_stats(partials_ptr, nblk, rows, dim, eps, stats_ptr):
    _check(lib().vh_op_finalize_stats(partials_ptr, nblk, rows, dim, eps, stats_ptr, None))


def op_fold_ln(w_ptr, b_ptr, gamma_ptr, beta_ptr, rows, dim, scale, w16_ptr, c_ptr, d_ptr, dtype):
    _check(lib().vh_op_fold_ln(w_ptr, b_ptr, gamma_ptr, beta_ptr, rows, dim, scale, w16_ptr, c_ptr, d_ptr, dtype, None))


def bench_gemm(M, N, K, epilogue, dtype=DTYPE_BF16, variant=0, iters=20, device=0):
    ms = C.c_double(0)
    _check(lib().vh_bench_gemm(device, M, N, K, epilogue, dtype, variant, iters, C.byref(ms)))
    return ms.value


def op_layernorm(x_ptr, rows, dim, row_stride, gamma_ptr, beta_ptr, eps, out_ptr, dtype):
    _check(lib().vh_op_layernorm(x_ptr, rows, dim, row_stride, gamma_ptr, beta_ptr, eps, out_ptr, dtype, None))


def op_attention(qkv_ptr, batch, tokens, heads, out_ptr, dtype):
    _check(lib().vh_op_attention(qkv_ptr, batch, tokens, heads, out_ptr, dtype, None))


def op_attention_stream(qkv_ptr, batch, tokens, heads, out_ptr, dtype):
    _check(lib().vh_op_attention_stream(qkv_ptr, batch, tokens, heads, out_ptr, dtype, None))


def op_attention_hd(qkv_ptr, batch, tokens, heads, head_dim, out_ptr, dtype):
    _check(lib().vh_op_attention_hd(qkv_ptr, batch, tokens, heads, head_dim, out_ptr, dtype, None))


def op_attention_cls(qkv_ptr, batch, tokens, heads, out_ptr, dtype):
    _check(lib().vh_op_attention_cls(qkv_ptr, batch, tokens, heads, out_ptr, dtype, None))


def op_attention_layout(qkv_ptr, batch, tokens, heads, out_ptr, dtype, out_tiled=False, in_hm_rows=0):
    _check(lib().vh_op_attention_layout(qkv_ptr, batch, tokens, heads, out_ptr, dtype, 1 if out_tiled else 0, in_hm_rows, None))


def op_im2col(in_ptr, batch, image, patch, channels, out_ptr, dtype):
    _check(lib().vh_op_im2col(in_ptr, batch, image, patch, channels, out_ptr, dtype, None))

# ... 33 lines not shown
```

Measured before the change: 28330 images/s.

## Store residual lo8 plane in 16-row blocked layout and coalesce LN partial writes

Introduces a blocked layout for the fp8 low-residue plane of the split residual stream, grouping 16 rows by 64 columns so each lane loads and stores 16 contiguous bytes covering two row groups instead of scattered 8-byte accesses. The RESID_SPLIT and PATCH_SPLIT epilogues, the CLS row writer, the final layernorm and the debug readback all learn the new addressing, and it is enabled by default through an environment flag. Separately, the per-row LayerNorm partial sums are gathered across eight passes so each lane writes one float2 together, instead of only lane 0 of each group writing. The aim is fewer, wider memory transactions in the residual epilogue, at the cost of extra template variants and a layout that every consumer of the lo plane must honor.

```diff
diff --git a/include/vithip.h b/include/vithip.h
--- a/include/vithip.h
+++ b/include/vithip.h
@@ -180,6 +180,11 @@
                   int64_t M, int N, int K, int epilogue, const float* aux_dev, int aux_i,
                   const float* stats_dev, void* out16_dev, float* partials_dev,
                   int dtype, int variant, void* stream);
+#define VH_GEMM_LO_BLOCKED 1u
+int vh_op_gemm_ex2(const void* a16_dev, const void* w16_dev, const float* bias_dev, void* out_dev,
+                   int64_t M, int N, int K, int epilogue, const float* aux_dev, int aux_i,
+                   const float* stats_dev, void* out16_dev, float* partials_dev,
+                   int dtype, int variant, unsigned int flags, void* stream);
 int vh_op_rowstats_cast(const float* x_dev, int64_t rows, int dim, float eps, void* x16_dev, float* stats_dev,
                         int dtype, void* stream);
 int vh_op_finalize_stats(const float* partials_dev, int nblk, int64_t rows, int dim, float eps, float* stats_dev,
diff --git a/vit-fpga_amd/csrc/gemm_epilogue.h b/vit-fpga_amd/csrc/gemm_epilogue.h
--- a/vit-fpga_amd/csrc/gemm_epilogue.h
+++ b/vit-fpga_amd/csrc/gemm_epilogue.h
@@ -6,6 +6,9 @@
 
 #ifndef VH_EPI_ABL
 #define VH_EPI_ABL 0
+#endif
+#ifndef VH_EPI_PCOAL
+#define VH_EPI_PCOAL 1
 #endif
 #ifndef VH_EPI_NT
 #define VH_EPI_NT 1
@@ -200,7 +203,7 @@
     asm volatile("" : "+v"(bv[0]), "+v"(bv[1]), "+v"(bv[2]), "+v"(bv[3]), "+v"(cv[0]), "+v"(cv[1]), "+v"(cv[2]), "+v"(cv[3]));
 }
 
-template <typename T, int EPI, int MI, int NI, int SMI = MI, bool MFULL = false, bool OTILED = false>
+template <typename T, int EPI, int MI, int NI, int SMI = MI, bool MFULL = false, bool OTILED = false, bool LOB = false>
 __device__ __forceinline__ void gemm_epilogue_staged(const f32x4 (&acc)[MI][NI], const EpiArgs& e, int m_w, int n_w,
                                                      int lane, char* sw, int prio_grp = -1, bool cpre = false) {
     static_assert(NI == 4, "staged epilogue assumes a 64-column wave tile");
@@ -385,6 +388,11 @@
         const int64_t prow = PATCHS ? e.prow : (int64_t)M;
         struct Add { vec8 h; u32x2 l; f32x4 p0, p1; };
         Add xa[2][NL];
+        static_assert(!LOB || PATCHS || (MFULL && NL % 2 == 0), "blocked lo plane of RESID_SPLIT: whole tiles, whole 16-row blocks per pass");
+        u32x4 xl[2][LOB && !PATCHS ? NL / 2 : 1];
+        u32x2 lkeep = u32x2{0u, 0u};
+        constexpr bool PCOAL = VH_EPI_PCOAL && !PATCHS && (MI * 2) % 8 == 0;
+        float2 pkeep = make_float2(0.f, 0.f);
         const int q0 = PATCHS ? m_w / e.aux_i : 0, r0 = PATCHS ? m_w - q0 * e.aux_i : 0;
         auto where = [&](int h, int i, int& m, int64_t& orow, int& p) {
             const int dr = h * FMI * 16 + i * 8 + rr;
@@ -400,7 +408,7 @@
             }
             return orow * N + n_w + 8 * pc;
         };
-        auto load_pass = [&](int h, Add (&a)[NL]) {
+        auto load_pass = [&](int h, Add (&a)[NL], u32x4 (&xlp)[LOB && !PATCHS ? NL / 2 : 1]) {
 #pragma unroll
             for (int i = 0; i < NL; ++i) {
                 int m, p;
@@ -410,16 +418,24 @@
                     const float* pr = e.aux + (int64_t)(1 + p) * N + n_w + 8 * pc;
                     a[i].p0 = *(const f32x4*)pr;
                     a[i].p1 = *(const f32x4*)(pr + 4);
+                } else if constexpr (LOB) {
+                    if constexpr (!(VH_EPI_ABL & 8)) {
+                        a[i].h = *(const vec8*)(hi + off);
+                        if ((i & 1) == 0) xlp[i >> 1] = *(const u32x4*)(lo + lo_blocked_offset(orow, n_w + 8 * pc, N));
+                    } else {
+                        a[i].h = vec8{};
+                        if ((i & 1) == 0) xlp[i >> 1] = u32x4{0u, 0u, 0u, 0u};
+                    }
                 } else {
                     if ((MFULL || m < M) && !(VH_EPI_ABL & 8)) { a[i].h = *(const vec8*)(hi + off); a[i].l = *(const u32x2*)(lo + off); }
                     else { a[i].h = vec8{}; a[i].l = u32x2{0u, 0u}; }
                 }
             }
         };
-        load_pass(0, xa[0]);
+        load_pass(0, xa[0], xl[0]);
 #pragma unroll
         for (int h = 0; h < NP; ++h) {
-            if (h + 1 < NP) load_pass(h + 1, xa[(h + 1) & 1]);
+            if (h + 1 < NP) load_pass(h + 1, xa[(h + 1) & 1], xl[(h + 1) & 1]);
 #pragma unroll
             for (int mi = 0; mi < FMI; ++mi) {
                 const int r = mi * 16 + frow;
@@ -441,7 +457,11 @@
                 vec8 hn;
                 float s1 = 0.f, s2 = 0.f;
                 f32x4 l0 = f32x4{0.f, 0.f, 0.f, 0.f}, l1 = l0;
-                if constexpr (!PATCHS) { l0 = lo8_unpack4<T>(a.l[0]); l1 = lo8_unpack4<T>(a.l[1]); }
+                if constexpr (!PATCHS && LOB) {
+                    const u32x4 lw = xl[h & 1][i >> 1];
+                    l0 = lo8_unpack4<T>(lw[(i & 1) * 2]);
+                    l1 = lo8_unpack4<T>(lw[(i & 1) * 2 + 1]);
+                } else if constexpr (!PATCHS) { l0 = lo8_unpack4<T>(a.l[0]); l1 = lo8_unpack4<T>(a.l[1]); }
 #pragma unroll
                 for (int j = 0; j < 8; ++j) {
                     const float add = PATCHS ? (j < 4 ? a.p0[j] : a.p1[j - 4]) : ((float)a.h[j] + (j < 4 ? l0[j] : l1[j - 4]));
@@ -451,14 +471,31 @@
                     s1 += v[j];
                     s2 = fmaf(v[j], v[j], s2);
                 }
-                if (ok && !(VH_EPI_ABL & 4)) {
+                const u32x2 lp{lo8_pack4<T>(ln[0], ln[1], ln[2], ln[3]), lo8_pack4<T>(ln[4], ln[5], ln[6], ln[7])};
+                if constexpr (LOB && !PATCHS) {
+                    if constexpr (!(VH_EPI_ABL & 4)) {
+                        *(vec8*)(hi + off) = hn;
+                        if ((i & 1) == 0) lkeep = lp;
+                        else *(u32x4*)(lo + lo_blocked_offset(orow - 8, n_w + 8 * pc, N)) = u32x4{lkeep[0], lkeep[1], lp[0], lp[1]};
+                    }
+                } else if (ok && !(VH_EPI_ABL & 4)) {
                     *(vec8*)(hi + off) = hn;
-                    *(u32x2*)(lo + off) = u32x2{lo8_pack4<T>(ln[0], ln[1], ln[2], ln[3]), lo8_pack4<T>(ln[4], ln[5], ln[6], ln[7])};
+                    if constexpr (LOB) *(u32x2*)(lo + lo_blocked_offset(orow, n_w + 8 * pc, N)) = lp;
+                    else *(u32x2*)(lo + off) = lp;
                 }
                 s1 += dpp_mov<0xB1>(s1); s2 += dpp_mov<0xB1>(s2);
                 s1 += dpp_mov<0x4E>(s1); s2 += dpp_mov<0x4E>(s2);
                 s1 += dpp_mov<0x141>(s1); s2 += dpp_mov<0x141>(s2);
-                if (ok && pc == 0 && !(VH_EPI_ABL & 1)) *(float2*)(e.partials + 2 * ((int64_t)(n_w >> 6) * prow + orow)) = make_float2(s1, s2);
+                if constexpr (PCOAL) {
+                    const int L = h * NL + i;
+                    if ((L & 7) == pc) pkeep = make_float2(s1, s2);
+                    if ((L & 7) == 7) {
+                        const int mk = m_w + (L - 7 + pc) * 8 + rr;
+                        if ((MFULL || mk < M) && !(VH_EPI_ABL & 1)) *(float2*)(e.partials + 2 * ((int64_t)(n_w >> 6) * prow + mk)) = pkeep;
+                    }
+                } else {
+                    if (ok && pc == 0 && !(VH_EPI_ABL & 1)) *(float2*)(e.partials + 2 * ((int64_t)(n_w >> 6) * prow + orow)) = make_float2(s1, s2);
+                }
             }
         }
     } else {
@@ -513,14 +550,14 @@
     }
 }
 
-template <typename T, int EPI, int MI, int NI, int SMI = MI, bool BARRIER = true>
+template <typename T, int EPI, int MI, int NI, int SMI = MI, bool BARRIER = true, bool LOB = false>
 __device__ __forceinline__ void gemm_epilogue(const f32x4 (&acc)[MI][NI], const EpiArgs& e, int m_w, int n_w, int lane,
                                               bool n_full, bool m_full, char* smem, int wave) {
     if constexpr (EPI != VH_EPI_PATCH) {
         if (EPI == VH_EPI_RESID_LN || EPI == VH_EPI_RESID_SPLIT || EPI == VH_EPI_PATCH_SPLIT || n_full) {
             if constexpr (BARRIER) __syncthreads();
             if (m_full && epi_is_16bit(EPI)) gemm_epilogue_staged<T, EPI, MI, NI, SMI, true>(acc, e, m_w, n_w, lane, smem + wave * (SMI * 16 * 128));
-            else gemm_epilogue_staged<T, EPI, MI, NI, SMI, false>(acc, e, m_w, n_w, lane, smem + wave * (SMI * 16 * 128));
+            else gemm_epilogue_staged<T, EPI, MI, NI, SMI, false, false, LOB>(acc, e, m_w, n_w, lane, smem + wave * (SMI * 16 * 128));
             return;
         }
     }
diff --git a/vit-fpga_amd/csrc/kernels_gemm.hip b/vit-fpga_amd/csrc/kernels_gemm.hip
--- a/vit-fpga_amd/csrc/kernels_gemm.hip
+++ b/vit-fpga_amd/csrc/kernels_gemm.hip
@@ -188,7 +188,8 @@
 hipError_t launch_gemm(const GemmArgs& g, hipStream_t s) {
     if (gemm_check(g)) return hipErrorInvalidValue;
     const int variant = g.variant ? g.variant : gemm_pick_variant(g.M, g.N, g.epilogue);
-    if ((g.out_tiled || g.ab_tiled) && variant != 6) return hipErrorInvalidValue;
+    if ((g.out_tiled || g.ab_tiled || g.lo_blocked) && variant != 6) return hipErrorInvalidValue;
+    if (g.lo_blocked && g.epilogue != VH_EPI_RESID_SPLIT && g.epilogue != VH_EPI_PATCH_SPLIT) return hipErrorInvalidValue;
     if ((g.tile_count || g.tile_begin) && variant != 5 && variant != 7) return hipErrorInvalidValue;
     return g.dtype == VH_DTYPE_BF16 ? launch_epi<BF16>(g, variant, s) : launch_epi<FP16>(g, variant, s);
 }
diff --git a/vit-fpga_amd/csrc/kernels_gemm5.hip b/vit-fpga_amd/csrc/kernels_gemm5.hip
--- a/vit-fpga_amd/csrc/kernels_gemm5.hip
+++ b/vit-fpga_amd/csrc/kernels_gemm5.hip
@@ -73,7 +73,7 @@
     return (xcd < rm ? xcd * (qd + 1) : rm * (qd + 1) + (xcd - rm) * qd) + (bid >> 3);
 }
 
-template <typename T, int EPI, bool PERSIST, bool F8 = false, int AST = 2, bool OT = false, bool AT = false>
+template <typename T, int EPI, bool PERSIST, bool F8 = false, int AST = 2, bool OT = false, bool AT = false, bool LB = false>
 __global__ void __launch_bounds__(512, 2)
 gemm_nt_pp_kernel(const void* __restrict__ Av, const void* __restrict__ Wv,
                   const float* __restrict__ bias, void* __restrict__ outp, int M, int N, int K,
@@ -402,14 +402,14 @@
             else if constexpr (F8 && (EPI == VH_EPI_RESID_LN || EPI == VH_EPI_RESID_SPLIT))
                 gemm_epilogue_staged<E4M3, EPI, MI, NI, VH_PP_SMI, true>(acc, e, m_w, n_w, lane_e, stage_epi + wave * SLICE);
             else
-                gemm_epilogue_staged<T, EPI, MI, NI, VH_PP_SMI, true, OT>(acc, e, m_w, n_w, lane_e, stage_epi + wave * SLICE, epi_is_16bit(EPI) ? grp : -1, cpre);
+                gemm_epilogue_staged<T, EPI, MI, NI, VH_PP_SMI, true, OT, LB>(acc, e, m_w, n_w, lane_e, stage_epi + wave * SLICE, epi_is_16bit(EPI) ? grp : -1, cpre);
         } else {
             if constexpr (F8 && epi_has_act(EPI))
                 gemm_epilogue8<EPI, MI, NI, VH_PP_SMI>(acc, e, m_w, n_w, lane_e, n_full, stage_epi, wave);
             else if constexpr (F8 && (EPI == VH_EPI_RESID_LN || EPI == VH_EPI_RESID_SPLIT))
                 gemm_epilogue<E4M3, EPI, MI, NI, 4, false>(acc, e, m_w, n_w, lane_e, n_full, m_full, stage_epi, wave);
             else
-                gemm_epilogue<T, EPI, MI, NI, (epi_is_16bit(EPI) ? VH_PP_SMI : 4), false>(acc, e, m_w, n_w, lane_e, n_full, m_full, stage_epi, wave);
+                gemm_epilogue<T, EPI, MI, NI, (epi_is_16bit(EPI) ? VH_PP_SMI : 4), false, LB>(acc, e, m_w, n_w, lane_e, n_full, m_full, stage_epi, wave);
         }
 #ifdef VH_DIAG_STAMPS
         if (first_tile_) VH_STAMP(3, diag_rt());
@@ -460,10 +460,11 @@
 #define VH_STAMP_ARG(g, epi, f8, grid, variant)
 #endif
 
-template <typename T, int EPI, bool F8, bool PERSIST, int AST, bool OT = false, bool AT = false>
+template <typename T, int EPI, bool F8, bool PERSIST, int AST, bool OT = false, bool AT = false, bool LB = false>
 static hipError_t launch_pp_one(const GemmArgs& g, int grid, int tiles_m, int tiles_n, hipStream_t s) {
     constexpr size_t lds = (AST == 3 || PERSIST) ? 163840 : 131072;
-    auto k = gemm_nt_pp_kernel<T, EPI, PERSIST, F8, AST, OT, AT>;
+    static_assert(!LB || (!F8 && ((PERSIST && EPI == VH_EPI_RESID_SPLIT) || EPI == VH_EPI_PATCH_SPLIT)), "blocked lo plane: RESID_SPLIT persistent, PATCH_SPLIT either form");
+    auto k = gemm_nt_pp_kernel<T, EPI, PERSIST, F8, AST, OT, AT, LB>;
     static LdsDone lds_done;
     if (hipError_t e = ensure_dynamic_lds((const void*)k, lds, lds_done); e != hipSuccess) return e;
     hipLaunchKernelGGL(k, dim3(grid), dim3(512), lds, s, g.a, g.w, g.bias, g.out, (int)g.M, g.N, g.K, g.aux, g.aux_i, tiles_m,
@@ -474,7 +475,13 @@
 }
 
 template <typename T, int EPI, bool F8>
-static hipError_t launch_pp(const GemmArgs& g, int mode, hipStream_t s) {
+static hipError_t launch_pp(const GemmArgs& g_in, int mode, hipStream_t s) {
+#ifdef VH_LO_FORCE
+    GemmArgs g = g_in;
+    if (!F8 && EPI == VH_EPI_RESID_SPLIT && mode == 1 && g.M % 256 == 0 && g.N % 256 == 0 && g.K >= 128) g.lo_blocked = 1;
+#else
+    const GemmArgs& g = g_in;
+#endif
     if constexpr (EPI == VH_EPI_PATCH) { if (mode == 1) mode = 0; }
     const int tiles_m = (int)((g.M + 255) / 256), tiles_n = (g.N + 255) / 256;
     int ntiles = tiles_m * tiles_n;
@@ -484,13 +491,30 @@
     } else if (g.tile_begin != 0) {
         return hipErrorInvalidValue;
     }
-    if (mode == 2) return launch_pp_one<T, EPI, F8, false, 3>(g, ntiles, tiles_m, tiles_n, s);
+    if constexpr (!F8 && EPI == VH_EPI_PATCH_SPLIT) {
+        if (g.lo_blocked) {
+            if (mode == 2 || g.out_tiled || g.ab_tiled || g.tile_count || g.tile_begin) return hipErrorInvalidValue;
+            const int full_m = (int)(g.M / 256);
+            if (mode == 1 && (g.N % 256 != 0 || full_m == 0 || g.K / 64 < 2 || (full_m != tiles_m && g.variant != 6))) mode = 0;
+            if (mode == 0) return launch_pp_one<T, EPI, F8, false, 2, false, false, true>(g, ntiles, tiles_m, tiles_n, s);
+            const int num_cu = device_num_cu();
+            if (!num_cu) return hipErrorUnknown;
+            const int nfull = full_m * tiles_n;
+            if (hipError_t e = launch_pp_one<T, EPI, F8, true, 2, false, false, true>(g, nfull < num_cu ? nfull : num_cu, full_m, tiles_n, s); e != hipSuccess) return e;
+            if (full_m == tiles_m) return hipSuccess;
+            GemmArgs tail = g;
+            tail.tile_begin = nfull;
+            tail.tile_count = tiles_n;
+            return launch_pp_one<T, EPI, F8, false, 2, false, false, true>(tail, tiles_n, tiles_m, tiles_n, s);
+        }
+    }
+    if (mode == 2) return g.lo_blocked ? hipErrorInvalidValue : launch_pp_one<T, EPI, F8, false, 3>(g, ntiles, tiles_m, tiles_n, s);
     if constexpr (EPI != VH_EPI_PATCH) {
         const int full_m = (int)(g.M / 256);
         const int nk = g.K / (F8 ? 128 : 64);
         if (mode == 1 && (g.N % 256 != 0 || full_m == 0 || nk < (pp_uses_cpre<EPI, F8>() ? 4 : 2))) mode = 0;
         if (mode == 1 && full_m != tiles_m && g.variant != 6) mode = 0;
-        if ((g.out_tiled || g.ab_tiled) && (mode != 1 || full_m != tiles_m)) return hipErrorInvalidValue;
+        if ((g.out_tiled || g.ab_tiled || g.lo_blocked) && (mode != 1 || full_m != tiles_m)) return hipErrorInvalidValue;
         if (mode == 1) {
             const int num_cu = device_num_cu();
             if (!num_cu) return hipErrorUnknown;
@@ -498,6 +522,14 @@
             if constexpr (epi_has_act(EPI) || EPI == VH_EPI_LNFOLD || (!F8 && EPI == VH_EPI_BIAS)) {
                 if (g.out_tiled) return g.ab_tiled ? hipErrorInvalidValue : launch_pp_one<T, EPI, F8, true, 2, true, false>(g, nfull < num_cu ? nfull : num_cu, full_m, tiles_n, s);
             }
+            if constexpr (!F8 && EPI == VH_EPI_RESID_SPLIT) {
+                if (g.lo_blocked) {
+                    if (g.out_tiled) return hipErrorInvalidValue;
+                    if (g.ab_tiled) return launch_pp_one<T, EPI, F8, true, 2, false, true, true>(g, nfull < num_cu ? nfull : num_cu, full_m, tiles_n, s);
+                    return launch_pp_one<T, EPI, F8, true, 2, false, false, true>(g, nfull < num_cu ? nfull : num_cu, full_m, tiles_n, s);
+                }
+            }
+            if (g.lo_blocked) return hipErrorInvalidValue;
             if constexpr (F8 ? EPI == VH_EPI_RESID_SPLIT : (EPI == VH_EPI_RESID_SPLIT || EPI == VH_EPI_BIAS)) {
                 if (g.ab_tiled) return g.out_tiled ? hipErrorInvalidValue : launch_pp_one<T, EPI, F8, true, 2, false, true>(g, nfull < num_cu ? nfull : num_cu, full_m, tiles_n, s);
             }
@@ -510,7 +542,7 @@
             return launch_pp_one<T, EPI, F8, false, 2>(tail, tiles_n, tiles_m, tiles_n, s);
         }
     }
-    if (g.out_tiled || g.ab_tiled) return hipErrorInvalidValue;
+    if (g.out_tiled || g.ab_tiled || g.lo_blocked) return hipErrorInvalidValue;
     return launch_pp_one<T, EPI, F8, false, 2>(g, ntiles, tiles_m, tiles_n, s);
 }
 
diff --git a/vit-fpga_amd/csrc/kernels_misc.hip b/vit-fpga_amd/csrc/kernels_misc.hip
--- a/vit-fpga_amd/csrc/kernels_misc.hip
+++ b/vit-fpga_amd/csrc/kernels_misc.hip
@@ -234,7 +234,7 @@
 template <typename T>
 __global__ void __launch_bounds__(256)
 cls_rows_split_kernel(typename T::elem* __restrict__ hi, uint8_t* __restrict__ lo, float* __restrict__ partials, int64_t prow,
-                      const float* __restrict__ cls, const float* __restrict__ pos, int batch, int tokens, int dim) {
+                      const float* __restrict__ cls, const float* __restrict__ pos, int batch, int tokens, int dim, int lo_blocked) {
     const int lane = threadIdx.x & 63;
     const int b = blockIdx.x * 4 + (threadIdx.x >> 6);
     if (b >= batch) return;
@@ -246,7 +246,7 @@
             v = cls[d] + pos[d];
             const typename T::elem h = (typename T::elem)v;
             hi[row * dim + d] = h;
-            lo[row * dim + d] = lo8_pack1<T>(v - (float)h);
+            lo[lo_blocked ? lo_blocked_offset(row, d, dim) : row * dim + d] = lo8_pack1<T>(v - (float)h);
         }
         float s1 = v, s2 = v * v;
 #pragma unroll
@@ -255,13 +255,13 @@
     }
 }
 hipError_t launch_cls_rows_split(void* hi, void* lo, float* partials, int64_t prow, const float* cls, const float* pos, int batch,
-                                 int tokens, int dim, int dtype, hipStream_t s) {
+                                 int tokens, int dim, int dtype, hipStream_t s, bool lo_blocked) {
     if (batch <= 0 || dim % 64) return hipErrorInvalidValue;
     const dim3 grid((unsigned)((batch + 3) / 4));
     if (dtype == VH_DTYPE_BF16)
-        hipLaunchKernelGGL(cls_rows_split_kernel<BF16>, grid, dim3(256), 0, s, (BF16::elem*)hi, (uint8_t*)lo, partials, prow, cls, pos, batch, tokens, dim);
+        hipLaunchKernelGGL(cls_rows_split_kernel<BF16>, grid, dim3(256), 0, s, (BF16::elem*)hi, (uint8_t*)lo, partials, prow, cls, pos, batch, tokens, dim, lo_blocked ? 1 : 0);
     else
-        hipLaunchKernelGGL(cls_rows_split_kernel<FP16>, grid, dim3(256), 0, s, (FP16::elem*)hi, (uint8_t*)lo, partials, prow, cls, pos, batch, tokens, dim);
+        hipLaunchKernelGGL(cls_rows_split_kernel<FP16>, grid, dim3(256), 0, s, (FP16::elem*)hi, (uint8_t*)lo, partials, prow, cls, pos, batch, tokens, dim, lo_blocked ? 1 : 0);
     return hipGetLastError();
 }
 
@@ -773,7 +773,7 @@
 __global__ void __launch_bounds__(256)
 layernorm_split_kernel(const typename T::elem* __restrict__ hi, const void* __restrict__ lo_, int64_t rows, int dim,
                        int64_t row_stride, const float* __restrict__ gamma, const float* __restrict__ beta, float eps,
-                       float* __restrict__ out) {
+                       float* __restrict__ out, int lo_blocked) {
     const int lane = threadIdx.x & 63;
     const int64_t row = (int64_t)blockIdx.x * 4 + (threadIdx.x >> 6);
     if (row >= rows) return;
@@ -781,6 +781,8 @@
     auto xk = [&](int k) {
         if constexpr (std::is_same<T, E4M3>::value)
             return __builtin_amdgcn_cvt_f32_fp8((int)hr[k], 0) + (float)((const typename BF16::elem*)lo_ + row * row_stride)[k];
+        else if (lo_blocked)
+            return (float)hr[k] + lo8_unpack1<T>(((const uint8_t*)lo_)[lo_blocked_offset(row * (row_stride / dim), k, dim)]);
         else
             return (float)hr[k] + lo8_unpack1<T>(((const uint8_t*)lo_ + row * row_stride)[k]);
     };
@@ -797,15 +799,17 @@
     for (int k = lane; k < dim; k += 64) out[row * dim + k] = ((xk(k)) - mean) * rstd * gamma[k] + beta[k];
 }
 hipError_t launch_layernorm_split(const void* hi, const void* lo, int64_t rows, int dim, int64_t row_stride, const float* gamma,
-                                  const float* beta, float eps, float* out32, int dtype, hipStream_t s) {
+                                  const float* beta, float eps, float* out32, int dtype, hipStream_t s, bool lo_blocked) {
     if (rows <= 0 || dim <= 0) return hipErrorInvalidValue;
+    if (lo_blocked && (dtype == VH_DTYPE_FP8 || dim % 64 || row_stride % dim)) return hipErrorInvalidValue;
+    const int lb = lo_blocked ? 1 : 0;
     const dim3 grid((unsigned)((rows + 3) / 4)), block(256);
     if (dtype == VH_DTYPE_FP8)
-        hipLaunchKernelGGL(layernorm_split_kernel<E4M3>, grid, block, 0, s, (const E4M3::elem*)hi, lo, rows, dim, row_stride, gamma, beta, eps, out32);
+        hipLaunchKernelGGL(layernorm_split_kernel<E4M3>, grid, block, 0, s, (const E4M3::elem*)hi, lo, rows, dim, row_stride, gamma, beta, eps, out32, lb);
     else if (dtype == VH_DTYPE_BF16)
-        hipLaunchKernelGGL(layernorm_split_kernel<BF16>, grid, block, 0, s, (const BF16::elem*)hi, (const void*)lo, rows, dim, row_stride, gamma, beta, eps, out32);
+        hipLaunchKernelGGL(layernorm_split_kernel<BF16>, grid, block, 0, s, (const BF16::elem*)hi, (const void*)lo, rows, dim, row_stride, gamma, beta, eps, out32, lb);
     else
-        hipLaunchKernelGGL(layernorm_split_kernel<FP16>, grid, block, 0, s, (const FP16::elem*)hi, (const void*)lo, rows, dim, row_stride, gamma, beta, eps, out32);
+        hipLaunchKernelGGL(layernorm_split_kernel<FP16>, grid, block, 0, s, (const FP16::elem*)hi, (const void*)lo, rows, dim, row_stride, gamma, beta, eps, out32, lb);
     return hipGetLastError();
 }
 
diff --git a/vit-fpga_amd/csrc/vh_common.h b/vit-fpga_amd/csrc/vh_common.h
--- a/vit-fpga_amd/csrc/vh_common.h
+++ b/vit-fpga_amd/csrc/vh_common.h
@@ -108,6 +108,9 @@
 }
 template <typename T>
 __device__ __forceinline__ float lo8_unpack1(uint8_t b) { return __builtin_amdgcn_cvt_f32_fp8((int)b, 0) * Lo8<T>::inv; }
+__host__ __device__ __forceinline__ int64_t lo_blocked_offset(int64_t r, int c, int N) {
+    return ((r >> 4) * (N >> 6) + (c >> 6)) * 1024 + (r & 7) * 128 + ((c >> 3) & 7) * 16 + ((r >> 3) & 1) * 8 + (c & 7);
+}
 
 __device__ __forceinline__ void asm_lds_dma16(const void* base, uint32_t lane_off, uint32_t lds_addr) {
     asm volatile("s_mov_b32 m0, %0\n\ts_nop 4\n\tglobal_load_lds_dwordx4 %1, %2"
diff --git a/vit-fpga_amd/csrc/vh_kernels.h b/vit-fpga_amd/csrc/vh_kernels.h
--- a/vit-fpga_amd/csrc/vh_kernels.h
+++ b/vit-fpga_amd/csrc/vh_kernels.h
@@ -27,6 +27,7 @@
     int tile_begin = 0, tile_count = 0;
     int64_t prow = 0;
     int out_tiled = 0, ab_tiled = 0;
+    int lo_blocked = 0;
 };
 bool gemm_tiled_applies(int64_t M, int N, int K);
 hipError_t launch_cast_tiled_w(const float* w, int rows, int cols, void* w16, int dtype, hipStream_t stream);
@@ -93,7 +94,7 @@
 hipError_t launch_cls_rows(float* x, const float* cls, const float* pos, int batch, int tokens,
                            int dim, hipStream_t stream);
 hipError_t launch_cls_rows_split(void* hi, void* lo, float* partials, int64_t prow, const float* cls, const float* pos, int batch,
-                                 int tokens, int dim, int dtype, hipStream_t stream);
+                                 int tokens, int dim, int dtype, hipStream_t stream, bool lo_blocked = false);
 hipError_t launch_cast(const float* in, void* out16, int64_t n, int dtype, hipStream_t stream);
 hipError_t launch_fill(float* out, int64_t n, uint64_t seed, uint32_t tensor_id, int kind,
                        float sigma, float offset, hipStream_t stream);
@@ -116,7 +117,7 @@
                                 void* hi, void* lo, float* stats, int dtype, hipStream_t stream, int64_t guard_rows = 0,
                                 unsigned int* guard = nullptr, unsigned int* amax_guard = nullptr);
 hipError_t launch_layernorm_split(const void* hi, const void* lo, int64_t rows, int dim, int64_t row_stride, const float* gamma,
-                                  const float* beta, float eps, float* out32, int dtype, hipStream_t stream);
+                                  const float* beta, float eps, float* out32, int dtype, hipStream_t stream, bool lo_blocked = false);
 hipError_t launch_fold_ln_f8(const float* w, const float* b, const float* gamma, const float* beta, int rows, int dim,
                              float scale, void* w8, float* wscale, float* c, float* d, hipStream_t stream);
 hipError_t launch_fold_ln(const float* w, const float* b, const float* gamma, const float* beta, int rows, int dim,
diff --git a/vit-fpga_amd/csrc/vithip_api.hip b/vit-fpga_amd/csrc/vithip_api.hip
--- a/vit-fpga_amd/csrc/vithip_api.hip
+++ b/vit-fpga_amd/csrc/vithip_api.hip
@@ -228,6 +228,10 @@
     bool tail_overlap = false;
     bool last_h_tiled = false;
     bool last_qkv_hm = false;
+    bool lo_blocked = true;
+    bool last_lo_blocked = false;
+    struct LoPart { int64_t row0, rows; bool blocked; };
+    std::vector<LoPart> lo_parts;
     int tail_splits = 0;
     int num_cu = 256;
     bool use_graph = false;
@@ -421,12 +425,14 @@
         ev->push_back({stage, e});
         return VH_OK;
     };
+    bool lo_blocked = false;
     auto gemm = [&](const void* a, const void* w, const float* bias, void* out, int64_t Mr, int N, int K, int epi,
                     const float* aux, int aux_i, const float* wscale = nullptr) {
         GemmArgs g{a, w, bias, out, Mr, N, K, epi, aux, aux_i, dt16, 0};
         g.stats = stats_p;
         g.out16 = epi == VH_EPI_RESID_SPLIT ? xlo16 : xn16;
         g.partials = partials_p;
+        g.lo_blocked = epi == VH_EPI_RESID_SPLIT && lo_blocked;
         if (wscale) {
             g.dtype = VH_DTYPE_FP8;
             if (epi == VH_EPI_LNFOLD || epi == VH_EPI_LNFOLD_GELU || epi == VH_EPI_LNFOLD_QGELU) g.wscale = wscale;
@@ -453,6 +459,12 @@
     const int epi_fc1 = (f.flags & VH_FLAG_QUICK_GELU) ? VH_EPI_LNFOLD_QGELU : VH_EPI_LNFOLD_GELU;
     const int epi_fc1_plain = (f.flags & VH_FLAG_QUICK_GELU) ? VH_EPI_BIAS_QGELU : VH_EPI_BIAS_GELU;
     const bool fused_patch = !in.u8 && !pre_ln && c->patch_fused && c->split && !c->fp8 && nl > 0 && patch_fused_supported(f.image_size, f.patch_size, f.channels, D);
+    lo_blocked = c->lo_blocked && c->ln_fold && c->split && !c->fp8 && nl > 0 && !pre_ln && !fused_patch && !c->cls_tail && D % 256 == 0 &&
+                            gemm_tiled_applies(rows_g, D, D) && gemm_tiled_applies(rows_g, D, M) &&
+                            gemm_pick_variant((int64_t)batch * L.NP, D, VH_EPI_PATCH_SPLIT) == 6;
+    c->last_lo_blocked = lo_blocked;
+    if (img0 == 0) c->lo_parts.clear();
+    c->lo_parts.push_back({(int64_t)r0, lo_blocked ? rows_g : rows, lo_blocked});
     if (!fused_patch) {
         if ((rc = tmark(ST_IM2COL))) return rc;
         if (in.u8)
@@ -475,12 +487,12 @@
         if ((rc = mark(ST_LNSTATS))) return rc;
     } else if (c->split && !c->fp8 && nl > 0 && !pre_ln) {
         GemmArgs g{col16, c->wp16, P + L.patch_b, xn16, (int64_t)batch * L.NP, D, L.KPA, VH_EPI_PATCH_SPLIT, P + L.pos, L.NP, dt16, 0};
-        g.out16 = xlo16; g.partials = partials_p; g.prow = rows_g;
+        g.out16 = xlo16; g.partials = partials_p; g.prow = rows_g; g.lo_blocked = lo_blocked;
         if ((rc = tmark(ST_PATCH))) return rc;
         HIPCHK(&c->err, launch_gemm(g, s));
         if ((rc = tmark(ST_PATCH))) return rc;
         if ((rc = mark(ST_PATCH))) return rc;
-        HIPCHK(&c->err, launch_cls_rows_split(xn16, xlo16, partials_p, rows_g, P + L.cls, P + L.pos, batch, T, D, dt16, s));
+        HIPCHK(&c->err, launch_cls_rows_split(xn16, xlo16, partials_p, rows_g, P + L.cls, P + L.pos, batch, T, D, dt16, s, lo_blocked));
         if ((rc = mark(ST_CLS))) return rc;
         HIPCHK(&c->err, launch_finalize_stats(partials_p, D / 64, rows_g, D, f.ln_eps, stats_p, s, rows, c->guard_dev, amax_guard));
         if ((rc = mark(ST_LNSTATS))) return rc;
@@ -570,7 +582,7 @@
         if ((rc = tmark(ST_PROJ))) return rc;
         if (att_tiled) {
             GemmArgs go{att16, c->wot_16[l], P + o.ob, xn16, rows_g, D, D, VH_EPI_RESID_SPLIT, nullptr, 0, dt16, 0};
-            go.out16 = xlo16; go.partials = partials_p; go.ab_tiled = 1;
+            go.out16 = xlo16; go.partials = partials_p; go.ab_tiled = 1; go.lo_blocked = lo_blocked;
             HIPCHK(&c->err, launch_gemm(go, s));
         } else if (att_tiled8) {
             GemmArgs go{att16, c->wot_16[l], P + o.ob, xn16, rows_g, D, D, VH_EPI_RESID_SPLIT, so, 0, VH_DTYPE_FP8, 0};
@@ -599,7 +611,7 @@
         if ((rc = tmark(ST_FC2))) return rc;
         if (h_tiled) {
             GemmArgs g2{h16, c->w2t_16[l], P + o.f2b, xn16, rows_g, D, M, VH_EPI_RESID_SPLIT, nullptr, 0, dt16, 0};
-            g2.out16 = xlo16; g2.partials = partials_p; g2.ab_tiled = 1;
+            g2.out16 = xlo16; g2.partials = partials_p; g2.ab_tiled = 1; g2.lo_blocked = lo_blocked;
             HIPCHK(&c->err, launch_gemm(g2, s));
         } else if (h_tiled8) {
             GemmArgs g2{h16, c->w2t_16[l], P + o.f2b, xn16, rows_g, D, M, VH_EPI_RESID_SPLIT, s2, 0, VH_DTYPE_FP8, 0};
@@ -692,7 +704,8 @@
                                 more ? P + L.layer[l + 1].ln1b : nullptr, ST_FC2))) return rc;
     }
     if (c->split && nl > 0)
-        HIPCHK(&c->err, launch_layernorm_split(xn16, xlo16, batch, D, (int64_t)T * D, P + L.lnfw, P + L.lnfb, f.ln_eps, clsn32, c->fp8 ? VH_DTYPE_FP8 : dt16, s));
+        HIPCHK(&c->err, launch_layernorm_split(xn16, xlo16, batch, D, (int64_t)T * D, P + L.lnfw, P + L.lnfb, f.ln_eps, clsn32, c->fp8 ? VH_DTYPE_FP8 : dt16, s,
+                                               lo_blocked && c->ln_fold));
     else
         HIPCHK(&c->err, launch_layernorm(x, batch, D, (int64_t)T * D, P + L.lnfw, P + L.lnfb, f.ln_eps, clsn32, VH_DTYPE_F32_INTERNAL, s));
     if ((rc = mark(ST_LNF))) return rc;
@@ -1112,6 +1125,7 @@
         c->h_tiled = want_tiled || want_tiled8;
         { const char* e = getenv("VH_ATT_TILED"); c->att_tiled = !(e && e[0] == '0'); }
         { const char* e = getenv("VH_QKV_HM"); c->qkv_hm = !(e && e[0] == '0'); }
+        { const char* e = getenv("VH_LO_BLOCKED"); c->lo_blocked = !(e && e[0] == '0'); }
         const char* pf = getenv("VH_PATCH_FUSED");
         c->patch_fused = pf && pf[0] == '1';
     }
@@ -1879,11 +1893,21 @@
                 return VH_OK;
             }
             std::vector<uint16_t> hi(n);
-            std::vector<uint8_t> lo(n);
             HIPCHK(&c->err, hipMemcpy(hi.data(), c->xn16, n * 2, hipMemcpyDeviceToHost));
-            HIPCHK(&c->err, hipMemcpy(lo.data(), c->xlo16, n, hipMemcpyDeviceToHost));
             const float inv = c->dt16 == VH_DTYPE_BF16 ? 1.f / 32.f : 1.f / 256.f;
-            for (size_t i = 0; i < n; ++i) host_out[i] = f(hi[i], c->dt16) + g(lo[i]) * inv;
+            const size_t total_rows = (size_t)c->last_batch * c->L.T;
+            std::vector<uint8_t> lo;
+            for (const auto& part : c->lo_parts) {
+                const size_t r0 = (size_t)part.row0, r1 = std::min(total_rows, r0 + (size_t)part.rows);
+                if (r0 >= r1) continue;
+                lo.resize((size_t)part.rows * D);
+                HIPCHK(&c->err, hipMemcpy(lo.data(), (const char*)c->xlo16 + r0 * D, lo.size(), hipMemcpyDeviceToHost));
+                for (size_t r = r0; r < r1; ++r)
+                    for (size_t k = 0; k < D; ++k) {
+                        const size_t at = part.blocked ? (size_t)lo_blocked_offset((int64_t)(r - r0), (int)k, (int)D) : (r - r0) * D + k;
+                        host_out[r * D + k] = f(hi[r * D + k], c->dt16) + g(lo[at]) * inv;
+                    }
+            }
             return VH_OK;
         }
         HIPCHK(&c->err, hipMemcpy(host_out, c->x, n * 4, hipMemcpyDeviceToHost));
@@ -1908,6 +1932,11 @@
     if (what == 4) {
         if (n_floats != 1) return fail(&c->err, VH_ERR_INVALID, "expected 1 float");
         host_out[0] = c->last_qkv_hm ? 1.f : 0.f;
+        return VH_OK;
+    }
+    if (what == 5) {
+        if (n_floats != 1) return fail(&c->err, VH_ERR_INVALID, "expected 1 float");
+        host_out[0] = c->last_lo_blocked ? 1.f : 0.f;
         return VH_OK;
     }
     return fail(&c->err, VH_ERR_INVALID, "unknown tap %d", what);
@@ -1974,6 +2003,18 @@
                   void* stream) {
     GemmArgs g{a, w, bias, out, M, N, K, epi, aux, aux_i, dtype, variant};
     g.stats = stats; g.out16 = out16; g.partials = partials;
+    if (const char* why = gemm_check(g)) return fail(nullptr, VH_ERR_INVALID, "%s", why);
+    OPCHK(launch_gemm(g, (hipStream_t)stream));
+    OPCHK(hipStreamSynchronize((hipStream_t)stream));
+    return VH_OK;
+}
+int vh_op_gemm_ex2(const void* a, const void* w, const float* bias, void* out, int64_t M, int N, int K, int epi,
+                   const float* aux, int aux_i, const float* stats, void* out16, float* partials, int dtype, int variant,
+                   unsigned int flags, void* stream) {
+    if (flags & ~(unsigned)VH_GEMM_LO_BLOCKED) return fail(nullptr, VH_ERR_INVALID, "gemm_ex2: unknown flag");
+    GemmArgs g{a, w, bias, out, M, N, K, epi, aux, aux_i, dtype, variant};
+    g.stats = stats; g.out16 = out16; g.partials = partials;
+    g.lo_blocked = (flags & VH_GEMM_LO_BLOCKED) ? 1 : 0;
     if (const char* why = gemm_check(g)) return fail(nullptr, VH_ERR_INVALID, "%s", why);
     OPCHK(launch_gemm(g, (hipStream_t)stream));
     OPCHK(hipStreamSynchronize((hipStream_t)stream));
diff --git a/vit-fpga_amd/python/vithip.py b/vit-fpga_amd/python/vithip.py
--- a/vit-fpga_amd/python/vithip.py
+++ b/vit-fpga_amd/python/vithip.py
@@ -133,6 +133,7 @@
     "vh_op_gemm_fp8_ex": (_i, [_vp, _vp, _vp, _vp, _vp, _i64, _i, _i, _i, _vp, _vp, _vp, _vp, _i, _vp]),
     "vh_op_quantize_rows": (_i, [_vp, _i, _i, C.c_float, _vp, _vp, _vp]),
     "vh_op_gemm_ex": (_i, [_vp, _vp, _vp, _vp, _i64, _i, _i, _i, _vp, _i, _vp, _vp, _vp, _i, _i, _vp]),
+    "vh_op_gemm_ex2": (_i, [_vp, _vp, _vp, _vp, _i64, _i, _i, _i, _vp, _i, _vp, _vp, _vp, _i, _i, C.c_uint, _vp]),
     "vh_op_rowstats_cast": (_i, [_vp, _i64, _i, _f, _vp, _vp, _i, _vp]),
     "vh_op_finalize_stats": (_i, [_vp, _i, _i64, _i, _f, _vp, _vp]),
     "vh_op_pre_layernorm": (_i, [_vp, _i64, _i, _vp, _vp, _f, _vp, _vp, _vp, _vp, _i, _vp]),
@@ -942,6 +943,45 @@
                                partials_ptr, dtype, variant, None))
 
 
+GEMM_LO_BLOCKED = 1
+
+
+def op_gemm_ex2(a_ptr, w_ptr, bias_ptr, out_ptr, M, N, K, epilogue, dtype, aux_ptr=None, aux_i=0, stats_ptr=None,
+                out16_ptr=None, partials_ptr=None, variant=0, flags=0):
+    _check(lib().vh_op_gemm_ex2(a_ptr, w_ptr, bias_ptr, out_ptr, M, N, K, epilogue, aux_ptr, aux_i, stats_ptr, out16_ptr,
+                                partials_ptr, dtype, variant, flags, None))
+
+
+def lo_blocked_offset(r, c, n):
+    r, c = np.asarray(r, dtype=np.int64), np.asarray(c, dtype=np.int64)
+    return ((r >> 4) * (n // 64) + (c >> 6)) * 1024 + (r & 7) * 128 + ((c >> 3) & 7) * 16 + ((r >> 3) & 1) * 8 + (c & 7)
+
+
+def _lo_block_index(rows, n):
+    if n <= 0 or n % 64:
+        raise ValueError(f"blocked lo plane: {n} columns is not a positive multiple of 64")
+    if rows <= 0 or rows % 16:
+        raise ValueError(f"blocked lo plane: {rows} rows is not a positive multiple of 16")
+    return lo_blocked_offset(np.arange(rows)[:, None], np.arange(n)[None, :], n)
+
+
+def lo_block(a):
+    a = np.ascontiguousarray(a, dtype=np.uint8)
+    if a.ndim != 2:
+        raise ValueError("lo_block: a [rows, n] plane is expected")
+    out = np.empty(a.size, np.uint8)
+    out[_lo_block_index(*a.shape)] = a
+    return out
+
+
+def lo_unblock(flat, rows, n):
+    flat = np.ascontiguousarray(flat, dtype=np.uint8).reshape(-1)
+    idx = _lo_block_index(rows, n)
+    if flat.size != rows * n:
+        raise ValueError(f"lo_unblock: {flat.size} bytes for a {rows} x {n} plane")
+    return flat[idx]
+
+
 def op_rowstats_cast(x_ptr, rows, dim, eps, x16_ptr, stats_ptr, dtype):
     _check(lib().vh_op_rowstats_cast(x_ptr, rows, dim, eps, x16_ptr, stats_ptr, dtype, None))
 
```

Measured after the change: 28600 images/s (median of 6 runs). About the same (+1.0%).
